# kfkq/DQMC

Measured on AMD Instinct MI355X. Metric: MC sweeps/sec, 2D Hubbard N=256 Ltau=200, higher is better.
Workload: dtype f64; 1 GPU; cfg3: 16x16 Hubbard U=8.0 beta=8.0 Ltau=200 n_stab=10 t=1 mu=-0.1; chains_per_gpu=1, n_chains_total=1, parallelism=independent chains, 1 gpu x 1 chain

## Files before the change

dqmc_amd/abi.py:

```python
from __future__ import annotations

import ctypes as C
import os
from typing import Optional, Tuple

import numpy as np

c_double_p = C.POINTER(C.c_double)
c_int64_p = C.POINTER(C.c_int64)
c_int32_p = C.POINTER(C.c_int32)
c_uint8_p = C.POINTER(C.c_uint8)


class Stats(C.Structure):
    _fields_ = [("acc_rate", C.c_double), ("max_err", C.c_double), ("sum_err", C.c_double),
                ("n_err", C.c_double), ("n_accepted", C.c_int64), ("n_proposed", C.c_int64)]

    @property
    def mean_err(self) -> float:
        return self.sum_err / self.n_err if self.n_err else 0.0


class DqmcError(RuntimeError):
    def __init__(self, code: int, msg: str):
        super().__init__(f"[{code}] {msg}")
        self.code = code


ABI_SYMBOLS = [
    "last_error", "backend", "device_count",
    "to_ldr", "ldr_mul_mat", "mat_mul_ldr", "ldr_mul_ldr", "inv_I_plus_ldr", "inv_I_plus_ldr_mul_ldr",
    "gemm", "rank1_update",
    "create", "create_batch", "n_chains", "destroy", "set_fields", "get_fields", "init", "get_G", "set_G", "get_logdet",
    "n_stack", "get_stack", "sweep_0_to_beta", "sweep_beta_to_0", "sync", "get_stats",
    "wrap_forward", "wrap_backward", "local_update_slice", "calculate_Bbar", "global_action", "set_checkerboard",
    "update_kernel_time", "set_profiling", "slice_path", "debug_snapshot",
    "measure_equal_time", "measure_accumulate", "measure_fetch",
    "sweep_unequal_time", "get_G_tau", "half_warp", "measure_unequal_time", "measure_unequal_fetch",
    "comm_unique_id", "comm_create_rccl", "comm_create_callbacks", "comm_destroy", "comm_rank", "comm_world_size",
    "comm_transport", "comm_barrier", "comm_allreduce_sum", "comm_selftest", "partner_rank", "replica_exchange_round",
    "replica_exchange_batch",
]

UNIQUE_ID_BYTES = 128
SENDRECV_FN = C.CFUNCTYPE(C.c_int, C.c_void_p, C.c_void_p, C.c_void_p, C.c_size_t, C.c_int, C.c_int)


class ExchangeResult(C.Structure):
    _fields_ = [("partner", C.c_int), ("decider", C.c_int), ("accepted", C.c_int), ("pad", C.c_int),
                ("S", C.c_double), ("S_prime", C.c_double), ("S_partner", C.c_double), ("S_prime_partner", C.c_double),
                ("deltaS", C.c_double)]


def _f64(a) -> np.ndarray:
    return np.asfortranarray(a, dtype=np.float64)


def _p(a: np.ndarray):
    return a.ctypes.data_as(c_double_p)


class DqmcLib:

    def __init__(self, path: str, prefix: str):
        if not os.path.exists(path):
            raise FileNotFoundError(
                f"{path} not found: build it first (python -c 'import __graft_entry__ as g; g.build()' or make)")
        self.path, self.prefix = path, prefix
        self._dll = C.CDLL(path, mode=C.RTLD_GLOBAL)
        g = self._sym
        g("last_error").restype = C.c_char_p
        g("backend").restype = C.c_char_p
        g("destroy").restype = None
        g("destroy").argtypes = [C.c_void_p]
        for name in ("set_fields", "get_fields"):
            g(name).argtypes = [C.c_void_p, c_int64_p]
        for name in ("init", "sync", "n_stack"):
            g(name).argtypes = [C.c_void_p]
        g("create").argtypes = [C.POINTER(C.c_void_p), C.c_int, C.c_int, C.c_int, C.c_int, C.c_double,
                                c_double_p, c_double_p, c_double_p, c_double_p]
        if self.has_symbol("create_batch"):
            g("create_batch").argtypes = [C.POINTER(C.c_void_p), C.c_int, C.c_int, C.c_int, C.c_int, C.c_int, c_double_p,
                                          c_double_p, c_double_p, c_double_p, c_double_p]
            g("n_chains").argtypes = [C.c_void_p]
        for name in ("get_G", "set_G", "get_logdet", "global_action"):
            g(name).argtypes = [C.c_void_p, c_double_p]
        g("get_stack").argtypes = [C.c_void_p, C.c_int, c_double_p, c_double_p, c_double_p]
        for name in ("sweep_0_to_beta", "sweep_beta_to_0"):
            g(name).argtypes = [C.c_void_p, c_int32_p, c_uint8_p, c_double_p]
        g("get_stats").argtypes = [C.c_void_p, C.c_void_p]
        for name in ("wrap_forward", "wrap_backward"):
            g(name).argtypes = [C.c_void_p, C.c_int]
        g("local_update_slice").argtypes = [C.c_void_p, C.c_int, c_int32_p, c_uint8_p, c_double_p, C.c_void_p]
        g("calculate_Bbar").argtypes = [C.c_void_p, C.c_int, c_double_p]
        g("set_checkerboard").argtypes = [C.c_void_p, C.c_int, c_int32_p, c_int32_p, c_double_p, c_double_p, c_double_p]
        g("update_kernel_time").argtypes = [C.c_void_p, c_double_p, c_int64_p, c_int64_p]
        g("set_profiling").argtypes = [C.c_void_p, C.c_int]
        if self.has_symbol("slice_path"):
            g("slice_path").argtypes = [C.c_void_p]
        if self.has_symbol("measure_equal_time"):
            g("measure_equal_time").argtypes = [C.c_void_p, C.c_int, C.c_int, c_double_p, c_double_p]
            g("measure_accumulate").argtypes = [C.c_void_p, C.c_int, C.c_int]
            g("measure_fetch").argtypes = [C.c_void_p, c_double_p, c_double_p, c_int64_p, C.c_int]
        if self.has_symbol("sweep_unequal_time"):
            g("sweep_unequal_time").argtypes = [C.c_void_p]
            g("get_G_tau").argtypes = [C.c_void_p, C.c_int, C.c_int, c_double_p]
            g("measure_unequal_time").argtypes = [C.c_void_p, C.c_int, C.c_int, C.c_int, c_double_p]
            g("measure_unequal_fetch").argtypes = [C.c_void_p, c_double_p, c_int64_p, C.c_int]
        if self.has_symbol("half_warp"):
            g("half_warp").argtypes = [C.c_void_p, c_double_p, c_double_p, C.c_int, C.c_int, c_double_p]
        if self.has_symbol("debug_snapshot"):
            g("debug_snapshot").argtypes = [C.c_void_p, c_double_p, C.c_void_p, C.c_void_p, C.c_void_p]
        if self.has_symbol("replica_exchange_round"):
            g("comm_unique_id").argtypes = [C.c_void_p]
            g("comm_create_rccl").argtypes = [C.POINTER(C.c_void_p), C.c_void_p, C.c_int, C.c_int, C.c_int]
            g("comm_create_callbacks").argtypes = [C.POINTER(C.c_void_p), C.c_int, C.c_int, SENDRECV_FN, C.c_void_p]
            g("comm_destroy").argtypes = [C.c_void_p]; g("comm_destroy").restype = None
            g("comm_rank").argtypes = [C.c_void_p]; g("comm_world_size").argtypes = [C.c_void_p]
            g("comm_transport").argtypes = [C.c_void_p]; g("comm_transport").restype = C.c_char_p
            g("comm_barrier").argtypes = [C.c_void_p]; g("comm_selftest").argtypes = [C.c_void_p]
            g("comm_allreduce_sum").argtypes = [C.c_void_p, c_double_p, C.c_int]
            g("partner_rank").argtypes = [C.c_int, C.c_int, C.c_int]
            g("replica_exchange_round").argtypes = [C.c_void_p, C.c_void_p, C.c_int, C.c_double, C.POINTER(ExchangeResult)]
        if self.has_symbol("replica_exchange_batch"):
            g("replica_exchange_batch").argtypes = [C.c_void_p, C.c_void_p, C.c_int, c_double_p, C.POINTER(ExchangeResult)]
        g("to_ldr").argtypes = [C.c_int] + [c_double_p] * 4
        g("ldr_mul_mat").argtypes = [C.c_int] + [c_double_p] * 7
        g("mat_mul_ldr").argtypes = [C.c_int] + [c_double_p] * 7
        g("ldr_mul_ldr").argtypes = [C.c_int] + [c_double_p] * 9
        g("inv_I_plus_ldr").argtypes = [C.c_int] + [c_double_p] * 5
        g("inv_I_plus_ldr_mul_ldr").argtypes = [C.c_int] + [c_double_p] * 7
        g("gemm").argtypes = [C.c_int, c_double_p, C.c_int, c_double_p, C.c_int, c_double_p]
        g("rank1_update").argtypes = [C.c_int, c_double_p, C.c_int, C.c_double]

    def _sym(self, name: str):
        return getattr(self._dll, self.prefix + name)

    def has_symbol(self, name: str) -> bool:
        return hasattr(self._dll, self.prefix + name)

    def check(self, rc: int):
        if rc != 0:
            raise DqmcError(rc, (self._sym("last_error")() or b"").decode())

    def backend(self) -> str:
        return self._sym("backend")().decode()

    def device_count(self) -> int:
        return int(self._sym("device_count")())

    def to_ldr(self, M) -> Tuple[np.ndarray, np.ndarray, np.ndarray]:
        M = _f64(M); n = M.shape[0]
        L, d, R = np.empty((n, n), order="F"), np.empty(n), np.empty((n, n), order="F")
        self.check(self._sym("to_ldr")(n, _p(M), _p(L), _p(d), _p(R)))
        return L, d, R

    def ldr_mul_mat(self, F, M):
        L, d, R = (_f64(x) for x in F); M = _f64(M); n = M.shape[0]
        Lo, do, Ro = np.empty((n, n), order="F"), np.empty(n), np.empty((n, n), order="F")
        self.check(self._sym("ldr_mul_mat")(n, _p(L), _p(d), _p(R), _p(M), _p(Lo), _p(do), _p(Ro)))
        return Lo, do, Ro

    def mat_mul_ldr(self, M, F):
        L, d, R = (_f64(x) for x in F); M = _f64(M); n = M.shape[0]
        Lo, do, Ro = np.empty((n, n), order="F"), np.empty(n), np.empty((n, n), order="F")
        self.check(self._sym("mat_mul_ldr")(n, _p(M), _p(L), _p(d), _p(R), _p(Lo), _p(do), _p(Ro)))
        return Lo, do, Ro

    def ldr_mul_ldr(self, F1, F2):
        L1, d1, R1 = (_f64(x) for x in F1); L2, d2, R2 = (_f64(x) for x in F2); n = L1.shape[0]
        Lo, do, Ro = np.empty((n, n), order="F"), np.empty(n), np.empty((n, n), order="F")
        self.check(self._sym("ldr_mul_ldr")(n, _p(L1), _p(d1), _p(R1), _p(L2), _p(d2), _p(R2), _p(Lo), _p(do), _p(Ro)))
        return Lo, do, Ro

    def inv_I_plus_ldr(self, F) -> Tuple[np.ndarray, float]:
        L, d, R = (_f64(x) for x in F); n = L.shape[0]
        G = np.empty((n, n), order="F"); ld = C.c_double(0.0)
        self.check(self._sym("inv_I_plus_ldr")(n, _p(L), _p(d), _p(R), _p(G), C.byref(ld)))
        return G, ld.value

    def inv_I_plus_ldr_mul_ldr(self, F1, F2) -> np.ndarray:
        L1, d1, R1 = (_f64(x) for x in F1); L2, d2, R2 = (_f64(x) for x in F2); n = L1.shape[0]
        G = np.empty((n, n), order="F")
        self.check(self._sym("inv_I_plus_ldr_mul_ldr")(n, _p(L1), _p(d1), _p(R1), _p(L2), _p(d2), _p(R2), _p(G)))
        return G

    def gemm(self, A, B, transA: bool = False, transB: bool = False) -> np.ndarray:
        A = _f64(A); B = _f64(B); n = A.shape[0]
        Cm = np.empty((n, n), order="F")
        self.check(self._sym("gemm")(n, _p(A), int(transA), _p(B), int(transB), _p(Cm)))
        return Cm

    def rank1_update(self, G, i: int, delta: float) -> np.ndarray:
        G = np.array(G, dtype=np.float64, order="F", copy=True); n = G.shape[0]
        self.check(self._sym("rank1_update")(n, _p(G), int(i), float(delta)))
        return G

    def engine(self, *args, **kw) -> "Engine":
        return Engine(self, *args, **kw)

    def partner_rank(self, rank: int, world: int, attempt: int) -> int:
        return int(self._sym("partner_rank")(rank, world, attempt))

    def exchange_batch(self, engine: "Engine", attempt: int, u, comm: Optional["Comm"] = None) -> list:
        uv = np.ascontiguousarray(np.asarray(u, dtype=np.float64).reshape(-1))
        if uv.shape != (engine.C,):
            raise ValueError(f"u must have shape ({engine.C},), got {uv.shape}")
        res = (ExchangeResult * engine.C)()
        self.check(self._sym("replica_exchange_batch")(engine._h, comm._h if comm is not None else None, int(attempt), _p(uv), res))
        return list(res)

    def comm_unique_id(self) -> bytes:
        buf = C.create_string_buffer(UNIQUE_ID_BYTES)
        self.check(self._sym("comm_unique_id")(buf))
        return buf.raw

    def comm_rccl(self, uid: bytes, world: int, rank: int, device: int) -> "Comm":
        h = C.c_void_p()
        self.check(self._sym("comm_create_rccl")(C.byref(h), C.c_char_p(uid), world, rank, device))
        return Comm(self, h)

    def comm_callbacks(self, world: int, rank: int, fn) -> "Comm":
        def tramp(_user, send, recv, nbytes, partner, tag):
            try:
                got = fn(C.string_at(send, nbytes), int(partner), int(tag))
                if len(got) != nbytes:
                    return -2
                C.memmove(recv, got, nbytes)
                return 0
            except Exception:
                return -1
        cb = SENDRECV_FN(tramp)
        h = C.c_void_p()
        self.check(self._sym("comm_create_callbacks")(C.byref(h), world, rank, cb, None))
        return Comm(self, h, keep=cb)


class Comm:

    def __init__(self, lib: "DqmcLib", h, keep=None):
        self.lib, self._h, self._keep = lib, h, keep

    @property
    def rank(self) -> int:
        return int(self.lib._sym("comm_rank")(self._h))

    @property
    def world(self) -> int:
        return int(self.lib._sym("comm_world_size")(self._h))

    @property
    def transport(self) -> str:
        return self.lib._sym("comm_transport")(self._h).decode()

    def selftest(self):
        self.lib.check(self.lib._sym("comm_selftest")(self._h))

    def barrier(self):
        self.lib.check(self.lib._sym("comm_barrier")(self._h))

    def allreduce_sum(self, x) -> np.ndarray:
        v = np.ascontiguousarray(x, dtype=np.float64).copy()
        self.lib.check(self.lib._sym("comm_allreduce_sum")(self._h, _p(v), int(v.size)))
        return v

    def exchange_round(self, engine: "Engine", attempt: int, u: float) -> ExchangeResult:
        res = ExchangeResult()
        self.lib.check(self.lib._sym("replica_exchange_round")(engine._h, self._h, int(attempt), float(u), C.byref(res)))
        return res

    def exchange_batch(self, engine: "Engine", attempt: int, u) -> list:
        return self.lib.exchange_batch(engine, attempt, u, comm=self)

    def close(self):
        if self._h is not None:
            self.lib._sym("comm_destroy")(self._h); self._h = None

    def __del__(self):
        try:
            self.close()
        except Exception:
            pass


class Engine:

    def __init__(self, lib: DqmcLib, n_sites: int, nt: int, n_stab: int, g, gamma, eta,
                 expK, invexpK, device: int = 0, n_chains: Optional[int] = None):
        self.lib, self.n, self.nt, self.n_stab = lib, int(n_sites), int(nt), int(n_stab)
        self.batched = n_chains is not None
        self.C = int(n_chains) if self.batched else 1
        gamma = np.ascontiguousarray(gamma, dtype=np.float64); eta = np.ascontiguousarray(eta, dtype=np.float64)
        h = C.c_void_p()
        if not self.batched:
            eK, iK = _f64(expK), _f64(invexpK)
            assert eK.shape == (self.n, self.n) and iK.shape == (self.n, self.n)
            lib.check(lib._sym("create")(C.byref(h), device, self.n, self.nt, self.n_stab, float(g),
                                         _p(gamma), _p(eta), _p(eK), _p(iK)))
        else:
            gv = np.ascontiguousarray(np.broadcast_to(np.asarray(g, dtype=np.float64), (self.C,)))
            eK = self._mats_in(np.broadcast_to(np.asarray(expK), (self.C, self.n, self.n)) if np.ndim(expK) == 2 else expK)
            iK = self._mats_in(np.broadcast_to(np.asarray(invexpK), (self.C, self.n, self.n)) if np.ndim(invexpK) == 2 else invexpK)
            lib.check(lib._sym("create_batch")(C.byref(h), device, self.C, self.n, self.nt, self.n_stab, _p(gv),
                                               _p(gamma), _p(eta), _p(eK), _p(iK)))
        self._h: Optional[C.c_void_p] = h

    def _mats_in(self, a) -> np.ndarray:
        a = np.asarray(a, dtype=np.float64).reshape(self.C, self.n, self.n)
        return np.ascontiguousarray(a.transpose(0, 2, 1))

    def _mats_out(self, buf: np.ndarray) -> np.ndarray:
        m = buf.reshape(self.C, self.n, self.n).transpose(0, 2, 1)
        return m if self.batched else np.asfortranarray(m[0])

    def _vec_out(self, buf: np.ndarray) -> np.ndarray:
        return buf.reshape(self.C, -1) if self.batched else buf.reshape(-1)

    def close(self):
        if self._h is not None:
            self.lib._sym("destroy")(self._h); self._h = None

    def __del__(self):
        try:
            self.close()
        except Exception:
            pass

    def __enter__(self):
        return self

    def __exit__(self, *a):
        self.close()

    def _c(self, name, *args):
        self.lib.check(self.lib._sym(name)(self._h, *args))

    def set_fields(self, fields):
        f = np.asarray(fields).reshape(self.C, self.nt, self.n)
        f = np.ascontiguousarray(f.transpose(0, 2, 1), dtype=np.int64)
        self._c("set_fields", f.ctypes.data_as(c_int64_p))

    def get_fields(self) -> np.ndarray:
        f = np.empty((self.C, self.n, self.nt), dtype=np.int64)
        self._c("get_fields", f.ctypes.data_as(c_int64_p))
        f = f.transpose(0, 2, 1)
        return f if self.batched else f[0]

    def init(self):
        self._c("init")

    def get_G(self) -> np.ndarray:
        G = np.empty(self.C * self.n * self.n); self._c("get_G", _p(G)); return self._mats_out(G)

    def set_G(self, G):
        G = self._mats_in(G); self._c("set_G", _p(G))

    def get_logdet(self):
        v = np.zeros(self.C); self._c("get_logdet", _p(v)); return v if self.batched else float(v[0])

    def n_stack(self) -> int:
        return int(self.lib._sym("n_stack")(self._h))

    def get_stack(self, i: int):
        L, d, R = np.empty(self.C * self.n * self.n), np.empty(self.C * self.n), np.empty(self.C * self.n * self.n)
        self._c("get_stack", int(i), _p(L), _p(d), _p(R))
        return self._mats_out(L), self._vec_out(d), self._mats_out(R)

    def _stream(self, perm, kprop, u, rows):
        perm = np.ascontiguousarray(np.asarray(perm).reshape(self.C, rows, self.n), dtype=np.int32)
        kprop = np.ascontiguousarray(np.asarray(kprop).reshape(self.C, rows, self.n), dtype=np.uint8)
        u = np.ascontiguousarray(np.asarray(u).reshape(self.C, rows, self.n), dtype=np.float64)
        return perm, kprop, u

    def sweep_0_to_beta(self, perm, kprop, u):
        perm, kprop, u = self._stream(perm, kprop, u, self.nt)
        self._c("sweep_0_to_beta", perm.ctypes.data_as(c_int32_p), kprop.ctypes.data_as(c_uint8_p), _p(u))

    def sweep_beta_to_0(self, perm, kprop, u):
        perm, kprop, u = self._stream(perm, kprop, u, self.nt)
        self._c("sweep_beta_to_0", perm.ctypes.data_as(c_int32_p), kprop.ctypes.data_as(c_uint8_p), _p(u))

    def sync(self):
        self._c("sync")

    def stats(self):
        arr = (Stats * self.C)(); self._c("get_stats", arr)
        return list(arr) if self.batched else arr[0]

    def wrap_forward(self, l: int):
        self._c("wrap_forward", int(l))

    def wrap_backward(self, l: int):
        self._c("wrap_backward", int(l))

    def local_update_slice(self, l: int, perm, kprop, u):
        perm, kprop, u = self._stream(perm, kprop, u, 1)
        acc = (C.c_int * self.C)()
        self._c("local_update_slice", int(l), perm.ctypes.data_as(c_int32_p), kprop.ctypes.data_as(c_uint8_p), _p(u), acc)
        return list(acc) if self.batched else acc[0]

    def calculate_Bbar(self, i_stack: int) -> np.ndarray:
        B = np.empty(self.C * self.n * self.n); self._c("calculate_Bbar", int(i_stack), _p(B)); return self._mats_out(B)

    def set_checkerboard(self, groups, cosh_t, sinh_t, diag_factor):
        sizes = np.ascontiguousarray([len(g) for g in groups], np.int32)
        flat = [p for g in groups for p in g]
        bonds = np.ascontiguousarray(np.asarray(flat, np.int32).reshape(-1, 2) if flat else np.zeros((1, 2), np.int32))
        par = [np.ascontiguousarray(np.broadcast_to(np.asarray(x, np.float64), (self.C,))) for x in (cosh_t, sinh_t, diag_factor)]
        self._c("set_checkerboard", len(groups), bonds.ctypes.data_as(c_int32_p), sizes.ctypes.data_as(c_int32_p), _p(par[0]), _p(par[1]), _p(par[2]))

    def global_action(self):
        v = np.zeros(self.C); self._c("global_action", _p(v)); return v if self.batched else float(v[0])

    def measure_equal_time(self, L1: int, L2: int):
        sc = np.empty((self.C, 3)); chi = np.empty((self.C, L1 * L2))
        self._c("measure_equal_time", int(L1), int(L2), _p(sc), _p(chi))
        chi = chi.reshape(self.C, L2, L1).transpose(0, 2, 1)
        return (sc, chi) if self.batched else (sc[0], chi[0])

    def measure_accumulate(self, L1: int, L2: int):
        self._c("measure_accumulate", int(L1), int(L2))

    def measure_fetch(self, L1: int, L2: int, reset: bool = True):
        sc = np.empty((self.C, 3)); chi = np.empty((self.C, L1 * L2)); cnt = np.zeros(1, dtype=np.int64)
        self._c("measure_fetch", _p(sc), _p(chi), cnt.ctypes.data_as(c_int64_p), 1 if reset else 0)
        chi = chi.reshape(self.C, L2, L1).transpose(0, 2, 1)
        return ((sc, chi) if self.batched else (sc[0], chi[0])) + (int(cnt[0]),)

    def sweep_unequal_time(self):
        self._c("sweep_unequal_time")

    def get_G_tau(self, which: str, l: int) -> np.ndarray:
        B = np.empty(self.C * self.n * self.n); self._c("get_G_tau", {"tt": 0, "t0": 1, "0t": 2}[which], int(l), _p(B)); return self._mats_out(B)

    def half_warp(self, expK_half=None, invexpK_half=None, which: str = "G", l: int = 0) -> np.ndarray:
        a = _f64(expK_half) if expK_half is not None else None; b = _f64(invexpK_half) if invexpK_half is not None else None
        B = np.empty(self.C * self.n * self.n)
        self._c("half_warp", _p(a) if a is not None else None, _p(b) if b is not None else None, {"G": -1, "tt": 0, "t0": 1, "0t": 2}[which], int(l), _p(B))
        return self._mats_out(B)

    def _ut_cube(self, flat, L1, L2):
        a = flat.reshape(self.C, 3, self.nt + 1, L2, L1).transpose(0, 1, 2, 4, 3)
        return a if self.batched else a[0]

    def measure_unequal_time(self, L1: int, L2: int, accumulate: bool = False):
        if accumulate:
            self._c("measure_unequal_time", int(L1), int(L2), 1, None); return None
        out = np.empty(self.C * 3 * (self.nt + 1) * L1 * L2)
        self._c("measure_unequal_time", int(L1), int(L2), 0, _p(out)); return self._ut_cube(out, L1, L2)

    def measure_unequal_fetch(self, L1: int, L2: int, reset: bool = True):
        out = np.empty(self.C * 3 * (self.nt + 1) * L1 * L2); cnt = np.zeros(1, dtype=np.int64)
        self._c("measure_unequal_fetch", _p(out), cnt.ctypes.data_as(c_int64_p), 1 if reset else 0)
        return self._ut_cube(out, L1, L2), int(cnt[0])

    def debug_snapshot(self):
        ns = self.n_stack()
        we = np.zeros(ns); acc = np.zeros(self.nt, np.int32); sw = np.zeros(80, np.uint32); ep = C.c_uint(0)
        self._c("debug_snapshot", _p(we), acc.ctypes.data, sw.ctypes.data, C.byref(ep))
        return dict(wrap_err=we, accepted=acc, sync_words=sw, slice_epoch=int(ep.value))

    def slice_path(self) -> int:
        return int(self.lib._sym("slice_path")(self._h))

    def set_profiling(self, on: bool):
        self._c("set_profiling", int(bool(on)))

    def update_kernel_time(self):
        ms = C.c_double(0.0); nl = C.c_int64(0); na = C.c_int64(0)
        self._c("update_kernel_time", C.cast(C.byref(ms), c_double_p), C.cast(C.byref(nl), c_int64_p), C.cast(C.byref(na), c_int64_p))
        return ms.value, nl.value, na.value
```

dqmc_amd/csrc/common.h:

```cpp
#pragma once

#include <hip/hip_runtime.h>
#include <cstdint>
#include <memory>
#include <string>

struct dqmc_engine;

namespace dq {

constexpr int WAVE = 64;

void set_error(const std::string& msg);
const char* get_error();

#define DQ_HIP(call)                                                                    \
    do {                                                                                \
        hipError_t _e = (call);                                                         \
        if (_e != hipSuccess) {                                                         \
            ::dq::set_error(std::string(#call) + ": " + hipGetErrorString(_e));         \
            return -2;                                              \
        }                                                                               \
    } while (0)

#define DQ_TRY(expr)                \
    do {                            \
        int _rc = (expr);           \
        if (_rc != 0) return _rc;   \
    } while (0)

template <class T, hipError_t (*Free)(void*)> struct HipDelete { void operator()(T* p) const { (void)Free(p); } };
template <class T> using DevPtr = std::unique_ptr<T[], HipDelete<T, hipFree>>;
using PinnedPtr = std::unique_ptr<char[], HipDelete<char, hipHostFree>>;
template <class T> int dev_alloc(DevPtr<T>& out, size_t count) {
    void* p = nullptr;
    DQ_HIP(hipMalloc(&p, sizeof(T) * count));
    out.reset(static_cast<T*>(p));
    return 0;
}

constexpr int DQ_STATUS_PIVOT = 1;
constexpr int DQ_STATUS_COOP_QR = 2;
constexpr int DQ_STATUS_HANDOFF = 4;
constexpr int DQ_STATUS_CENSUS = 8;

struct Mat {
    double* p = nullptr;
    long stride = 0;
    __host__ __device__ double* at(int c) const { return p + (long)c * stride; }
};
struct CMat {
    const double* p = nullptr;
    long stride = 0;
    CMat() = default;
    __host__ __device__ CMat(const double* p_, long s) : p(p_), stride(s) {}
    __host__ __device__ CMat(const Mat& m) : p(m.p), stride(m.stride) {}
    __host__ __device__ const double* at(int c) const { return p + (long)c * stride; }
};
using Vec = Mat;
using CVec = CMat;

struct GemmDesc {
    CMat A, B;
    Mat C;
    Mat CT{nullptr, 0};
    CVec rs, ks, cs;
    int n = 0;
    int transA = 0;
    int accumulate = 0;
};
int launch_gemm(const GemmDesc& g, int n_chains, hipStream_t s);

int launch_build_expv(const int8_t* fields, long f_stride, int nt, int n, const double* tab_expv ,
                      double* expv, double* invexpv, long v_stride, int n_chains, hipStream_t s);
int launch_split_d(CVec d, Vec dl_inv, Vec ds, double* logsum, int n, int n_chains, hipStream_t s);
int launch_split_d2(CVec d1, Vec dl1, Vec ds1, CVec d2, Vec dl2, Vec ds2, int n, int n_chains, hipStream_t s);
int launch_measure_equal_time(CMat G, double* out, long out_stride, int L1, int L2, int accumulate, int n_chains, hipStream_t s);
int launch_measure_unequal_time(const double* Gtt, const double* Gt0, const double* G0t, double* out, long out_stride, int L1, int L2, int nt,
                                int accumulate, int n_chains, hipStream_t s);
int launch_axpb_identity(CMat in, Mat out, double a, double b, int n, int n_chains, hipStream_t s);
int launch_copy(CMat in, Mat out, long count, int n_chains, hipStream_t s);
int launch_set_identity(Mat out, int n, int n_chains, hipStream_t s);
int launch_transpose_scale(CMat in, Mat out, CVec rs, int n, int n_chains, hipStream_t s);
int launch_max_abs_diff(CMat A, CMat B, double* err, long err_stride, int n, int n_chains, hipStream_t s);
int launch_add_scaled_cols(CMat A, CMat B, CVec cs, Mat C, int n, int n_chains, hipStream_t s);
int launch_scale_rows(CMat in, CVec rs, Mat out, int n, int n_chains, hipStream_t s);
struct DevStats { double acc_rate, max_err, sum_err, n_err; long long n_accepted, n_proposed; };
int launch_fold_stats(DevStats* st, const int* acc, long acc_stride, int n_slices, const double* err, long err_stride, int n_err,
                      int n, int nt, int n_chains, hipStream_t s);

struct QrWork {
    double* tau; long tau_stride;
    int* jpvt; long jpvt_stride;
    unsigned long long* sync = nullptr; long sync_stride = 0;
    int* abort_words = nullptr;
    int* info = nullptr;
    double* pw = nullptr; long pw_stride = 0;
    int* pivpos = nullptr; long pivpos_stride = 0;
};
long qr_panel_work_doubles(int n);
int launch_qr_panel_formq(QrWork w, Mat L, int n, int n_chains, hipStream_t s);
int launch_qr_panel(Mat A, QrWork w, int n, int n_chains, hipStream_t s);
long qrcp_coop_sync_granules(int n);
int qrcp_coop_workgroups(int n, int n_chains);
enum class QrFamily { Panel, ColumnOwner, Cooperative, Streaming };
int launch_to_ldr(QrFamily f, Mat A, Mat L, Vec d, Mat R, QrWork w, int n, int n_chains, hipStream_t s);

int launch_lu_blocked(Mat A, int* perm, long perm_stride, int* rowpos, long rowpos_stride, double* logabsdet, int accumulate_logdet,
                      int* info, int n, int n_chains, hipStream_t s);
int launch_lu_solve(CMat LU, const int* perm, long perm_stride, Mat X, CVec dg, int mode, int n, int n_chains, hipStream_t s);

int launch_tri_solve(CMat R, const int* perm, long perm_stride, Mat X, CVec dg, double* scratch, long scratch_stride, int n, int n_chains, hipStream_t s);

int launch_gj_solve(Mat A, Mat B, Mat X, Mat SA, double* tinv, int* perm, long perm_stride, int* rowpos, long rowpos_stride,
                    double* logabsdet, int accumulate_logdet, int* info, int n, int n_chains, hipStream_t s);

struct UpdateTables {
    double rb[4][3];
    double delta[4][3];
    double ev[4];
    double iev[4];
    double pad[32];
};
struct UpdateDesc {
    Mat G;
    int8_t* fields; long f_stride;
    double* expv; double* invexpv; long v_stride;
    const UpdateTables* tabs;
    const int32_t* perm; const uint8_t* kprop; const double* u; long rs_stride;
    double* Upanel; double* Wpanel; long panel_stride;
    double* Cpanel = nullptr;
    int* state; long state_stride;
    double* prep; long prep_stride;
    Mat GT{nullptr, 0};
    int gt_valid = 0;
    void* slice_sync = nullptr;
    unsigned slice_epoch = 0;
    int slice_absent_tile = -1;
    int slice_absent_l = -1;
    int slice_late_tile = -1, slice_late_us = 0;
    int* info = nullptr;
    int* acc_out; long acc_stride;
    int n, nt;
};
constexpr int UPDATE_KD = 32;

struct SliceSync {
    unsigned long long seq; unsigned int error; unsigned int solo_count; unsigned int pad[12];
    unsigned int arrive[496];
};
constexpr size_t SLICE_SYNC_BYTES = 2048;
static_assert(sizeof(SliceSync) == SLICE_SYNC_BYTES, "SliceSync layout");
constexpr unsigned SLICE_EPOCH_LIMIT = 1u << 24;
constexpr unsigned SLICE_SOLO_BIT = 1u << 30, SLICE_FINAL_BIT = 1u << 31;
__host__ __device__ inline unsigned slice_tag(unsigned epoch, unsigned window) { return (epoch << 8) | window; }
enum class SlicePath { PersistentWalk, PersistentSubmatrix, Solo, Pairs, PairsTailSolo };
int launch_update_slice(SlicePath path, const UpdateDesc& d, int l, int acc_slot, int n_chains, hipStream_t s);
int launch_update_slice_sm(const UpdateDesc& d, int l, int acc_slot, int n_chains, hipStream_t s);
int slice_flush_workgroups(int n);
bool slice_reserve(int device, int n, int n_chains);
void slice_release(int device, int n, int n_chains);
int launch_rank1(Mat G, int i, double delta, double* scratch , long scratch_stride, int n, int n_chains, hipStream_t s);

struct CbDesc {
    CMat in;
    Mat out{nullptr, 0}, outT{nullptr, 0};
    const int* partner = nullptr;
    int n_groups = 0, reverse = 0, inverse = 0;
    const double* par = nullptr; long par_stride = 0;
    CVec rs_in, cs_in, rs_out, cs_out;
    int n = 0;
};
int launch_cb_apply(const CbDesc& d, int n_chains, hipStream_t s);

int update_init_device();
int update_sm_init_device();
int qr_init_device();
int qr_colown_init_device();
int init_device_kernels(int device);

struct EngineFieldsView { int device, n, nt, n_chains; int8_t* fields; hipStream_t stream; };
int engine_fields_view(dqmc_engine* h, EngineFieldsView* v);
int engine_fields_changed(dqmc_engine* h);
int engine_exchange_scratch(dqmc_engine* h, int8_t** saved, int8_t** recv, int** tab);

}
```

dqmc_amd/csrc/engine.hip:

```cpp
#include "common.h"
#include "../../include/dqmc_hip.h"

#include <cmath>
#include <cstdlib>
#include <cstring>
#include <map>
#include <memory>
#include <mutex>
#include <vector>

namespace dq {

static thread_local std::string g_err;
void set_error(const std::string& msg) { g_err = msg; }
const char* get_error() { return g_err.c_str(); }

int init_device_kernels(int device) {
    static std::mutex mu; static bool done[64] = {};
    std::lock_guard<std::mutex> lk(mu);
    if (device < 0 || device >= 64) { set_error("device ordinal out of range"); return -1; }
    if (done[device]) return 0;
    DQ_HIP(hipSetDevice(device));
    DQ_TRY(update_init_device()); DQ_TRY(update_sm_init_device()); DQ_TRY(qr_init_device()); DQ_TRY(qr_colown_init_device());
    done[device] = true;
    return 0;
}

struct Switches { bool qr_panel, qr_streaming, walk_submatrix, lu_classic, slice_multikernel; };
static const Switches& switches() {
    static const Switches sw = [] {
        const char* panel = getenv("DQMC_QR_PANEL");
        return Switches{!(panel && atoi(panel) == 0), getenv("DQMC_QR_STREAMING") != nullptr, getenv("DQMC_WALK_SUBMATRIX") != nullptr,
                        getenv("DQMC_LU_CLASSIC") != nullptr, getenv("DQMC_SLICE_MULTIKERNEL") != nullptr};
    }();
    return sw;
}

constexpr int GJ_MAX_N = 1024, GJ_MAX_CHAINS = 8;
constexpr int TRI_MAX_N = 640;

static QrFamily pick_qr(int n, int chains, bool allow_panel) {
    const Switches& sw = switches();
    if (sw.qr_streaming) return QrFamily::Streaming;
    if (allow_panel && sw.qr_panel && n >= 64 && n <= 1024 && n % 16 == 0 && chains <= 8) return QrFamily::Panel;
    if (n <= 256) return QrFamily::ColumnOwner;
    return qrcp_coop_workgroups(n, chains) <= 200 ? QrFamily::Cooperative : QrFamily::Streaming;
}

struct KernelPlan {
    QrFamily qr;
    enum class Solve { GaussJordan, BlockedLu } solve;
    enum class Rinv { Blocked, PerColumn } rinv;
    static KernelPlan pick(int n, int chains) {
        return KernelPlan{pick_qr(n, chains, true),
                          n <= GJ_MAX_N && chains <= GJ_MAX_CHAINS && !switches().lu_classic ? Solve::GaussJordan : Solve::BlockedLu,
                          n <= TRI_MAX_N ? Rinv::Blocked : Rinv::PerColumn};
    }
};

static SlicePath pick_slice_path(int n, int chains, bool reserved) {
    const Switches& sw = switches();
    const bool walk = n <= 256;
    if (sw.slice_multikernel) return SlicePath::Pairs;
    if (reserved) return walk && !sw.walk_submatrix ? SlicePath::PersistentWalk : SlicePath::PersistentSubmatrix;
    if (!walk) return SlicePath::Pairs;
    return chains >= 224 ? SlicePath::Solo : SlicePath::PairsTailSolo;
}
static bool is_persistent(SlicePath p) { return p == SlicePath::PersistentWalk || p == SlicePath::PersistentSubmatrix; }

struct LdrRef {
    Mat L; Vec d; Mat R;
    int* jpvt = nullptr;
    bool* tri = nullptr;
};
struct LdrStore {
    int n = 0, C = 0;
    DevPtr<double> L, d, R;
    DevPtr<int> jpvt;
    std::unique_ptr<bool[]> tri;
    int alloc(int k, int n_, int C_) {
        n = n_; C = C_;
        const size_t nn = (size_t)n * n;
        DQ_TRY(dev_alloc(L, (size_t)k * C * nn)); DQ_TRY(dev_alloc(d, (size_t)k * C * n));
        DQ_TRY(dev_alloc(R, (size_t)k * C * nn)); DQ_TRY(dev_alloc(jpvt, (size_t)k * C * n));
        tri.reset(new bool[k]());
        return 0;
    }
    LdrRef at(int i) const {
        const long nn = (long)n * n;
        return LdrRef{Mat{L.get() + (long)i * C * nn, nn}, Vec{d.get() + (long)i * C * n, (long)n}, Mat{R.get() + (long)i * C * nn, nn},
                      jpvt.get() + (long)i * C * n, &tri[i]};
    }
};

struct Ctx {
    int n = 0, C = 0, device = 0;
    long nn = 0;
    hipStream_t stream = nullptr;
    static constexpr int NT = 6, NV = 5;
    DevPtr<double> pool;
    DevPtr<double> vpool;
    DevPtr<int> ipool;
    DevPtr<unsigned long long> qsync;
    DevPtr<int> qabort;
    DevPtr<double> tinv;
    DevPtr<double> qpw;
    DevPtr<int> qpivpos;
    DevPtr<double> trinv;
    KernelPlan plan{};

    Mat T(int k) const { return Mat{pool.get() + (long)k * C * nn, nn}; }
    Vec V(int k) const { return Vec{vpool.get() + (long)k * C * n, (long)n}; }
    int* jpvt() const { return ipool.get(); }
    int* lperm() const { return ipool.get() + (long)C * n; }
    int* rowpos() const { return ipool.get() + 2L * C * n; }
    int* info() const { return ipool.get() + 3L * C * n; }

    int init(int n_, int C_, int device_) {
        n = n_; C = C_; device = device_; nn = (long)n * n;
        DQ_HIP(hipSetDevice(device));
        DQ_TRY(init_device_kernels(device));
        DQ_HIP(hipStreamCreateWithFlags(&stream, hipStreamNonBlocking));
        DQ_TRY(dev_alloc(pool, (size_t)NT * C * nn));
        DQ_TRY(dev_alloc(vpool, (size_t)NV * C * n));
        DQ_TRY(dev_alloc(ipool, 3L * C * n + 4));
        plan = KernelPlan::pick(n, C);
        if (plan.qr == QrFamily::Cooperative) { DQ_TRY(dev_alloc(qsync, (size_t)qrcp_coop_sync_granules(n) * C)); DQ_TRY(dev_alloc(qabort, C)); }
        if (plan.qr == QrFamily::Panel) { DQ_TRY(dev_alloc(qpw, (size_t)qr_panel_work_doubles(n) * C)); DQ_TRY(dev_alloc(qpivpos, (size_t)n * C)); }
        if (plan.solve == KernelPlan::Solve::GaussJordan) DQ_TRY(dev_alloc(tinv, (size_t)2048 * C));
        if (plan.rinv == KernelPlan::Rinv::Blocked) DQ_TRY(dev_alloc(trinv, (size_t)16 * (n + 16) * C));
        DQ_HIP(hipMemsetAsync(ipool.get(), 0, sizeof(int) * (3L * C * n + 4), stream));
        return 0;
    }
    ~Ctx() { if (stream) (void)hipStreamDestroy(stream); }

    int gemm(CMat A, CMat B, Mat Cm, CVec rs = CVec(), CVec ks = CVec(), CVec cs = CVec(), int transA = 0, int accumulate = 0, Mat CT = Mat{nullptr, 0}) {
        GemmDesc g; g.A = A; g.B = B; g.C = Cm; g.CT = CT; g.rs = rs; g.ks = ks; g.cs = cs; g.n = n; g.transA = transA; g.accumulate = accumulate;
        return launch_gemm(g, C, stream);
    }
    int to_ldr(Mat A, LdrRef out, bool direct = true) {
        const bool keep = direct && out.jpvt != nullptr;
        QrWork w{V(4).p, (long)n, keep ? out.jpvt : jpvt(), (long)n};
        w.sync = qsync.get(); w.sync_stride = qrcp_coop_sync_granules(n); w.abort_words = qabort.get(); w.info = info();
        w.pw = qpw.get(); w.pw_stride = qr_panel_work_doubles(n); w.pivpos = qpivpos.get(); w.pivpos_stride = n;
        if (out.tri) *out.tri = keep;
        return launch_to_ldr(plan.qr, A, out.L, out.d, out.R, w, n, C, stream);
    }
    int r_inverse_scaled(LdrRef F, CVec dinv, Mat X, Mat lu_scratch) {
        if (F.tri && *F.tri && F.jpvt) {
            if (plan.rinv == KernelPlan::Rinv::Blocked) return launch_tri_solve(F.R, F.jpvt, n, X, dinv, trinv.get(), 16L * (n + 16), n, C, stream);
            return launch_lu_solve(F.R, F.jpvt, n, X, dinv, 2, n, C, stream);
        }
        DQ_TRY(launch_copy(F.R, lu_scratch, nn, C, stream));
        DQ_TRY(launch_lu_blocked(lu_scratch, lperm(), n, rowpos(), n, nullptr, 0, info(), n, C, stream));
        return launch_lu_solve(lu_scratch, lperm(), n, X, dinv, 1, n, C, stream);
    }
    int mat_mul_ldr(CMat M, LdrRef F, LdrRef out) {
        DQ_TRY(gemm(M, F.L, T(0), CVec(), CVec(), CVec(F.d)));
        LdrRef q{out.L, out.d, T(1)};
        DQ_TRY(to_ldr(T(0), q));
        if (out.tri) *out.tri = false;
        return gemm(T(1), F.R, out.R);
    }
    int ldr_mul_mat(LdrRef F, CMat M, LdrRef out) {
        DQ_TRY(gemm(F.R, M, T(0), CVec(F.d)));
        LdrRef q{T(1), out.d, out.R, out.jpvt, out.tri};
        DQ_TRY(to_ldr(T(0), q));
        return gemm(F.L, T(1), out.L);
    }
    int ldr_mul_ldr(LdrRef F1, LdrRef F2, LdrRef out) {
        DQ_TRY(gemm(F1.R, F2.L, T(0), CVec(F1.d), CVec(), CVec(F2.d)));
        LdrRef q{T(1), out.d, T(2)};
        DQ_TRY(to_ldr(T(0), q));
        if (out.tri) *out.tri = false;
        DQ_TRY(gemm(F1.L, T(1), out.L));
        return gemm(T(2), F2.R, out.R);
    }
    int solve(Mat M, Mat RHS, Mat out, double* logdet_acc, Mat* Y) {
        if (plan.solve == KernelPlan::Solve::GaussJordan) {
            DQ_TRY(launch_gj_solve(M, RHS, out, T(5), tinv.get(), lperm(), n, rowpos(), n, logdet_acc, 1, info(), n, C, stream));
            *Y = out; return 0;
        }
        DQ_TRY(launch_lu_blocked(M, lperm(), n, rowpos(), n, logdet_acc, 1, info(), n, C, stream));
        DQ_TRY(launch_lu_solve(M, lperm(), n, RHS, CVec(), 0, n, C, stream));
        *Y = RHS; return 0;
    }
    int inv_I_plus_ldr(LdrRef F, Mat G, double* logdet ) {
        DQ_TRY(launch_split_d(F.d, V(0), V(1), logdet, n, C, stream));
        DQ_TRY(r_inverse_scaled(F, V(0), T(1), T(0)));
        DQ_TRY(launch_add_scaled_cols(T(1), F.L, V(1), T(2), n, C, stream));
        DQ_TRY(launch_transpose_scale(T(2), T(3), CVec(), n, C, stream));
        DQ_TRY(launch_transpose_scale(T(1), T(4), CVec(), n, C, stream));
        Mat Y; DQ_TRY(solve(T(3), T(4), T(0), logdet, &Y));
        return launch_transpose_scale(Y, G, CVec(), n, C, stream);
    }
    int inv_I_plus_ldr_mul_ldr(LdrRef F1, LdrRef F2, Mat G) {
        DQ_TRY(launch_split_d2(F1.d, V(0), V(1), F2.d, V(2), V(3), n, C, stream));
        DQ_TRY(r_inverse_scaled(F2, V(2), T(1), T(0)));
        DQ_TRY(gemm(F1.L, T(1), T(2), V(0), CVec(), CVec(), 1));
        DQ_TRY(gemm(F1.R, F2.L, T(2), V(1), CVec(), V(3), 0, 1));
        DQ_TRY(launch_transpose_scale(F1.L, T(3), V(0), n, C, stream));
        Mat Y; DQ_TRY(solve(T(2), T(3), T(0), nullptr, &Y));
        return gemm(T(1), Y, G);
    }
    int inv_invldr_plus_ldr(LdrRef F1, LdrRef F2, Mat G, bool negate) {
        DQ_TRY(launch_split_d(F1.d, V(0), V(1), nullptr, n, C, stream));
        DQ_TRY(launch_split_d(F2.d, V(2), V(3), nullptr, n, C, stream));
        DQ_TRY(r_inverse_scaled(F2, V(2), T(1), T(0)));
        DQ_TRY(gemm(F1.L, T(1), T(2), V(0), CVec(), CVec(), 1));
        DQ_TRY(gemm(F1.R, F2.L, T(2), V(1), CVec(), V(3), 0, 1));
        DQ_TRY(launch_scale_rows(F1.R, V(1), T(3), n, C, stream));
        Mat Y; DQ_TRY(solve(T(2), T(3), T(0), nullptr, &Y));
        DQ_TRY(gemm(T(1), Y, G));
        if (negate) DQ_TRY(launch_axpb_identity(G, G, -1.0, 0.0, n, C, stream));
        return 0;
    }
};

static int take_status(const Ctx& c, int* bits = nullptr) {
    int w[4] = {0, 0, 0, 0};
    DQ_HIP(hipMemcpy(w, c.info(), sizeof w, hipMemcpyDeviceToHost));
    if (bits) *bits = w[0];
    if (w[0] == 0) return 0;
    (void)hipMemset(c.info(), 0, sizeof w);
    if (w[0] & DQ_STATUS_HANDOFF) {
        set_error("persistent slice kernel: a workgroup that had checked in stopped answering (device fault or pre-emption beyond the spin bound); the chain state is undefined -- set the fields again and call dqmc_init; this engine uses the scan / flush kernel pairs from now on");
    } else if (w[0] & DQ_STATUS_CENSUS) {
        char msg[640];
        snprintf(msg, sizeof msg, "persistent sub-matrix slice kernel: its workgroups did not all become resident at time slice %d (device shared with other "
                 "work?).  That slice and every later slice of the call(s) in flight proposed NOTHING (fields unchanged there, acceptance counts 0, their part of "
                 "the random stream is spent); wraps and stabilisations ran, so fields, G and the stack are consistent with each other, but the sweep is not the "
                 "one the stream describes from that slice on.  This engine uses the scan / flush kernel pairs from now on: restore the fields of the last "
                 "completed sweep and call dqmc_init, or keep the state as a valid (shortened) sweep", w[1] - 1);
        set_error(msg);
    } else if (w[0] & DQ_STATUS_COOP_QR) {
        set_error("cooperative QRCP gave up waiting for a partner workgroup (not co-resident?)");
    } else {
        set_error("LU factorisation hit a zero or NaN pivot");
    }
    return DQMC_ENUMERIC;
}

struct Engine {
    int n = 0, nt = 0, n_stab = 0, n_stack = 0, C = 1, device = 0;
    long nn = 0;
    std::vector<int> loc_l_end;
    std::vector<double> g_host, gamma_host, eta_host;
    std::vector<unsigned char> seen;
    Ctx ctx;
    hipStream_t s = nullptr;

    DevPtr<double> expK, invexpK;
    bool cb = false; int cb_groups = 0;
    DevPtr<int> cb_partner;
    DevPtr<double> cb_par;
    DevPtr<int8_t> fields;
    DevPtr<double> expv, invexpv;
    DevPtr<UpdateTables> tabs; DevPtr<double> tab8;
    bool gt_valid = false;
    DevPtr<double> G, Gtmp, GT;
    DevPtr<double> pg_eye, pg_ones;
    DevPtr<double> bb0, bb1;
    LdrStore stack;
    LdrStore spare;
    DevPtr<double> logdet;
    DevPtr<int32_t> rs_perm; DevPtr<uint8_t> rs_k; DevPtr<double> rs_u;
    PinnedPtr h_stage;
    hipEvent_t stage_free = nullptr;
    DevPtr<double> Upanel, Wpanel;
    DevPtr<double> Cpanel;
    struct InitBatch { DevPtr<double> bb, tau; LdrStore f; } ib;
    DevPtr<int> state;
    DevPtr<double> prep;
    DevPtr<double> meas_now, meas_sum;
    struct UnequalTime { DevPtr<double> G[3], tmp, err, meas_now, meas_sum; LdrStore bt; } ut;
    bool ut_valid = false; long long ut_meas_count = 0;
    struct HalfWarp { DevPtr<double> expK, invexpK, out; } hw;
    long long meas_count = 0;
    DevPtr<char> slice_sync;
    bool reserved = false;
    SlicePath slice_path = SlicePath::Pairs;
    unsigned slice_epoch = 0;
    int slice_absent_l = -1;
    int slice_late_tile = -1, slice_late_us = 0;
    int slice_absent_tile = -1;
    DevPtr<int> acc;
    struct Exchange { DevPtr<int8_t> saved, recv; DevPtr<int> tab; } xch;
    DevPtr<double> err;
    DevPtr<DevStats> dstats;
    bool stack_valid = false;
    bool profiling = false;
    std::vector<std::pair<hipEvent_t, hipEvent_t>> ev_pairs;
    size_t ev_used = 0;
    double upd_ms = 0.0; long long upd_launches = 0; long long upd_accept_base = 0;

    Mat mG() const { return Mat{G.get(), nn}; }
    CVec ev(int l) const { return CVec(expv.get() + (long)l * n, (long)nt * n); }
    CVec iev(int l) const { return CVec(invexpv.get() + (long)l * n, (long)nt * n); }
    int stack_idx(int l) const { return l / n_stab; }
    int local_l(int l) const { return l % n_stab; }

    ~Engine() {
        if (s) (void)hipStreamSynchronize(s);
        if (reserved) slice_release(device, n, C);
        for (auto& p : ev_pairs) { (void)hipEventDestroy(p.first); (void)hipEventDestroy(p.second); }
        if (stage_free) (void)hipEventDestroy(stage_free);
    }

    int create(int device_, int C_, int n_, int nt_, int n_stab_, const double* g, const double* gamma, const double* eta,
               const double* eK, const double* ieK) {
        device = device_; C = C_; n = n_; nt = nt_; n_stab = n_stab_; nn = (long)n * n;
        n_stack = (int)std::ceil(static_cast<double>(nt) / n_stab);
        loc_l_end.assign(n_stack, n_stab - 1);
        if (nt % n_stab != 0) loc_l_end[n_stack - 1] = nt % n_stab - 1;
        g_host.assign(g, g + C); gamma_host.assign(gamma, gamma + 4); eta_host.assign(eta, eta + 4);
        DQ_TRY(ctx.init(n, C, device)); s = ctx.stream;
        reserved = slice_reserve(device, n, C);
        slice_path = pick_slice_path(n, C, reserved);
        if (const char* a = getenv("DQMC_DEBUG_SLICE_ABSENT")) { slice_absent_tile = atoi(a); if (const char* c = strchr(a, ':')) slice_absent_l = atoi(c + 1); }
        if (const char* a = getenv("DQMC_DEBUG_SLICE_LATE")) { slice_late_tile = atoi(a); if (const char* c = strchr(a, ':')) slice_late_us = atoi(c + 1); }
        DQ_TRY(dev_alloc(expK, C * nn)); DQ_TRY(dev_alloc(invexpK, C * nn));
        DQ_TRY(dev_alloc(fields, (size_t)C * nt * n)); DQ_TRY(dev_alloc(expv, (size_t)C * nt * n)); DQ_TRY(dev_alloc(invexpv, (size_t)C * nt * n));
        DQ_TRY(dev_alloc(tabs, C)); DQ_TRY(dev_alloc(tab8, (size_t)C * 8));
        if (C == 1) { DQ_TRY(dev_alloc(pg_eye, nn)); DQ_TRY(dev_alloc(pg_ones, (size_t)n)); DQ_TRY(launch_set_identity(Mat{pg_eye.get(), nn}, n, 1, s)); const std::vector<double> one_h((size_t)n, 1.0); DQ_HIP(hipMemcpy(pg_ones.get(), one_h.data(), sizeof(double) * n, hipMemcpyHostToDevice)); }
        DQ_TRY(dev_alloc(G, C * nn)); DQ_TRY(dev_alloc(Gtmp, C * nn)); DQ_TRY(dev_alloc(GT, C * nn)); DQ_TRY(dev_alloc(bb0, C * nn)); DQ_TRY(dev_alloc(bb1, C * nn));
        DQ_TRY(stack.alloc(n_stack, n, C)); DQ_TRY(spare.alloc(1, n, C));
        DQ_TRY(dev_alloc(logdet, C));
        DQ_TRY(dev_alloc(rs_perm, (size_t)C * nt * n)); DQ_TRY(dev_alloc(rs_k, (size_t)C * nt * n)); DQ_TRY(dev_alloc(rs_u, (size_t)C * nt * n));
        DQ_TRY(dev_alloc(Upanel, (size_t)C * UPDATE_KD * n)); DQ_TRY(dev_alloc(Wpanel, (size_t)C * UPDATE_KD * n)); DQ_TRY(dev_alloc(Cpanel, (size_t)C * UPDATE_KD * UPDATE_KD));
        DQ_TRY(dev_alloc(state, (size_t)C * 4)); DQ_TRY(dev_alloc(prep, (size_t)C * 4 * n)); DQ_TRY(dev_alloc(meas_now, (size_t)C * (3 + n))); DQ_TRY(dev_alloc(meas_sum, (size_t)C * (3 + n))); DQ_HIP(hipMemsetAsync(meas_sum.get(), 0, sizeof(double) * C * (3 + n), s)); DQ_TRY(dev_alloc(slice_sync, (size_t)C * SLICE_SYNC_BYTES)); DQ_HIP(hipMemsetAsync(slice_sync.get(), 0, (size_t)C * SLICE_SYNC_BYTES, s)); DQ_TRY(dev_alloc(acc, (size_t)C * nt)); DQ_TRY(dev_alloc(err, (size_t)C * n_stack));
        DQ_TRY(dev_alloc(dstats, C));
        void* stage = nullptr;
        DQ_HIP(hipHostMalloc(&stage, (size_t)C * nt * n * (sizeof(int32_t) + sizeof(uint8_t) + sizeof(double)), hipHostMallocDefault)); h_stage.reset(static_cast<char*>(stage));
        DQ_HIP(hipEventCreateWithFlags(&stage_free, hipEventDisableTiming));
        DQ_HIP(hipEventRecord(stage_free, s));
        DQ_HIP(hipMemcpyAsync(expK.get(), eK, sizeof(double) * C * nn, hipMemcpyHostToDevice, s));
        DQ_HIP(hipMemcpyAsync(invexpK.get(), ieK, sizeof(double) * C * nn, hipMemcpyHostToDevice, s));
        DQ_HIP(hipMemsetAsync(fields.get(), 0, (size_t)C * nt * n, s));
        DQ_HIP(hipMemsetAsync(G.get(), 0, sizeof(double) * C * nn, s));
        DQ_HIP(hipMemsetAsync(dstats.get(), 0, sizeof(DevStats) * C, s));
        DQ_HIP(hipMemsetAsync(logdet.get(), 0, sizeof(double) * C, s));
        DQ_HIP(hipMemsetAsync(state.get(), 0, sizeof(int) * C * 4, s));
        std::vector<UpdateTables> ht(C); std::vector<double> h8((size_t)C * 8);
        static const int proposal[4][3] = {{1, 2, 3}, {0, 2, 3}, {0, 1, 3}, {0, 1, 2}};
        const double alpha = -1.0;
        for (int c = 0; c < C; ++c) {
            std::memset(&ht[c], 0, sizeof(UpdateTables));
            for (int o = 0; o < 4; ++o) for (int k = 0; k < 3; ++k) {
                const int nf = proposal[o][k];
                const double gammaR = gamma[nf] / gamma[o];
                const double d_eta = eta[nf] - eta[o];
                const double bosonR = std::exp(alpha * g[c] * d_eta);
                ht[c].rb[o][k] = gammaR * bosonR;
                ht[c].delta[o][k] = (1.0 / bosonR) - 1.0;
            }
            for (int f = 0; f < 4; ++f) { ht[c].ev[f] = std::exp(g[c] * eta[f]); ht[c].iev[f] = std::exp(-g[c] * eta[f]); h8[(size_t)c * 8 + f] = ht[c].ev[f]; h8[(size_t)c * 8 + 4 + f] = ht[c].iev[f]; }
        }
        DQ_HIP(hipMemcpyAsync(tabs.get(), ht.data(), sizeof(UpdateTables) * C, hipMemcpyHostToDevice, s));
        DQ_HIP(hipMemcpyAsync(tab8.get(), h8.data(), sizeof(double) * C * 8, hipMemcpyHostToDevice, s));
        DQ_TRY(launch_build_expv(fields.get(), (long)nt * n, nt, n, tab8.get(), expv.get(), invexpv.get(), (long)nt * n, C, s));
        DQ_HIP(hipStreamSynchronize(s));
        return 0;
    }

    int cb_apply(CMat in, Mat out, Mat outT, bool reverse, bool inverse, CVec rs_in, CVec cs_in, CVec rs_out, CVec cs_out, int chains, long par_stride) {
        CbDesc d; d.in = in; d.out = out; d.outT = outT; d.partner = cb_partner.get(); d.n_groups = cb_groups; d.reverse = reverse ? 1 : 0; d.inverse = inverse ? 1 : 0;
        d.par = cb_par.get(); d.par_stride = par_stride; d.rs_in = rs_in; d.cs_in = cs_in; d.rs_out = rs_out; d.cs_out = cs_out; d.n = n;
        return launch_cb_apply(d, chains, s);
    }
    int set_checkerboard(int n_groups, const int32_t* bonds, const int32_t* group_sizes, const double* ch, const double* sh, const double* f) {
        if (n_groups < 1 || n_groups > 64 || !bonds || !group_sizes || !ch || !sh || !f) { set_error("set_checkerboard: bad argument"); return DQMC_EINVAL; }
        if (n > 4096) { set_error("set_checkerboard: n_sites > 4096"); return DQMC_EINVAL; }
        std::vector<int> partner((size_t)n_groups * n);
        size_t b = 0;
        for (int g = 0; g < n_groups; ++g) {
            int* pt = partner.data() + (size_t)g * n;
            for (int i = 0; i < n; ++i) pt[i] = i;
            if (group_sizes[g] < 0 || group_sizes[g] > n / 2) { set_error("set_checkerboard: a group holds at most n_sites/2 bonds"); return DQMC_EINVAL; }
            for (int k = 0; k < group_sizes[g]; ++k, ++b) {
                const int i = bonds[2 * b], j = bonds[2 * b + 1];
                if (i < 0 || i >= n || j < 0 || j >= n || i == j) { set_error("set_checkerboard: bond site out of range"); return DQMC_EINVAL; }
                if (pt[i] != i || pt[j] != j) { set_error("set_checkerboard: the bonds of one group must be disjoint"); return DQMC_EINVAL; }
                pt[i] = j; pt[j] = i;
            }
        }
        std::vector<double> par((size_t)C * 4);
        for (int c = 0; c < C; ++c) {
            if (!(f[c] > 0.0) || !std::isfinite(ch[c]) || !std::isfinite(sh[c])) { set_error("set_checkerboard: diag_factor must be positive, cosh / sinh finite"); return DQMC_EINVAL; }
            par[4 * c] = ch[c]; par[4 * c + 1] = sh[c]; par[4 * c + 2] = f[c]; par[4 * c + 3] = 1.0 / f[c];
        }
        DQ_HIP(hipStreamSynchronize(s));
        if (!cb_par) DQ_TRY(dev_alloc(cb_par, (size_t)C * 4));
        DevPtr<int> pt;
        DQ_TRY(dev_alloc(pt, partner.size()));
        DQ_HIP(hipMemcpy(pt.get(), partner.data(), sizeof(int) * partner.size(), hipMemcpyHostToDevice));
        DQ_HIP(hipMemcpy(cb_par.get(), par.data(), sizeof(double) * par.size(), hipMemcpyHostToDevice));
        cb_partner = std::move(pt); cb_groups = n_groups; cb = true;
        Mat id{bb0.get(), nn};
        DQ_TRY(launch_set_identity(id, n, C, s));
        DQ_TRY(cb_apply(id, Mat{expK.get(), nn}, Mat{nullptr, 0}, false, false, CVec(), CVec(), CVec(), CVec(), C, 4));
        DQ_TRY(cb_apply(id, Mat{invexpK.get(), nn}, Mat{nullptr, 0}, true, true, CVec(), CVec(), CVec(), CVec(), C, 4));
        stack_valid = false; gt_valid = false; ut_valid = false;
        DQ_HIP(hipStreamSynchronize(s));
        return 0;
    }

    int Bbar(int is, Mat* out) {
        const int l0 = is * n_stab;
        Mat cur{bb0.get(), nn}, nxt{bb1.get(), nn};
        DQ_TRY(launch_scale_rows(CMat(expK.get(), nn), ev(l0), cur, n, C, s));
        for (int loc = 1; loc <= loc_l_end[is]; ++loc) {
            if (cb) DQ_TRY(cb_apply(cur, nxt, Mat{nullptr, 0}, false, false, CVec(), CVec(), ev(l0 + loc), CVec(), C, 4));
            else DQ_TRY(ctx.gemm(CMat(expK.get(), nn), cur, nxt, ev(l0 + loc)));
            std::swap(cur, nxt);
        }
        *out = cur; return 0;
    }
    int init() {
        if (C == 1 && n <= 256 && nt % n_stab == 0 && n_stack >= 2) return init_batched();
        const LdrRef tmp = spare.at(0);
        for (int i = n_stack - 1; i >= 0; --i) {
            Mat bb; DQ_TRY(Bbar(i, &bb));
            if (i == n_stack - 1) DQ_TRY(ctx.to_ldr(bb, stack.at(i)));
            else { DQ_TRY(ctx.to_ldr(bb, tmp)); DQ_TRY(ctx.ldr_mul_ldr(stack.at(i + 1), tmp, stack.at(i))); }
        }
        stack_valid = true;
        gt_valid = false;
        return ctx.inv_I_plus_ldr(stack.at(0), mG(), logdet.get());
    }
    int init_batched() {
        const int S = n_stack;
        if (!ib.tau) {
            InitBatch b; DQ_TRY(dev_alloc(b.bb, (size_t)2 * S * nn)); DQ_TRY(dev_alloc(b.tau, (size_t)S * n)); DQ_TRY(b.f.alloc(S, n, 1));
            ib = std::move(b);
        }
        const long bstride = (long)n_stab * n;
        Mat cur{ib.bb.get(), nn}, nxt{ib.bb.get() + (size_t)S * nn, nn};
        DQ_TRY(launch_scale_rows(CMat(expK.get(), 0), CVec(expv.get(), bstride), cur, n, S, s));
        for (int loc = 1; loc < n_stab; ++loc) {
            if (cb) DQ_TRY(cb_apply(cur, nxt, Mat{nullptr, 0}, false, false, CVec(), CVec(), CVec(expv.get() + (long)loc * n, bstride), CVec(), S, 0));
            else {
                GemmDesc g; g.A = CMat(expK.get(), 0); g.B = cur; g.C = nxt; g.rs = CVec(expv.get() + (long)loc * n, bstride); g.n = n;
                DQ_TRY(launch_gemm(g, S, s));
            }
            std::swap(cur, nxt);
        }
        const LdrRef all = ib.f.at(0);
        QrWork w{ib.tau.get(), (long)n, all.jpvt, (long)n};
        w.info = ctx.info();
        DQ_TRY(launch_to_ldr(pick_qr(n, S, false), cur, all.L, all.d, all.R, w, n, S, s));
        const LdrRef last = stack.at(S - 1), own = ib.f.at(S - 1);
        DQ_TRY(launch_copy(own.L, last.L, nn, 1, s));
        DQ_TRY(launch_copy(own.R, last.R, nn, 1, s));
        DQ_HIP(hipMemcpyAsync(last.d.p, own.d.p, sizeof(double) * n, hipMemcpyDeviceToDevice, s));
        DQ_HIP(hipMemcpyAsync(last.jpvt, own.jpvt, sizeof(int) * n, hipMemcpyDeviceToDevice, s));
        *last.tri = true;
        for (int i = S - 2; i >= 0; --i) DQ_TRY(ctx.ldr_mul_ldr(stack.at(i + 1), ib.f.at(i), stack.at(i)));
        stack_valid = true;
        gt_valid = false;
        return ctx.inv_I_plus_ldr(stack.at(0), mG(), logdet.get());
    }
    int wrap_forward(int l) {
        if (cb) {
            DQ_TRY(cb_apply(mG(), Mat{nullptr, 0}, ctx.T(0), false, false, CVec(), CVec(), CVec(), CVec(), C, 4));
            gt_valid = use_gt();
            return cb_apply(ctx.T(0), Mat{GT.get(), nn}, mG(), false, true, CVec(), CVec(), iev(l), ev(l), C, 4);
        }
        DQ_TRY(ctx.gemm(CMat(expK.get(), nn), mG(), ctx.T(0)));
        gt_valid = use_gt();
        return ctx.gemm(ctx.T(0), CMat(invexpK.get(), nn), mG(), ev(l), CVec(), iev(l), 0, 0, use_gt() ? Mat{GT.get(), nn} : Mat{nullptr, 0});
    }
    bool piggyback() const { return C == 1 && !cb && n <= 256 && pg_eye != nullptr; }
    int wrap_forward_piggy(int l, const double* Pprev, double* Pnext) {
        GemmDesc g; g.A = CMat(expK.get(), 0); g.B = CMat(G.get(), (long)(Pprev - G.get())); g.C = Mat{ctx.T(0).p, (long)(Pnext - ctx.T(0).p)};
        g.rs = CVec(pg_ones.get(), (long)((expv.get() + (long)(l - 1) * n) - pg_ones.get())); g.n = n;
        DQ_TRY(launch_gemm(g, 2, s));
        gt_valid = use_gt();
        return ctx.gemm(ctx.T(0), CMat(invexpK.get(), nn), mG(), ev(l), CVec(), iev(l), 0, 0, use_gt() ? Mat{GT.get(), nn} : Mat{nullptr, 0});
    }
    int wrap_backward_piggy(int l, const double* Pprev, double* Pnext) {
        DQ_TRY(ctx.gemm(CMat(invexpK.get(), nn), mG(), ctx.T(0), CVec(), iev(l)));
        gt_valid = use_gt();
        GemmDesc g; g.A = CMat(ctx.T(0).p, (long)(Pprev - ctx.T(0).p)); g.B = CMat(expK.get(), 0); g.C = Mat{G.get(), (long)(Pnext - G.get())};
        g.ks = CVec(expv.get() + (long)l * n, 0); g.n = n;
        if (use_gt()) g.CT = Mat{GT.get(), (long)(ctx.T(1).p - GT.get())};
        return launch_gemm(g, 2, s);
    }
    int wrap_backward(int l) {
        if (cb) {
            DQ_TRY(cb_apply(mG(), Mat{nullptr, 0}, ctx.T(0), true, true, iev(l), ev(l), CVec(), CVec(), C, 4));
            gt_valid = use_gt();
            return cb_apply(ctx.T(0), Mat{GT.get(), nn}, mG(), true, false, CVec(), CVec(), CVec(), CVec(), C, 4);
        }
        DQ_TRY(ctx.gemm(CMat(invexpK.get(), nn), mG(), ctx.T(0), CVec(), iev(l)));
        gt_valid = use_gt();
        return ctx.gemm(ctx.T(0), CMat(expK.get(), nn), mG(), CVec(), ev(l), CVec(), 0, 0, use_gt() ? Mat{GT.get(), nn} : Mat{nullptr, 0});
    }
    bool use_gt() const { return n <= 256 || slice_path == SlicePath::PersistentSubmatrix; }
    UpdateDesc udesc() const {
        UpdateDesc d; d.G = mG(); d.fields = fields.get(); d.f_stride = (long)nt * n; d.expv = expv.get(); d.invexpv = invexpv.get(); d.v_stride = (long)nt * n;
        d.tabs = tabs.get(); d.perm = rs_perm.get(); d.kprop = rs_k.get(); d.u = rs_u.get(); d.rs_stride = (long)nt * n; d.Upanel = Upanel.get(); d.Wpanel = Wpanel.get(); d.Cpanel = Cpanel.get();
        d.panel_stride = (long)UPDATE_KD * n; d.state = state.get(); d.state_stride = 4; d.prep = prep.get(); d.prep_stride = 4L * n; d.slice_sync = is_persistent(slice_path) ? slice_sync.get() : nullptr; d.slice_epoch = slice_epoch; d.slice_absent_tile = slice_absent_tile; d.slice_absent_l = slice_absent_l; d.slice_late_tile = slice_late_tile; d.slice_late_us = slice_late_us; d.GT = Mat{GT.get(), nn}; d.gt_valid = gt_valid ? 1 : 0; d.info = ctx.info(); d.acc_out = acc.get(); d.acc_stride = nt; d.n = n; d.nt = nt;
        return d;
    }
    int local_update(int l) {
        hipEvent_t e0 = nullptr, e1 = nullptr;
        if (profiling) {
            if (ev_used == ev_pairs.size()) { hipEvent_t a, b; DQ_HIP(hipEventCreate(&a)); DQ_HIP(hipEventCreate(&b)); ev_pairs.emplace_back(a, b); }
            e0 = ev_pairs[ev_used].first; e1 = ev_pairs[ev_used].second; ++ev_used;
            DQ_HIP(hipEventRecord(e0, s));
        }
        if (is_persistent(slice_path)) {
            if (++slice_epoch >= SLICE_EPOCH_LIMIT) { DQ_HIP(hipMemsetAsync(slice_sync.get(), 0, (size_t)C * SLICE_SYNC_BYTES, s)); slice_epoch = 1; }
        }
        DQ_TRY(launch_update_slice(slice_path, udesc(), l, l, C, s));
        if (profiling) DQ_HIP(hipEventRecord(e1, s));
        return 0;
    }
    int check_stream(const char* who, const int32_t* perm, const uint8_t* kprop, const double* u, size_t rows) {
        if (!perm || !kprop || !u) { set_error(std::string(who) + ": null random-stream pointer"); return DQMC_EINVAL; }
        seen.assign((size_t)n, 0);
        for (size_t row = 0; row < rows; ++row) {
            const int32_t* pr = perm + row * n; const uint8_t* kr = kprop + row * n; const unsigned char mark = (unsigned char)(1 + (row & 1));
            if ((row & 1) == 0) std::fill(seen.begin(), seen.end(), 0);
            for (int idx = 0; idx < n; ++idx) {
                const int32_t i = pr[idx];
                if (i < 0 || i >= n || seen[i] == mark || kr[idx] > 2) { set_error(std::string(who) + ": perm is not a permutation of the sites, or kprop > 2"); return DQMC_EINVAL; }
                seen[i] = mark;
            }
        }
        return 0;
    }
    int upload_stream(const int32_t* perm, const uint8_t* kprop, const double* u) {
        const size_t cnt = (size_t)C * nt * n;
        DQ_TRY(check_stream("sweep", perm, kprop, u, (size_t)C * nt));
        DQ_HIP(hipEventSynchronize(stage_free));
        char* base = h_stage.get();
        double* hu = reinterpret_cast<double*>(base);
        int32_t* hp = reinterpret_cast<int32_t*>(base + cnt * sizeof(double));
        uint8_t* hk = reinterpret_cast<uint8_t*>(base + cnt * (sizeof(double) + sizeof(int32_t)));
        std::memcpy(hu, u, cnt * sizeof(double)); std::memcpy(hp, perm, cnt * sizeof(int32_t)); std::memcpy(hk, kprop, cnt);
        DQ_HIP(hipMemcpyAsync(rs_u.get(), hu, cnt * sizeof(double), hipMemcpyHostToDevice, s));
        DQ_HIP(hipMemcpyAsync(rs_perm.get(), hp, cnt * sizeof(int32_t), hipMemcpyHostToDevice, s));
        DQ_HIP(hipMemcpyAsync(rs_k.get(), hk, cnt, hipMemcpyHostToDevice, s));
        DQ_HIP(hipEventRecord(stage_free, s));
        return 0;
    }
    int sweep_fwd() {
        int n_err = 0;
        DQ_HIP(hipMemsetAsync(err.get(), 0, sizeof(double) * C * n_stack, s));
        const bool pg = piggyback();
        double* Pcur = bb0.get(); double* Pnxt = bb1.get();
        for (int l = 0; l < nt; ++l) {
            const int is = stack_idx(l), loc = local_l(l);
            if (pg && loc >= 1) { DQ_TRY(wrap_forward_piggy(l, loc == 1 ? pg_eye.get() : Pcur, Pnxt)); std::swap(Pcur, Pnxt); }
            else DQ_TRY(wrap_forward(l));
            DQ_TRY(local_update(l));
            if (loc == loc_l_end[is]) {
                std::swap(G, Gtmp);
                Mat bb;
                if (pg) {
                    if (loc == 0) DQ_TRY(launch_scale_rows(CMat(expK.get(), nn), ev(l), Mat{Pnxt, nn}, n, C, s));
                    else DQ_TRY(ctx.gemm(CMat(expK.get(), nn), CMat(Pcur, nn), Mat{Pnxt, nn}, ev(l)));
                    std::swap(Pcur, Pnxt); bb = Mat{Pcur, nn};
                } else DQ_TRY(Bbar(is, &bb));
                if (is == 0) DQ_TRY(ctx.to_ldr(bb, stack.at(0)));
                else DQ_TRY(ctx.mat_mul_ldr(bb, stack.at(is - 1), stack.at(is)));
                gt_valid = false;
                if (l == nt - 1) DQ_TRY(ctx.inv_I_plus_ldr(stack.at(is), mG(), logdet.get()));
                else DQ_TRY(ctx.inv_I_plus_ldr_mul_ldr(stack.at(is), stack.at(is + 1), mG()));
                DQ_TRY(launch_max_abs_diff(CMat(Gtmp.get(), nn), mG(), err.get() + n_err, n_stack, n, C, s));
                ++n_err;
            }
        }
        return launch_fold_stats(dstats.get(), acc.get(), nt, nt, err.get(), n_stack, n_err, n, nt, C, s);
    }
    int sweep_bwd() {
        int n_err = 0;
        DQ_HIP(hipMemsetAsync(err.get(), 0, sizeof(double) * C * n_stack, s));
        const bool pg = piggyback();
        double* Pcur = bb0.get(); double* Pnxt = bb1.get();
        for (int l = nt - 1; l >= 0; --l) {
            DQ_TRY(local_update(l));
            const int is = stack_idx(l);
            if (pg) { DQ_TRY(wrap_backward_piggy(l, local_l(l) == loc_l_end[is] ? pg_eye.get() : Pcur, Pnxt)); std::swap(Pcur, Pnxt); }
            else DQ_TRY(wrap_backward(l));
            if (local_l(l) == 0) {
                std::swap(G, Gtmp);
                Mat bb;
                if (pg) bb = Mat{Pcur, nn}; else DQ_TRY(Bbar(is, &bb));
                if (is == n_stack - 1) DQ_TRY(ctx.to_ldr(bb, stack.at(is)));
                else DQ_TRY(ctx.ldr_mul_mat(stack.at(is + 1), bb, stack.at(is)));
                gt_valid = false;
                if (l == 0) DQ_TRY(ctx.inv_I_plus_ldr(stack.at(is), mG(), logdet.get()));
                else DQ_TRY(ctx.inv_I_plus_ldr_mul_ldr(stack.at(is - 1), stack.at(is), mG()));
                DQ_TRY(launch_max_abs_diff(CMat(Gtmp.get(), nn), mG(), err.get() + n_err, n_stack, n, C, s));
                ++n_err;
            }
        }
        return launch_fold_stats(dstats.get(), acc.get(), nt, nt, err.get(), n_stack, n_err, n, nt, C, s);
    }
    Mat utm(int which, int l) const { return Mat{ut.G[which].get() + (long)l * C * nn, nn}; }
    int sweep_unequal() {
        if (!ut.tmp) {
            UnequalTime u;
            for (int w = 0; w < 3; ++w) DQ_TRY(dev_alloc(u.G[w], (size_t)(nt + 1) * C * nn));
            DQ_TRY(dev_alloc(u.tmp, (size_t)3 * C * nn)); DQ_TRY(dev_alloc(u.err, (size_t)C * 3 * n_stack));
            const size_t mcount = (size_t)C * 3 * (nt + 1) * n;
            DQ_TRY(dev_alloc(u.meas_now, mcount)); DQ_TRY(dev_alloc(u.meas_sum, mcount)); DQ_TRY(u.bt.alloc(2, n, C));
            DQ_HIP(hipMemsetAsync(u.meas_sum.get(), 0, sizeof(double) * mcount, s));
            ut = std::move(u);
        }
        auto bt = [&](int b) { return ut.bt.at(b); };
        int cur = 0, n_err = 0;
        DQ_HIP(hipMemsetAsync(ut.err.get(), 0, sizeof(double) * C * 3 * n_stack, s));
        DQ_TRY(launch_copy(mG(), utm(0, 0), nn, C, s));
        for (int l = 0; l < nt; ++l) {
            if (l == 0) {
                DQ_TRY(launch_copy(utm(0, 0), utm(1, 0), nn, C, s));
                DQ_TRY(launch_axpb_identity(utm(0, 0), utm(2, 0), 1.0, -1.0, n, C, s));
            }
            DQ_TRY(ctx.gemm(CMat(expK.get(), nn), utm(0, l), ctx.T(0)));
            DQ_TRY(ctx.gemm(ctx.T(0), CMat(invexpK.get(), nn), utm(0, l + 1), ev(l), CVec(), iev(l)));
            DQ_TRY(ctx.gemm(CMat(expK.get(), nn), utm(1, l), utm(1, l + 1), ev(l)));
            DQ_TRY(ctx.gemm(utm(2, l), CMat(invexpK.get(), nn), utm(2, l + 1), CVec(), CVec(), iev(l)));
            const int is = stack_idx(l);
            if (local_l(l) == loc_l_end[is]) {
                for (int w = 0; w < 3; ++w) DQ_TRY(launch_copy(utm(w, l + 1), Mat{ut.tmp.get() + (long)w * C * nn, nn}, nn, C, s));
                Mat bb; DQ_TRY(Bbar(is, &bb));
                if (is == 0) DQ_TRY(ctx.to_ldr(bb, bt(cur)));
                else { DQ_TRY(ctx.mat_mul_ldr(bb, bt(cur), bt(cur ^ 1))); cur ^= 1; }
                if (l == nt - 1) {
                    DQ_TRY(ctx.inv_I_plus_ldr(bt(cur), utm(0, l + 1), logdet.get()));
                    DQ_TRY(launch_axpb_identity(utm(0, l + 1), utm(1, l + 1), -1.0, 1.0, n, C, s));
                    DQ_TRY(launch_axpb_identity(utm(0, l + 1), utm(2, l + 1), -1.0, 0.0, n, C, s));
                } else {
                    DQ_TRY(ctx.inv_I_plus_ldr_mul_ldr(bt(cur), stack.at(is + 1), utm(0, l + 1)));
                    DQ_TRY(ctx.inv_invldr_plus_ldr(bt(cur), stack.at(is + 1), utm(1, l + 1), false));
                    DQ_TRY(ctx.inv_invldr_plus_ldr(stack.at(is + 1), bt(cur), utm(2, l + 1), true));
                }
                for (int w = 0; w < 3; ++w) {
                    DQ_TRY(launch_max_abs_diff(CMat(ut.tmp.get() + (long)w * C * nn, nn), utm(w, l + 1), ut.err.get() + n_err, 3L * n_stack, n, C, s));
                    ++n_err;
                }
            }
        }
        ut_valid = true;
        return launch_fold_stats(dstats.get(), acc.get(), nt, 0, ut.err.get(), 3L * n_stack, n_err, n, nt, C, s);
    }
    int sync_and_check() {
        DQ_HIP(hipStreamSynchronize(s));
        if (profiling && ev_used) {
            for (size_t k = 0; k < ev_used; ++k) { float ms = 0.f; DQ_HIP(hipEventElapsedTime(&ms, ev_pairs[k].first, ev_pairs[k].second)); upd_ms += ms; }
            upd_launches += (long long)ev_used; ev_used = 0;
        }
        int bits = 0;
        const int rc = take_status(ctx, &bits);
        if (bits & (DQ_STATUS_HANDOFF | DQ_STATUS_CENSUS)) {
            slice_path = pick_slice_path(n, C, false); gt_valid = false;
            if (bits & DQ_STATUS_HANDOFF) { (void)hipMemset(slice_sync.get(), 0, (size_t)C * SLICE_SYNC_BYTES); slice_epoch = 0; }
        }
        return rc;
    }
    int download_fields(std::vector<int8_t>& f) const {
        std::vector<int8_t> dev((size_t)C * nt * n);
        DQ_HIP(hipMemcpy(dev.data(), fields.get(), dev.size(), hipMemcpyDeviceToHost));
        f.resize(dev.size());
        for (int c = 0; c < C; ++c) for (int i = 0; i < n; ++i) for (int l = 0; l < nt; ++l)
            f[(size_t)c * nt * n + l + (size_t)nt * i] = dev[(size_t)c * nt * n + (size_t)l * n + i];
        return 0;
    }
    int copy_out_equal_time(const double* src, double* scalars, double* chi_r) const {
        const size_t w = 3 + (size_t)n;
        std::vector<double> tmp((size_t)C * w);
        DQ_HIP(hipMemcpy(tmp.data(), src, sizeof(double) * tmp.size(), hipMemcpyDeviceToHost));
        for (int c = 0; c < C; ++c) {
            if (scalars) std::copy(tmp.begin() + c * w, tmp.begin() + c * w + 3, scalars + 3 * (size_t)c);
            if (chi_r) std::copy(tmp.begin() + c * w + 3, tmp.begin() + (c + 1) * w, chi_r + (size_t)c * n);
        }
        return 0;
    }
};

struct Stateless {
    Ctx ctx;
    LdrStore ldr;
    DevPtr<double> mats;
    DevPtr<double> logdet;
    Mat M(int k) const { return Mat{mats.get() + k * ctx.nn, ctx.nn}; }
};
static std::mutex g_ctx_mu;
static std::map<int, std::unique_ptr<Stateless>> g_ctx;

static int get_ctx(int n, Stateless** out) {
    if (n <= 0) { set_error("n must be positive"); return DQMC_EINVAL; }
    int count = 0;
    if (hipGetDeviceCount(&count) != hipSuccess || count == 0) { set_error("no HIP device available: this library requires a gfx950 GPU"); return DQMC_ENODEVICE; }
    auto it = g_ctx.find(n);
    if (it == g_ctx.end()) {
        std::unique_ptr<Stateless> x(new Stateless);
        DQ_TRY(x->ctx.init(n, 1, 0));
        DQ_TRY(x->ldr.alloc(3, n, 1)); DQ_TRY(dev_alloc(x->mats, 4L * n * n)); DQ_TRY(dev_alloc(x->logdet, 1));
        it = g_ctx.emplace(n, std::move(x)).first;
    }
    *out = it->second.get();
    return hipSetDevice(0) == hipSuccess ? 0 : DQMC_ENODEVICE;
}
static int upload_ldr(Stateless* x, int k, const double* L, const double* d, const double* R, LdrRef* out) {
    const Ctx& c = x->ctx;
    *out = x->ldr.at(k); *out->tri = false;
    DQ_HIP(hipMemcpyAsync(out->L.p, L, sizeof(double) * c.nn, hipMemcpyHostToDevice, c.stream));
    DQ_HIP(hipMemcpyAsync(out->R.p, R, sizeof(double) * c.nn, hipMemcpyHostToDevice, c.stream));
    DQ_HIP(hipMemcpyAsync(out->d.p, d, sizeof(double) * c.n, hipMemcpyHostToDevice, c.stream));
    return 0;
}
static int download_ldr(Ctx* c, LdrRef f, double* L, double* d, double* R) {
    DQ_HIP(hipMemcpyAsync(L, f.L.p, sizeof(double) * c->nn, hipMemcpyDeviceToHost, c->stream));
    DQ_HIP(hipMemcpyAsync(R, f.R.p, sizeof(double) * c->nn, hipMemcpyDeviceToHost, c->stream));
    DQ_HIP(hipMemcpyAsync(d, f.d.p, sizeof(double) * c->n, hipMemcpyDeviceToHost, c->stream));
    DQ_HIP(hipStreamSynchronize(c->stream));
    return take_status(*c);
}

}

using namespace dq;

struct dqmc_engine { Engine e; };

#define ENGINE_CALL(h) if (!(h)) { set_error("null engine"); return DQMC_EINVAL; } Engine& e = (h)->e; DQ_HIP(hipSetDevice(e.device))

namespace dq {
int engine_fields_view(dqmc_engine* h, EngineFieldsView* v) {
    if (!h || !v) { set_error("null engine"); return DQMC_EINVAL; }
    Engine& e = h->e;
    v->device = e.device; v->n = e.n; v->nt = e.nt; v->n_chains = e.C; v->fields = e.fields.get(); v->stream = e.s;
    return 0;
}
int engine_fields_changed(dqmc_engine* h) {
    ENGINE_CALL(h);
    e.stack_valid = false; e.gt_valid = false;
    return launch_build_expv(e.fields.get(), (long)e.nt * e.n, e.nt, e.n, e.tab8.get(), e.expv.get(), e.invexpv.get(), (long)e.nt * e.n, e.C, e.s);
}
int engine_exchange_scratch(dqmc_engine* h, int8_t** saved, int8_t** recv, int** tab) {
    ENGINE_CALL(h);
    if (!e.xch.tab) {
        Engine::Exchange x; DQ_TRY(dev_alloc(x.saved, (size_t)e.C * e.nt * e.n)); DQ_TRY(dev_alloc(x.recv, (size_t)2 * e.nt * e.n)); DQ_TRY(dev_alloc(x.tab, (size_t)2 * e.C));
        e.xch = std::move(x);
    }
    *saved = e.xch.saved.get(); *recv = e.xch.recv.get(); *tab = e.xch.tab.get();
    return 0;
}
}

#define API_LOCK std::lock_guard<std::mutex> _lk(g_ctx_mu)

extern "C" {

const char* dqmc_last_error(void) { return get_error(); }
const char* dqmc_backend(void) { return "hip:gfx950"; }
int dqmc_device_count(void) { int c = 0; if (hipGetDeviceCount(&c) != hipSuccess) return 0; return c; }

int dqmc_to_ldr(int n, const double* M, double* L, double* d, double* R) {
    API_LOCK; Stateless* x; DQ_TRY(get_ctx(n, &x)); Ctx* c = &x->ctx;
    if (!M || !L || !d || !R) { set_error("null pointer"); return DQMC_EINVAL; }
    DQ_HIP(hipMemcpyAsync(x->M(0).p, M, sizeof(double) * c->nn, hipMemcpyHostToDevice, c->stream));
    LdrRef out = x->ldr.at(0);
    DQ_TRY(c->to_ldr(x->M(0), out));
    return download_ldr(c, out, L, d, R);
}
int dqmc_ldr_mul_mat(int n, const double* L, const double* d, const double* R, const double* M, double* Lo, double* d_o, double* Ro) {
    API_LOCK; Stateless* x; DQ_TRY(get_ctx(n, &x)); Ctx* c = &x->ctx;
    LdrRef F; DQ_TRY(upload_ldr(x, 0, L, d, R, &F));
    DQ_HIP(hipMemcpyAsync(x->M(0).p, M, sizeof(double) * c->nn, hipMemcpyHostToDevice, c->stream));
    LdrRef out = x->ldr.at(2);
    DQ_TRY(c->ldr_mul_mat(F, x->M(0), out));
    return download_ldr(c, out, Lo, d_o, Ro);
}
int dqmc_mat_mul_ldr(int n, const double* M, const double* L, const double* d, const double* R, double* Lo, double* d_o, double* Ro) {
    API_LOCK; Stateless* x; DQ_TRY(get_ctx(n, &x)); Ctx* c = &x->ctx;
    LdrRef F; DQ_TRY(upload_ldr(x, 0, L, d, R, &F));
    DQ_HIP(hipMemcpyAsync(x->M(0).p, M, sizeof(double) * c->nn, hipMemcpyHostToDevice, c->stream));
    LdrRef out = x->ldr.at(2);
    DQ_TRY(c->mat_mul_ldr(x->M(0), F, out));
    return download_ldr(c, out, Lo, d_o, Ro);
}
int dqmc_ldr_mul_ldr(int n, const double* L1, const double* d1, const double* R1, const double* L2, const double* d2, const double* R2, double* Lo, double* d_o, double* Ro) {
    API_LOCK; Stateless* x; DQ_TRY(get_ctx(n, &x)); Ctx* c = &x->ctx;
    LdrRef F1, F2; DQ_TRY(upload_ldr(x, 0, L1, d1, R1, &F1)); DQ_TRY(upload_ldr(x, 1, L2, d2, R2, &F2));
    LdrRef out = x->ldr.at(2);
    DQ_TRY(c->ldr_mul_ldr(F1, F2, out));
    return download_ldr(c, out, Lo, d_o, Ro);
}
int dqmc_inv_I_plus_ldr(int n, const double* L, const double* d, const double* R, double* G, double* logdet) {
    API_LOCK; Stateless* x; DQ_TRY(get_ctx(n, &x)); Ctx* c = &x->ctx;
    LdrRef F; DQ_TRY(upload_ldr(x, 0, L, d, R, &F));
    DQ_TRY(c->inv_I_plus_ldr(F, x->M(1), x->logdet.get()));
    DQ_HIP(hipMemcpyAsync(G, x->M(1).p, sizeof(double) * c->nn, hipMemcpyDeviceToHost, c->stream));
    double ld = 0.0;
    DQ_HIP(hipMemcpyAsync(&ld, x->logdet.get(), sizeof(double), hipMemcpyDeviceToHost, c->stream));
    DQ_HIP(hipStreamSynchronize(c->stream));
    if (logdet) *logdet = ld;
    return take_status(*c);
}
int dqmc_inv_I_plus_ldr_mul_ldr(int n, const double* L1, const double* d1, const double* R1, const double* L2, const double* d2, const double* R2, double* G) {
    API_LOCK; Stateless* x; DQ_TRY(get_ctx(n, &x)); Ctx* c = &x->ctx;
    LdrRef F1, F2; DQ_TRY(upload_ldr(x, 0, L1, d1, R1, &F1)); DQ_TRY(upload_ldr(x, 1, L2, d2, R2, &F2));
    DQ_TRY(c->inv_I_plus_ldr_mul_ldr(F1, F2, x->M(1)));
    DQ_HIP(hipMemcpyAsync(G, x->M(1).p, sizeof(double) * c->nn, hipMemcpyDeviceToHost, c->stream));
    DQ_HIP(hipStreamSynchronize(c->stream));
    return take_status(*c);
}
int dqmc_gemm(int n, const double* A, int transA, const double* B, int transB, double* Cm) {
    API_LOCK; Stateless* x; DQ_TRY(get_ctx(n, &x)); Ctx* c = &x->ctx;
    DQ_HIP(hipMemcpyAsync(x->M(0).p, A, sizeof(double) * c->nn, hipMemcpyHostToDevice, c->stream));
    DQ_HIP(hipMemcpyAsync(x->M(1).p, B, sizeof(double) * c->nn, hipMemcpyHostToDevice, c->stream));
    CMat Bm = x->M(1);
    if (transB) { DQ_TRY(launch_transpose_scale(x->M(1), x->M(2), CVec(), n, 1, c->stream)); Bm = x->M(2); }
    DQ_TRY(c->gemm(x->M(0), Bm, x->M(3), CVec(), CVec(), CVec(), transA ? 1 : 0));
    DQ_HIP(hipMemcpyAsync(Cm, x->M(3).p, sizeof(double) * c->nn, hipMemcpyDeviceToHost, c->stream));
    DQ_HIP(hipStreamSynchronize(c->stream));
    return 0;
}
int dqmc_rank1_update(int n, double* G, int i, double delta) {
    API_LOCK; Stateless* x; DQ_TRY(get_ctx(n, &x)); Ctx* c = &x->ctx;
    if (i < 0 || i >= n) { set_error("site index out of range"); return DQMC_ERANGE; }
    DQ_HIP(hipMemcpyAsync(x->M(0).p, G, sizeof(double) * c->nn, hipMemcpyHostToDevice, c->stream));
    DQ_TRY(launch_rank1(x->M(0), i, delta, x->M(1).p, 2L * n + 1, n, 1, c->stream));
    DQ_HIP(hipMemcpyAsync(G, x->M(0).p, sizeof(double) * c->nn, hipMemcpyDeviceToHost, c->stream));
    DQ_HIP(hipStreamSynchronize(c->stream));
    return 0;
}

int dqmc_create_batch(dqmc_engine** out, int device, int n_chains, int n_sites, int nt, int n_stab, const double* g,
                      const double gamma[4], const double eta[4], const double* expK, const double* invexpK) {
    if (!out || n_chains <= 0 || n_sites <= 0 || nt <= 0 || n_stab <= 0 || !g || !gamma || !eta || !expK || !invexpK) { set_error("bad argument"); return DQMC_EINVAL; }
    if (n_sites > 1024) { set_error("n_sites > 1024 is not supported by the single-workgroup kernels"); return DQMC_EINVAL; }
    int count = 0;
    if (hipGetDeviceCount(&count) != hipSuccess || count == 0) { set_error("no HIP device available: this library requires a gfx950 GPU"); return DQMC_ENODEVICE; }
    if (device < 0 || device >= count) { set_error("device ordinal out of range"); return DQMC_EINVAL; }
    dqmc_engine* h = new (std::nothrow) dqmc_engine;
    if (!h) return DQMC_ENOMEM;
    int rc = h->e.create(device, n_chains, n_sites, nt, n_stab, g, gamma, eta, expK, invexpK);
    if (rc) { delete h; return rc; }
    *out = h; return 0;
}
int dqmc_create(dqmc_engine** out, int device, int n_sites, int nt, int n_stab, double g, const double gamma[4], const double eta[4],
                const double* expK, const double* invexpK) {
    return dqmc_create_batch(out, device, 1, n_sites, nt, n_stab, &g, gamma, eta, expK, invexpK);
}
int dqmc_set_checkerboard(dqmc_engine* h, int n_groups, const int32_t* bonds, const int32_t* group_sizes, const double* cosh_t, const double* sinh_t,
                          const double* diag_factor) {
    ENGINE_CALL(h);
    return e.set_checkerboard(n_groups, bonds, group_sizes, cosh_t, sinh_t, diag_factor);
}
void dqmc_destroy(dqmc_engine* h) { if (h) { (void)hipSetDevice(h->e.device); delete h; } }
int dqmc_n_chains(dqmc_engine* h) { return h ? h->e.C : 0; }

int dqmc_set_fields(dqmc_engine* h, const int64_t* f) {
    ENGINE_CALL(h);
    std::vector<int8_t> tmp((size_t)e.C * e.nt * e.n);
    for (int c = 0; c < e.C; ++c) for (int i = 0; i < e.n; ++i) for (int l = 0; l < e.nt; ++l) {
        const int64_t v = f[(size_t)c * e.nt * e.n + l + (size_t)e.nt * i];
        if (v < 0 || v > 3) { set_error("field value outside {0,1,2,3}"); return DQMC_EINVAL; }
        tmp[(size_t)c * e.nt * e.n + (size_t)l * e.n + i] = (int8_t)v;
    }
    DQ_HIP(hipStreamSynchronize(e.s));
    DQ_HIP(hipMemcpy(e.fields.get(), tmp.data(), tmp.size(), hipMemcpyHostToDevice));
    DQ_TRY(launch_build_expv(e.fields.get(), (long)e.nt * e.n, e.nt, e.n, e.tab8.get(), e.expv.get(), e.invexpv.get(), (long)e.nt * e.n, e.C, e.s));
    DQ_HIP(hipStreamSynchronize(e.s));
    return 0;
}
int dqmc_get_fields(dqmc_engine* h, int64_t* f) {
    ENGINE_CALL(h);
    DQ_TRY(e.sync_and_check());
    std::vector<int8_t> tmp; DQ_TRY(e.download_fields(tmp));
    std::copy(tmp.begin(), tmp.end(), f);
    return 0;
}
int dqmc_init(dqmc_engine* h) { ENGINE_CALL(h); DQ_TRY(e.init()); return e.sync_and_check(); }
int dqmc_get_G(dqmc_engine* h, double* G) {
    ENGINE_CALL(h); DQ_TRY(e.sync_and_check());
    DQ_HIP(hipMemcpy(G, e.G.get(), sizeof(double) * e.C * e.nn, hipMemcpyDeviceToHost)); return 0;
}
int dqmc_set_G(dqmc_engine* h, const double* G) {
    ENGINE_CALL(h); DQ_HIP(hipStreamSynchronize(e.s));
    DQ_HIP(hipMemcpy(e.G.get(), G, sizeof(double) * e.C * e.nn, hipMemcpyHostToDevice)); e.gt_valid = false; return 0;
}
int dqmc_get_logdet(dqmc_engine* h, double* ld) {
    ENGINE_CALL(h); DQ_TRY(e.sync_and_check());
    DQ_HIP(hipMemcpy(ld, e.logdet.get(), sizeof(double) * e.C, hipMemcpyDeviceToHost)); return 0;
}
int dqmc_n_stack(dqmc_engine* h) { return h ? h->e.n_stack : 0; }
int dqmc_get_stack(dqmc_engine* h, int i, double* L, double* d, double* R) {
    ENGINE_CALL(h);
    if (i < 0 || i >= e.n_stack) { set_error("LDR Stack index out of bounds"); return DQMC_ERANGE; }
    if (!e.stack_valid) { set_error("stack not initialised: call dqmc_init first"); return DQMC_EINVAL; }
    DQ_TRY(e.sync_and_check());
    LdrRef f = e.stack.at(i);
    DQ_HIP(hipMemcpy(L, f.L.p, sizeof(double) * e.C * e.nn, hipMemcpyDeviceToHost));
    DQ_HIP(hipMemcpy(R, f.R.p, sizeof(double) * e.C * e.nn, hipMemcpyDeviceToHost));
    DQ_HIP(hipMemcpy(d, f.d.p, sizeof(double) * e.C * e.n, hipMemcpyDeviceToHost));
    return 0;
}
int dqmc_sweep_0_to_beta(dqmc_engine* h, const int32_t* perm, const uint8_t* kprop, const double* u) {
    ENGINE_CALL(h);
    if (!e.stack_valid) { set_error("dqmc_init must be called before sweeping"); return DQMC_EINVAL; }
    DQ_TRY(e.upload_stream(perm, kprop, u)); return e.sweep_fwd();
}
int dqmc_sweep_beta_to_0(dqmc_engine* h, const int32_t* perm, const uint8_t* kprop, const double* u) {
    ENGINE_CALL(h);
    if (!e.stack_valid) { set_error("dqmc_init must be called before sweeping"); return DQMC_EINVAL; }
    DQ_TRY(e.upload_stream(perm, kprop, u)); return e.sweep_bwd();
}
int dqmc_sync(dqmc_engine* h) { ENGINE_CALL(h); return e.sync_and_check(); }
int dqmc_get_stats(dqmc_engine* h, dqmc_stats* out) {
    ENGINE_CALL(h); DQ_TRY(e.sync_and_check());
    static_assert(sizeof(DevStats) == sizeof(dqmc_stats), "stats layout");
    DQ_HIP(hipMemcpy(out, e.dstats.get(), sizeof(DevStats) * e.C, hipMemcpyDeviceToHost)); return 0;
}
int dqmc_wrap_forward(dqmc_engine* h, int l) {
    ENGINE_CALL(h);
    if (l < 0 || l >= e.nt) { set_error("time slice out of range"); return DQMC_ERANGE; }
    return e.wrap_forward(l);
}
int dqmc_wrap_backward(dqmc_engine* h, int l) {
    ENGINE_CALL(h);
    if (l < 0 || l >= e.nt) { set_error("time slice out of range"); return DQMC_ERANGE; }
    return e.wrap_backward(l);
}
int dqmc_local_update_slice(dqmc_engine* h, int l, const int32_t* perm, const uint8_t* kprop, const double* u, int* accepted) {
    ENGINE_CALL(h);
    if (l < 0 || l >= e.nt) { set_error("time slice out of range"); return DQMC_ERANGE; }
    DQ_TRY(e.check_stream("local_update_slice", perm, kprop, u, e.C));
    DQ_HIP(hipStreamSynchronize(e.s));
    for (int c = 0; c < e.C; ++c) {
        const size_t off = ((size_t)c * e.nt + l) * e.n;
        DQ_HIP(hipMemcpy(e.rs_perm.get() + off, perm + (size_t)c * e.n, sizeof(int32_t) * e.n, hipMemcpyHostToDevice));
        DQ_HIP(hipMemcpy(e.rs_k.get() + off, kprop + (size_t)c * e.n, e.n, hipMemcpyHostToDevice));
        DQ_HIP(hipMemcpy(e.rs_u.get() + off, u + (size_t)c * e.n, sizeof(double) * e.n, hipMemcpyHostToDevice));
    }
    DQ_TRY(e.local_update(l));
    DQ_TRY(launch_fold_stats(e.dstats.get(), e.acc.get() + l, e.nt, 1, e.err.get(), e.n_stack, 0, e.n, e.nt, e.C, e.s));
    DQ_TRY(e.sync_and_check());
    if (accepted) for (int c = 0; c < e.C; ++c) DQ_HIP(hipMemcpy(accepted + c, e.acc.get() + (size_t)c * e.nt + l, sizeof(int), hipMemcpyDeviceToHost));
    return 0;
}
int dqmc_calculate_Bbar(dqmc_engine* h, int is, double* out) {
    ENGINE_CALL(h);
    if (is < 0 || is >= e.n_stack) { set_error("stack index out of range"); return DQMC_ERANGE; }
    Mat bb; DQ_TRY(e.Bbar(is, &bb)); DQ_HIP(hipStreamSynchronize(e.s));
    DQ_HIP(hipMemcpy(out, bb.p, sizeof(double) * e.C * e.nn, hipMemcpyDeviceToHost)); return 0;
}
int dqmc_global_action(dqmc_engine* h, double* S) {
    ENGINE_CALL(h); DQ_TRY(e.sync_and_check());
    std::vector<int8_t> tmp; std::vector<double> ld(e.C);
    DQ_TRY(e.download_fields(tmp));
    DQ_HIP(hipMemcpy(ld.data(), e.logdet.get(), sizeof(double) * e.C, hipMemcpyDeviceToHost));
    const double alpha = -1.0;
    const size_t per = (size_t)e.nt * e.n;
    for (int c = 0; c < e.C; ++c) {
        double lb = 0.0, lg = 0.0;
        for (size_t k = 0; k < per; ++k) {
            const int f = tmp[c * per + k];
            lb += alpha * e.g_host[c] * e.eta_host[f]; lg += std::log(e.gamma_host[f]);
        }
        S[c] = -2.0 * ld[c] - (lb + lg);
    }
    return 0;
}
int dqmc_sweep_unequal_time(dqmc_engine* h) {
    ENGINE_CALL(h);
    if (!e.stack_valid) { set_error("sweep_unequal_time: call dqmc_init first"); return DQMC_EINVAL; }
    return e.sweep_unequal();
}
int dqmc_get_G_tau(dqmc_engine* h, int which, int l, double* out) {
    ENGINE_CALL(h);
    if (which < 0 || which > 2 || l < 0 || l > e.nt) { set_error("get_G_tau: which in 0..2, l in 0..nt"); return DQMC_ERANGE; }
    if (!e.ut_valid) { set_error("get_G_tau: run dqmc_sweep_unequal_time first"); return DQMC_EINVAL; }
    DQ_TRY(e.sync_and_check());
    DQ_HIP(hipMemcpy(out, e.utm(which, l).p, sizeof(double) * e.C * e.nn, hipMemcpyDeviceToHost));
    return 0;
}
int dqmc_half_warp(dqmc_engine* h, const double* expK_half, const double* invexpK_half, int which, int l, double* out) {
    ENGINE_CALL(h);
    if (!out) { set_error("half_warp: out is NULL"); return DQMC_EINVAL; }
    if (which < -1 || which > 2 || (which >= 0 && (l < 0 || l > e.nt))) { set_error("half_warp: which in -1..2, l in 0..nt"); return DQMC_ERANGE; }
    if (which >= 0 && !e.ut_valid) { set_error("half_warp: run dqmc_sweep_unequal_time first"); return DQMC_EINVAL; }
    if ((expK_half == nullptr) != (invexpK_half == nullptr)) { set_error("half_warp: pass both half-step matrices or neither"); return DQMC_EINVAL; }
    if (expK_half) {
        if (!e.hw.out) { Engine::HalfWarp x; DQ_TRY(dev_alloc(x.expK, e.nn)); DQ_TRY(dev_alloc(x.invexpK, e.nn)); DQ_TRY(dev_alloc(x.out, (size_t)e.C * e.nn)); e.hw = std::move(x); }
        DQ_HIP(hipStreamSynchronize(e.s));
        DQ_HIP(hipMemcpy(e.hw.expK.get(), expK_half, sizeof(double) * e.nn, hipMemcpyHostToDevice));
        DQ_HIP(hipMemcpy(e.hw.invexpK.get(), invexpK_half, sizeof(double) * e.nn, hipMemcpyHostToDevice));
    } else if (!e.hw.out) { set_error("half_warp: no half-step matrices uploaded yet"); return DQMC_EINVAL; }
    const CMat M = which < 0 ? CMat(e.mG()) : CMat(e.utm(which, l));
    DQ_TRY(e.ctx.gemm(CMat(e.hw.invexpK.get(), 0), M, e.ctx.T(0)));
    DQ_TRY(e.ctx.gemm(e.ctx.T(0), CMat(e.hw.expK.get(), 0), Mat{e.hw.out.get(), e.nn}));
    DQ_TRY(e.sync_and_check());
    DQ_HIP(hipMemcpy(out, e.hw.out.get(), sizeof(double) * e.C * e.nn, hipMemcpyDeviceToHost));
    return 0;
}
int dqmc_measure_unequal_time(dqmc_engine* h, int L1, int L2, int accumulate, double* out) {
    ENGINE_CALL(h);
    if (L1 < 1 || L2 < 1 || L1 * L2 != e.n) { set_error("measure_unequal_time: L1*L2 must equal n_sites"); return DQMC_EINVAL; }
    if (!e.ut_valid) { set_error("measure_unequal_time: run dqmc_sweep_unequal_time first"); return DQMC_EINVAL; }
    const long stride = 3L * (e.nt + 1) * e.n;
    if (accumulate) {
        DQ_TRY(launch_measure_unequal_time(e.ut.G[0].get(), e.ut.G[1].get(), e.ut.G[2].get(), e.ut.meas_sum.get(), stride, L1, L2, e.nt, 1, e.C, e.s));
        ++e.ut_meas_count; return 0;
    }
    if (!out) { set_error("measure_unequal_time: out is NULL"); return DQMC_EINVAL; }
    DQ_TRY(launch_measure_unequal_time(e.ut.G[0].get(), e.ut.G[1].get(), e.ut.G[2].get(), e.ut.meas_now.get(), stride, L1, L2, e.nt, 0, e.C, e.s));
    DQ_TRY(e.sync_and_check());
    DQ_HIP(hipMemcpy(out, e.ut.meas_now.get(), sizeof(double) * e.C * stride, hipMemcpyDeviceToHost));
    return 0;
}
int dqmc_measure_unequal_fetch(dqmc_engine* h, double* out_sum, int64_t* n_measurements, int reset) {
    ENGINE_CALL(h); DQ_TRY(e.sync_and_check());
    if (!e.ut.meas_sum) { set_error("measure_unequal_fetch: nothing measured yet"); return DQMC_EINVAL; }
    const size_t cnt = (size_t)e.C * 3 * (e.nt + 1) * e.n;
    if (out_sum) DQ_HIP(hipMemcpy(out_sum, e.ut.meas_sum.get(), sizeof(double) * cnt, hipMemcpyDeviceToHost));
    if (n_measurements) *n_measurements = e.ut_meas_count;
    if (reset) { DQ_HIP(hipMemset(e.ut.meas_sum.get(), 0, sizeof(double) * cnt)); e.ut_meas_count = 0; }
    return 0;
}
int dqmc_measure_equal_time(dqmc_engine* h, int L1, int L2, double* scalars, double* chi_r) {
    ENGINE_CALL(h);
    if (L1 < 1 || L2 < 1 || L1 * L2 != e.n) { set_error("measure_equal_time: L1*L2 must equal n_sites"); return DQMC_EINVAL; }
    DQ_TRY(launch_measure_equal_time(CMat(e.G.get(), e.nn), e.meas_now.get(), 3 + e.n, L1, L2, 0, e.C, e.s));
    DQ_TRY(e.sync_and_check());
    return e.copy_out_equal_time(e.meas_now.get(), scalars, chi_r);
}
int dqmc_measure_accumulate(dqmc_engine* h, int L1, int L2) {
    ENGINE_CALL(h);
    if (L1 < 1 || L2 < 1 || L1 * L2 != e.n) { set_error("measure_accumulate: L1*L2 must equal n_sites"); return DQMC_EINVAL; }
    DQ_TRY(launch_measure_equal_time(CMat(e.G.get(), e.nn), e.meas_sum.get(), 3 + e.n, L1, L2, 1, e.C, e.s));
    ++e.meas_count;
    return 0;
}
int dqmc_measure_fetch(dqmc_engine* h, double* scalars_sum, double* chi_r_sum, int64_t* n_measurements, int reset) {
    ENGINE_CALL(h); DQ_TRY(e.sync_and_check());
    DQ_TRY(e.copy_out_equal_time(e.meas_sum.get(), scalars_sum, chi_r_sum));
    if (n_measurements) *n_measurements = e.meas_count;
    if (reset) { DQ_HIP(hipMemset(e.meas_sum.get(), 0, sizeof(double) * e.C * (3 + e.n))); e.meas_count = 0; }
    return 0;
}
int dqmc_update_kernel_time(dqmc_engine* h, double* ms, int64_t* n_launches, int64_t* n_accepted) {
    ENGINE_CALL(h); DQ_TRY(e.sync_and_check());
    std::vector<DevStats> st(e.C);
    DQ_HIP(hipMemcpy(st.data(), e.dstats.get(), sizeof(DevStats) * e.C, hipMemcpyDeviceToHost));
    long long acc = 0; for (auto& x : st) acc += x.n_accepted;
    if (ms) *ms = e.upd_ms; if (n_launches) *n_launches = e.upd_launches; if (n_accepted) *n_accepted = acc - e.upd_accept_base;
    e.upd_ms = 0.0; e.upd_launches = 0; e.upd_accept_base = acc;
    return 0;
}
int dqmc_debug_snapshot(dqmc_engine* h, double* wrap_err, int* accepted, unsigned int* sync_words, unsigned int* slice_epoch) {
    ENGINE_CALL(h);
    DQ_HIP(hipStreamSynchronize(e.s));
    if (wrap_err) DQ_HIP(hipMemcpy(wrap_err, e.err.get(), sizeof(double) * e.n_stack, hipMemcpyDeviceToHost));
    if (accepted) DQ_HIP(hipMemcpy(accepted, e.acc.get(), sizeof(int) * e.nt, hipMemcpyDeviceToHost));
    if (sync_words) DQ_HIP(hipMemcpy(sync_words, e.slice_sync.get(), sizeof(unsigned int) * 80, hipMemcpyDeviceToHost));
    if (slice_epoch) *slice_epoch = e.slice_epoch;
    return 0;
}
int dqmc_slice_path(dqmc_engine* h) {
    if (!h) return -1;
    Engine& e = h->e;
    if (!is_persistent(e.slice_path)) return 0;
    unsigned solo = 0;
    for (int c = 0; c < e.C && !solo; ++c) {
        SliceSync hs; if (hipMemcpy(&hs, e.slice_sync.get() + (size_t)c * SLICE_SYNC_BYTES, 64, hipMemcpyDeviceToHost) != hipSuccess) break;
        solo = hs.solo_count;
    }
    return solo ? 2 : 1;
}
int dqmc_set_profiling(dqmc_engine* h, int on) {
    ENGINE_CALL(h); DQ_TRY(e.sync_and_check());
    e.profiling = on != 0; return 0;
}

}
```

dqmc_amd/csrc/qr.hip:

```cpp
#include "common.h"
#include "wave.h"
#include <cstdlib>

namespace dq {


template <int NR>
__global__ __launch_bounds__(1024) void qrcp_kernel(Mat Am, QrWork w, int n) {
    extern __shared__ __attribute__((aligned(16))) unsigned char smem[];
    double* vn1 = reinterpret_cast<double*>(smem);
    double* vn2 = vn1 + n;
    double* v = vn2 + n;
    double* candcol = v + n;
    double* cand_v = candcol + 16 * (size_t)n;
    double* red = cand_v + 16;
    int* cand_i = reinterpret_cast<int*>(red + 16);
    int* pivpos = cand_i + 16;
    const int chain = blockIdx.y;
    double* __restrict__ A = Am.at(chain);
    double* tau = w.tau + (long)chain * w.tau_stride;
    int* jpvt = w.jpvt + (long)chain * w.jpvt_stride;
    const int t = threadIdx.x, lane = t & 63, wave = t >> 6;
    const double tol3z = 1.0536712127723509e-08;
    constexpr int QR_CB = NR <= 2 ? 8 : (NR <= 4 ? 4 : (NR <= 9 ? 2 : 1));

    {
        double bestn = -1.0; int besti = -1; double bcol[NR];
#pragma unroll
        for (int q = 0; q < NR; ++q) bcol[q] = 0.0;
        for (int c = wave; c < n; c += 16) {
            double a[NR]; double s = 0.0;
#pragma unroll
            for (int q = 0; q < NR; ++q) { const int r = lane + 64 * q; a[q] = (r < n) ? A[r + (long)n * c] : 0.0; s += a[q] * a[q]; }
            s = wave_sum(s);
            const double nn = sqrt(s);
            if (lane == 0) { vn1[c] = nn; vn2[c] = nn; pivpos[c] = -1; }
            if (nn > bestn) {
                bestn = nn; besti = c;
#pragma unroll
                for (int q = 0; q < NR; ++q) bcol[q] = a[q];
            }
        }
        if (lane == 0) { cand_v[wave] = bestn; cand_i[wave] = besti; }
#pragma unroll
        for (int q = 0; q < NR; ++q) { const int r = lane + 64 * q; if (r < n) candcol[(size_t)wave * n + r] = bcol[q]; }
    }
    __syncthreads();

    for (int i = 0; i < n; ++i) {
        double best = cand_v[0]; int bw = 0; int p = cand_i[0];
#pragma unroll
        for (int k = 1; k < 16; ++k) {
            const double ob = cand_v[k]; const int oi = cand_i[k];
            if (oi >= 0 && (p < 0 || ob > best || (ob == best && oi < p))) { best = ob; bw = k; p = oi; }
        }
        const double x = (t >= i && t < n) ? candcol[(size_t)bw * n + t] : 0.0;
        double ss = (t > i) ? x * x : 0.0;
        ss = wave_sum(ss);
        if (lane == 0) red[wave] = ss;
        __syncthreads();
        double xnorm2 = 0.0;
#pragma unroll
        for (int k = 0; k < 16; ++k) xnorm2 += red[k];
        const double al = candcol[(size_t)bw * n + i];
        double tau_i = 0.0, beta = al, scale = 0.0;
        if (xnorm2 != 0.0) {
            beta = -copysign(sqrt(al * al + xnorm2), al);
            tau_i = (beta - al) / beta;
            scale = 1.0 / (al - beta);
        }
        if (t < n) {
            double vr = 0.0;
            if (t == i) { vr = 1.0; A[t + (long)n * p] = beta; }
            else if (t > i) { vr = x * scale; A[t + (long)n * p] = vr; }
            v[t] = vr;
        }
        if (t == 0) { tau[i] = tau_i; jpvt[i] = p; pivpos[p] = i; }
        __syncthreads();
        double vr[NR];
#pragma unroll
        for (int q = 0; q < NR; ++q) { const int r = lane + 64 * q; vr[q] = (r < n) ? v[r] : 0.0; }
        double bestn = -1.0; int besti = -1; double bcol[NR];
#pragma unroll
        for (int q = 0; q < NR; ++q) bcol[q] = 0.0;
        for (int cb = wave; cb < n; cb += 16 * QR_CB) {
            double a[QR_CB][NR]; bool live[QR_CB];
#pragma unroll
            for (int k = 0; k < QR_CB; ++k) {
                const int c = cb + 16 * k;
                live[k] = c < n && pivpos[c] < 0;
#pragma unroll
                for (int q = 0; q < NR; ++q) { const int r = lane + 64 * q; a[k][q] = (live[k] && r >= i && r < n) ? A[r + (long)n * c] : 0.0; }
            }
#pragma unroll
            for (int k = 0; k < QR_CB; ++k) {
                if (!live[k]) continue;
                const int c = cb + 16 * k;
                double s = 0.0;
#pragma unroll
                for (int q = 0; q < NR; ++q) s += a[k][q] * vr[q];
                s = wave_sum(s) * tau_i;
                double tail = 0.0, ai_q = 0.0;
#pragma unroll
                for (int q = 0; q < NR; ++q) {
                    const int r = lane + 64 * q;
                    if (r >= i && r < n) {
                        a[k][q] -= s * vr[q];
                        if (tau_i != 0.0) A[r + (long)n * c] = a[k][q];
                        if (r > i) tail += a[k][q] * a[k][q];
                    }
                    if (q == (i >> 6)) ai_q = a[k][q];
                }
                const double aic = readlane_f64(ai_q, i & 63);
                double n1 = vn1[c];
                if (n1 != 0.0) {
                    double temp = fabs(aic) / n1; temp = fmax(0.0, 1.0 - temp * temp);
                    const double rr = n1 / vn2[c];
                    const double temp2 = temp * rr * rr;
                    if (temp2 <= tol3z) {
                        tail = wave_sum(tail);
                        n1 = (i + 1 < n) ? sqrt(tail) : 0.0;
                        if (lane == 0) { vn1[c] = n1; vn2[c] = n1; }
                    } else {
                        n1 = n1 * sqrt(temp);
                        if (lane == 0) vn1[c] = n1;
                    }
                }
                if (n1 > bestn || besti < 0) {
                    bestn = n1; besti = c;
#pragma unroll
                    for (int q = 0; q < NR; ++q) bcol[q] = a[k][q];
                }
            }
        }
        if (lane == 0) { cand_v[wave] = bestn; cand_i[wave] = besti; }
        if (besti >= 0) {
#pragma unroll
            for (int q = 0; q < NR; ++q) { const int r = lane + 64 * q; if (r < n) candcol[(size_t)wave * n + r] = bcol[q]; }
        }
        __syncthreads();
    }
}

template <int NRR>
__global__ __launch_bounds__(256) void formq_kernel(CMat Am, const double* tau_p, long tau_stride, const int* jpvt_p, long jpvt_stride, Mat Qm, int n) {
    const int chain = blockIdx.y;
    const double* __restrict__ A = Am.at(chain);
    const double* __restrict__ tau = tau_p + (long)chain * tau_stride;
    const int* __restrict__ jpvt = jpvt_p + (long)chain * jpvt_stride;
    double* __restrict__ Q = Qm.at(chain);
    const int lane = threadIdx.x & 63, wave = threadIdx.x >> 6;
    const int rg = lane & 15, cq = lane >> 4;
    const int c = blockIdx.x * 16 + wave * 4 + cq;
    const int cw_max = min(blockIdx.x * 16 + wave * 4 + 3, n - 1);
    const bool wave_idle = blockIdx.x * 16 + wave * 4 >= n;
    double q[NRR];
#pragma unroll
    for (int j = 0; j < NRR; ++j) q[j] = (16 * j + rg == c) ? 1.0 : 0.0;
    __shared__ int s_jpvt[1024];
    __shared__ double s_tau[1024];
    for (int k = threadIdx.x; k < n; k += blockDim.x) { s_jpvt[k] = jpvt[k]; s_tau[k] = tau[k]; }
    __syncthreads();
    if (wave_idle) return;
    constexpr int PD = 3;
    double vq[PD][NRR]; double tq[PD];
    auto fetch = [&](int slot, int ii) {
        const int ic = ii > 0 ? ii : 0;
        const long cb = (long)n * s_jpvt[ic]; tq[slot] = s_tau[ic];
#pragma unroll
        for (int j = 0; j < NRR; ++j) vq[slot][j] = A[min(16 * j + rg, n - 1) + cb];
    };
    auto apply = [&](int slot, int i) {
        const double ti = tq[slot];
        if (ti == 0.0) return;
        double v[NRR];
#pragma unroll
        for (int j = 0; j < NRR; ++j) { const int r = 16 * j + rg; v[j] = (r > i && r < n) ? vq[slot][j] : (r == i ? 1.0 : 0.0); }
        double s = 0.0;
#pragma unroll
        for (int j = 0; j < NRR; ++j) s += v[j] * q[j];
        s = row16_sum(s) * ti;
        if (c < i) s = 0.0;
#pragma unroll
        for (int j = 0; j < NRR; ++j) q[j] -= s * v[j];
    };
    fetch(0, cw_max); fetch(1, cw_max - 1); fetch(2, cw_max - 2);
    int i = cw_max;
    for (; i >= 2; i -= 3) {
        apply(0, i);     fetch(0, i - 3);
        apply(1, i - 1); fetch(1, i - 4);
        apply(2, i - 2); fetch(2, i - 5);
    }
    if (i >= 0) apply(0, i);
    if (i >= 1) apply(1, i - 1);
    if (c < n) {
#pragma unroll
        for (int j = 0; j < NRR; ++j) { const int r = 16 * j + rg; if (r < n) Q[r + (long)n * c] = q[j]; }
    }
}

template <int NRR, int M>
struct FormQBlock {
    static constexpr int J0 = M > 0 ? M - 1 : 0;
    static __device__ __forceinline__ void fetch(double (&v)[NRR], double& t, const double* __restrict__ A, const int* s_jpvt, const double* s_tau,
                                                 int n, int rg, int ii) {
        const int ic = ii > 0 ? ii : 0;
        const long cb = (long)n * s_jpvt[ic]; t = s_tau[ic];
#pragma unroll
        for (int j = J0; j < NRR; ++j) v[j] = A[16 * j + rg + cb];
    }
    static __device__ __forceinline__ void apply(double (&q)[NRR], const double (&v)[NRR], double ti, int c, int i, int rg) {
        if (ti == 0.0) return;
        const int rm = 16 * M + rg;
        const double vm = (rm > i) ? v[M] : (rm == i ? 1.0 : 0.0);
        double s0 = vm * q[M], s1 = 0.0;
#pragma unroll
        for (int j = M + 1; j < NRR; ++j) { if ((j - M) & 1) s1 = fma(v[j], q[j], s1); else s0 = fma(v[j], q[j], s0); }
        double s = row16_sum(s0 + s1) * ti;
        if (c < i) s = 0.0;
        q[M] = fma(-s, vm, q[M]);
#pragma unroll
        for (int j = M + 1; j < NRR; ++j) q[j] = fma(-s, v[j], q[j]);
    }
    static __device__ __forceinline__ void run(double (&q)[NRR], double (&vq)[4][NRR], double (&tq)[4], const double* __restrict__ A, const int* s_jpvt,
                                               const double* s_tau, int n, int rg, int c, int cw_max) {
        const int mtop = cw_max >> 4;
        if (M <= mtop) {
            const int hi = M == mtop ? cw_max : 16 * M + 15;
            if (M == mtop) {
#pragma unroll
                for (int e = 0; e < 4; ++e) fetch(vq[e], tq[e], A, s_jpvt, s_tau, n, rg, hi - e);
            }
            for (int top = hi; top >= 16 * M; top -= 4) {
#pragma unroll
                for (int e = 0; e < 4; ++e) {
                    apply(q, vq[e], tq[e], c, top - e, rg);
                    fetch(vq[e], tq[e], A, s_jpvt, s_tau, n, rg, top - e - 4);
                }
            }
        }
        FormQBlock<NRR, M - 1>::run(q, vq, tq, A, s_jpvt, s_tau, n, rg, c, cw_max);
    }
};
template <int NRR>
struct FormQBlock<NRR, -1> {
    static __device__ __forceinline__ void run(double (&)[NRR], double (&)[4][NRR], double (&)[4], const double*, const int*, const double*, int, int, int, int) {}
};
template <int NRR>
__global__ __launch_bounds__(256) void formq_blocked_kernel(CMat Am, const double* tau_p, long tau_stride, const int* jpvt_p, long jpvt_stride, Mat Qm, int n) {
    const int chain = blockIdx.y;
    const double* __restrict__ A = Am.at(chain);
    const double* __restrict__ tau = tau_p + (long)chain * tau_stride;
    const int* __restrict__ jpvt = jpvt_p + (long)chain * jpvt_stride;
    double* __restrict__ Q = Qm.at(chain);
    const int lane = threadIdx.x & 63, wave = threadIdx.x >> 6;
    const int rg = lane & 15, cq = lane >> 4;
    const int c = blockIdx.x * 16 + wave * 4 + cq;
    const int cw_max = blockIdx.x * 16 + wave * 4 + 3;
    __shared__ int s_jpvt[16 * NRR];
    __shared__ double s_tau[16 * NRR];
    for (int k = threadIdx.x; k < n; k += blockDim.x) { s_jpvt[k] = jpvt[k]; s_tau[k] = tau[k]; }
    __syncthreads();
    double q[NRR];
#pragma unroll
    for (int j = 0; j < NRR; ++j) q[j] = (16 * j + rg == c) ? 1.0 : 0.0;
    double vq[4][NRR]; double tq[4];
#pragma unroll
    for (int e = 0; e < 4; ++e) {
        tq[e] = 0.0;
#pragma unroll
        for (int j = 0; j < NRR; ++j) vq[e][j] = 0.0;
    }
    FormQBlock<NRR, NRR - 1>::run(q, vq, tq, A, s_jpvt, s_tau, n, rg, c, cw_max);
#pragma unroll
    for (int j = 0; j < NRR; ++j) { const int r = 16 * j + rg; if (r < n) Q[r + (long)n * c] = q[j]; }
}

static bool formq_blocked_ok(int n) {
    return (n == 16 || n == 32 || n == 64 || n == 128 || n == 256 || n == 576);
}
static void launch_formq_blocked(CMat A, const QrWork& w, Mat L, int n, int n_chains, hipStream_t s) {
    const dim3 grid(n / 16, n_chains), block(256);
#define DQ_FQ(NRR) hipLaunchKernelGGL((formq_blocked_kernel<NRR>), grid, block, 0, s, A, (const double*)w.tau, w.tau_stride, (const int*)w.jpvt, w.jpvt_stride, L, n)
    if (n <= 16) DQ_FQ(1); else if (n <= 32) DQ_FQ(2); else if (n <= 64) DQ_FQ(4); else if (n <= 128) DQ_FQ(8); else if (n <= 256) DQ_FQ(16); else DQ_FQ(36);
#undef DQ_FQ
}

__global__ void assemble_r_kernel(CMat Am, const int* jpvt_p, long jpvt_stride, Vec dv, Mat Rm, int n) {
    const int chain = blockIdx.y;
    const double* __restrict__ A = Am.at(chain);
    const int* jpvt = jpvt_p + (long)chain * jpvt_stride;
    double* __restrict__ R = Rm.at(chain);
    double* d = dv.at(chain);
    const int j = blockIdx.x;
    const int col = jpvt[j];
    for (int r = threadIdx.x; r < n; r += blockDim.x) {
        double val = 0.0;
        if (r <= j) val = A[r + (long)n * col] / fabs(A[r + (long)n * jpvt[r]]);
        R[r + (long)n * col] = val;
    }
    if (threadIdx.x == 0) d[j] = fabs(A[j + (long)n * col]);
}

int qr_init_device() {
    DQ_HIP(hipFuncSetAttribute(reinterpret_cast<const void*>(qrcp_kernel<1>), hipFuncAttributeMaxDynamicSharedMemorySize, 160 * 1024));
    DQ_HIP(hipFuncSetAttribute(reinterpret_cast<const void*>(qrcp_kernel<2>), hipFuncAttributeMaxDynamicSharedMemorySize, 160 * 1024));
    DQ_HIP(hipFuncSetAttribute(reinterpret_cast<const void*>(qrcp_kernel<4>), hipFuncAttributeMaxDynamicSharedMemorySize, 160 * 1024));
    DQ_HIP(hipFuncSetAttribute(reinterpret_cast<const void*>(qrcp_kernel<9>), hipFuncAttributeMaxDynamicSharedMemorySize, 160 * 1024));
    DQ_HIP(hipFuncSetAttribute(reinterpret_cast<const void*>(qrcp_kernel<16>), hipFuncAttributeMaxDynamicSharedMemorySize, 160 * 1024));
    return 0;
}

int launch_qrcp_coop(Mat A, QrWork w, int n, int n_chains, hipStream_t s);
int launch_qrcp_colown(Mat A, QrWork w, int n, int n_chains, hipStream_t s);

static int launch_assemble_r(Mat A, Vec d, Mat R, const QrWork& w, int n, int n_chains, hipStream_t s) {
    hipLaunchKernelGGL(assemble_r_kernel, dim3(n, n_chains), dim3(128), 0, s, CMat(A), (const int*)w.jpvt, w.jpvt_stride, d, R, n);
    DQ_HIP(hipGetLastError());
    return 0;
}
static int formq_assemble(Mat A, Mat L, Vec d, Mat R, const QrWork& w, int n, int n_chains, hipStream_t s) {
    if (formq_blocked_ok(n)) launch_formq_blocked(CMat(A), w, L, n, n_chains, s);
    else if (n <= 256) hipLaunchKernelGGL((formq_kernel<16>), dim3((n + 15) / 16, n_chains), dim3(256), 0, s, CMat(A), (const double*)w.tau, w.tau_stride,
                                          (const int*)w.jpvt, w.jpvt_stride, L, n);
    else if (n <= 576) hipLaunchKernelGGL((formq_kernel<36>), dim3((n + 15) / 16, n_chains), dim3(256), 0, s, CMat(A), (const double*)w.tau, w.tau_stride,
                                          (const int*)w.jpvt, w.jpvt_stride, L, n);
    else hipLaunchKernelGGL((formq_kernel<64>), dim3((n + 15) / 16, n_chains), dim3(256), 0, s, CMat(A), (const double*)w.tau, w.tau_stride,
                            (const int*)w.jpvt, w.jpvt_stride, L, n);
    return launch_assemble_r(A, d, R, w, n, n_chains, s);
}
static int to_ldr_panel(Mat A, Mat L, Vec d, Mat R, const QrWork& w, int n, int n_chains, hipStream_t s) {
    DQ_TRY(launch_qr_panel(A, w, n, n_chains, s));
    DQ_TRY(launch_qr_panel_formq(w, L, n, n_chains, s));
    return launch_assemble_r(A, d, R, w, n, n_chains, s);
}
template <int NR>
static int to_ldr_streaming(Mat A, Mat L, Vec d, Mat R, const QrWork& w, int n, int n_chains, hipStream_t s) {
    const size_t lds = sizeof(double) * ((size_t)3 * n + (size_t)16 * n + 32) + sizeof(int) * (16 + (size_t)n) + 64;
    hipLaunchKernelGGL((qrcp_kernel<NR>), dim3(1, n_chains), dim3(1024), lds, s, A, w, n);
    hipLaunchKernelGGL((formq_kernel<4 * NR>), dim3((n + 15) / 16, n_chains), dim3(256), 0, s, CMat(A), (const double*)w.tau, w.tau_stride,
                       (const int*)w.jpvt, w.jpvt_stride, L, n);
    return launch_assemble_r(A, d, R, w, n, n_chains, s);
}

int launch_to_ldr(QrFamily f, Mat A, Mat L, Vec d, Mat R, QrWork w, int n, int n_chains, hipStream_t s) {
    if (n > 1024) { set_error("to_LDR kernel supports n <= 1024"); return -1; }
    switch (f) {
    case QrFamily::Panel: return to_ldr_panel(A, L, d, R, w, n, n_chains, s);
    case QrFamily::ColumnOwner:
        if (n > 256) break;
        DQ_TRY(launch_qrcp_colown(A, w, n, n_chains, s));
        return formq_assemble(A, L, d, R, w, n, n_chains, s);
    case QrFamily::Cooperative:
        DQ_TRY(launch_qrcp_coop(A, w, n, n_chains, s));
        return formq_assemble(A, L, d, R, w, n, n_chains, s);
    case QrFamily::Streaming:
        if (n <= 64) return to_ldr_streaming<1>(A, L, d, R, w, n, n_chains, s);
        if (n <= 128) return to_ldr_streaming<2>(A, L, d, R, w, n, n_chains, s);
        if (n <= 256) return to_ldr_streaming<4>(A, L, d, R, w, n, n_chains, s);
        if (n <= 576) return to_ldr_streaming<9>(A, L, d, R, w, n, n_chains, s);
        return to_ldr_streaming<16>(A, L, d, R, w, n, n_chains, s);
    }
    set_error("to_LDR: kernel family not available at this n");
    return -1;
}

}
```

dqmc_amd/csrc/qr_panel.hip:

```cpp
#include "common.h"
#include "wave.h"
#include <utility>

namespace dq {

namespace {

#ifdef DQ_QP_STAMPS
#define QST(i) { unsigned long long t_; asm volatile("s_memtime %0\n\ts_waitcnt lgkmcnt(0)" : "=s"(t_) :: "memory"); if (threadIdx.x == 0) qst[i] = t_; }
#else
#define QST(i)
#endif

constexpr int QP_B = 16;
constexpr int QP_SR = 32;
#ifndef QP_SEL_ROWS
#define QP_SEL_ROWS 32
#endif
constexpr int QP_SEL = QP_SEL_ROWS;
typedef double d4 __attribute__((ext_vector_type(4)));

__device__ __forceinline__ unsigned qp_row_bits(unsigned r) {
    unsigned h = r * 0x9E3779B1u + 0x85EBCA77u;
    h ^= h >> 16; h *= 0x85EBCA6Bu; h ^= h >> 13; h *= 0xC2B2AE35u; h ^= h >> 16;
    return h;
}
__device__ __forceinline__ double qp_sign(unsigned bits, int i) {
    return __hiloint2double((int)(0x3FF00000u | (((bits >> i) & 1u) << 31)), 0);
}

__device__ __forceinline__ double rows4_sum(double x) {
    const unsigned lo = (unsigned)__double_as_longlong(x), hi = (unsigned)(__double_as_longlong(x) >> 32);
    auto l16 = __builtin_amdgcn_permlane16_swap(lo, lo, false, false);
    auto h16 = __builtin_amdgcn_permlane16_swap(hi, hi, false, false);
    const double e = __hiloint2double((int)h16[0], (int)l16[0]), o = __hiloint2double((int)h16[1], (int)l16[1]);
    const double s = e + o;
    const unsigned slo = (unsigned)__double_as_longlong(s), shi = (unsigned)(__double_as_longlong(s) >> 32);
    auto l32 = __builtin_amdgcn_permlane32_swap(slo, slo, false, false);
    auto h32 = __builtin_amdgcn_permlane32_swap(shi, shi, false, false);
    return __hiloint2double((int)h32[0], (int)l32[0]) + __hiloint2double((int)h32[1], (int)l32[1]);
}

template <int J>
__device__ __forceinline__ void dpp_fmac_self(double& d, double a) {
    asm volatile("v_fmac_f64_dpp %0, %1, %1 row_newbcast:%2 row_mask:0xf bank_mask:0xf" : "+v"(d) : "v"(a), "n"(J));
}
template <int J>
__device__ __forceinline__ void dpp_axpy_self(double& a, double m) {
    asm volatile("v_fmac_f64_dpp %0, %0, %1 row_newbcast:%2 row_mask:0xf bank_mask:0xf" : "+v"(a) : "v"(m), "n"(J));
}
__device__ __forceinline__ void dpp_fence(double (&a)[16]) {
    asm volatile("s_nop 1" : "+v"(a[0]), "+v"(a[1]), "+v"(a[2]), "+v"(a[3]), "+v"(a[4]), "+v"(a[5]), "+v"(a[6]), "+v"(a[7]),
                             "+v"(a[8]), "+v"(a[9]), "+v"(a[10]), "+v"(a[11]), "+v"(a[12]), "+v"(a[13]), "+v"(a[14]), "+v"(a[15]));
}

__device__ __forceinline__ void dpp_fence1(double& z) { asm volatile("s_nop 1" : "+v"(z)); }
template <int T>
__device__ __forceinline__ void dpp_fmac(double& d, double z, double y) {
    asm volatile("v_fmac_f64_dpp %0, %1, %2 row_newbcast:%3 row_mask:0xf bank_mask:0xf" : "+v"(d) : "v"(z), "v"(y), "n"(T));
}
template <int... Ts>
__device__ __forceinline__ void t_row_dot(double& tj, const double (&trow)[16], double z, std::integer_sequence<int, Ts...>) {
    (dpp_fmac<Ts>(tj, z, trow[Ts]), ...);
}

template <int NW>
struct PanelShared {
    static constexpr int NWP = NW < 2 ? 2 : NW;
    alignas(16) unsigned long long key[2][NWP];
    alignas(16) double cand[2][QP_SEL + 2];
    alignas(16) double part[2][QP_B][NWP];
    alignas(16) double prow[2][QP_B];
    int sel[QP_B];
};

template <int NEWTON>
__device__ __forceinline__ void householder(double alpha, double tail2, double& beta, double& tau, double& scale) {
    const double s = fma(alpha, alpha, tail2);
    double r = __builtin_amdgcn_rsq(s);
    const double h = 0.5 * s;
#pragma unroll
    for (int it = 0; it < NEWTON; ++it) r = r * fma(-h * r, r, 1.5);
    double sq = s * r;
    if (NEWTON > 1) sq = fma(0.5 * r, fma(-sq, sq, s), sq);
    const double b = -copysign(sq, alpha);
    const double d = alpha - b;
    double id = __builtin_amdgcn_rcp(d);
#pragma unroll
    for (int it = 0; it < NEWTON; ++it) id = id * fma(-d, id, 2.0);
    const bool none = tail2 == 0.0;
    beta = none ? alpha : b;
    tau = none ? 0.0 : d * copysign(r, alpha);
    scale = none ? 0.0 : id;
}

__device__ __forceinline__ void lds_barrier() {
    asm volatile("s_waitcnt lgkmcnt(0)" ::: "memory");
    __builtin_amdgcn_s_barrier();
    asm volatile("" ::: "memory");
}

template <int J, int NW, int CPL>
__device__ __forceinline__ void select_step(double (&y)[CPL][QP_SEL], unsigned& live, int t, int lane, int wave, PanelShared<NW>& sh) {
    constexpr int par = J & 1;
    unsigned long long key = 0ULL; int bq = 0; double btail = 0.0;
#pragma unroll
    for (int q = 0; q < CPL; ++q) {
        double tl[4] = {0.0, 0.0, 0.0, 0.0};
#pragma unroll
        for (int i = J + 1; i < QP_SEL; ++i) tl[i & 3] = fma(y[q][i], y[q][i], tl[i & 3]);
        const double tail = (tl[0] + tl[1]) + (tl[2] + tl[3]);
        const double nrm2 = fma(y[q][J], y[q][J], tail);
        const unsigned long long kq = ((live >> q) & 1u) ? (((unsigned long long)__double_as_longlong(nrm2) & ~0x7FFULL) | (unsigned long long)(1024 - (t + 64 * NW * q))) : 0ULL;
        if (kq > key) { key = kq; bq = q; btail = tail; }
    }
    const unsigned long long wmax = wave_max_u64(key);
    const bool cand_ = wmax != 0ULL && key == wmax;
    if (cand_) sh.key[par][wave] = wmax;
    if (wmax == 0ULL && lane == 0) sh.key[par][wave] = 0ULL;
    lds_barrier();
    unsigned long long best = sh.key[par][0]; int ww = 0;
#pragma unroll
    for (int q = 1; q < NW; ++q) { const unsigned long long o = sh.key[par][q]; if (o > best) { best = o; ww = q; } }
    if (cand_ && wave == ww) {
#pragma unroll
        for (int q = 0; q < CPL; ++q) {
            if (bq == q) {
#pragma unroll
                for (int i = J & ~1; i < QP_SEL; i += 2) *reinterpret_cast<double2*>(&sh.cand[par][i]) = double2{y[q][i], y[q][i + 1]};
            }
        }
        sh.cand[par][QP_SEL] = btail;
    }
    lds_barrier();
    const int pcol = 1024 - (int)(best & 0x7FFULL);
    const double* xs = sh.cand[par];
    double x[QP_SEL];
#pragma unroll
    for (int i = J & ~1; i < QP_SEL; i += 2) { const double2 v = *reinterpret_cast<const double2*>(&xs[i]); x[i] = v.x; x[i + 1] = v.y; }
    double beta, tau, scale;
    householder<1>(x[J], xs[QP_SEL], beta, tau, scale);
    const double st = -scale * tau;
#pragma unroll
    for (int q = 0; q < CPL; ++q) {
        double dt[4] = {0.0, 0.0, 0.0, 0.0};
#pragma unroll
        for (int i = J + 1; i < QP_SEL; ++i) dt[i & 3] = fma(x[i], y[q][i], dt[i & 3]);
        const double dot = (dt[0] + dt[1]) + (dt[2] + dt[3]);
        const double cf = st * fma(scale, dot, y[q][J]);
#pragma unroll
        for (int i = J + 1; i < QP_SEL; ++i) y[q][i] = fma(x[i], cf, y[q][i]);
        if (t + 64 * NW * q == pcol) live &= ~(1u << q);
    }
    if (lane == 0 && wave == 0) sh.sel[J] = pcol;
}

template <int J, int NW, int CPL>
__device__ __forceinline__ void panel_step(double (&a)[CPL][16], double (&trow)[QP_B], double& myscale, unsigned diag, unsigned blk_live, int c, int g, int wave,
                                           PanelShared<NW>& sh, double* tau_out) {
    constexpr int par = J & 1;
    if (blk_live) {
        double acc = 0.0;
#pragma unroll
        for (int b = 0; b < CPL; ++b) {
            if ((blk_live >> b) & 1u) {
                double dlo0 = 0.0, dlo1 = 0.0, dhi0 = 0.0, dhi1 = 0.0;
#pragma unroll
                for (int i = 0; i < 16; ++i) {
                    if (i <= J) { if (i & 1) dpp_fmac_self<J>(dlo1, a[b][i]); else dpp_fmac_self<J>(dlo0, a[b][i]); }
                    else { if (i & 1) dpp_fmac_self<J>(dhi1, a[b][i]); else dpp_fmac_self<J>(dhi0, a[b][i]); }
                }
                acc += (dhi0 + dhi1) + (((diag >> b) & 1u) ? 0.0 : dlo0 + dlo1);
                if ((diag >> b) & 1u) sh.prow[par][c] = a[b][J];
            }
        }
        const double part = rows4_sum(acc);
        if (g == 0) sh.part[par][c][wave] = part;
    } else if (g == 0) sh.part[par][c][wave] = 0.0;
    lds_barrier();
    double s_c = sh.part[par][c][0], s_j = sh.part[par][J][0];
#pragma unroll
    for (int q = 1; q < NW; ++q) { s_c += sh.part[par][c][q]; s_j += sh.part[par][J][q]; }
    const double alpha = sh.prow[par][J], apc = sh.prow[par][c];
    double beta, tau, scale;
    householder<2>(alpha, s_j, beta, tau, scale);
    const double zc = fma(scale, s_c, apc);
    if (c == J) myscale = scale;
    if (blk_live) {
        const double mcf = c > J ? -scale * tau * zc : 0.0;
#pragma unroll
        for (int b = 0; b < CPL; ++b) {
            if ((blk_live >> b) & 1u) {
                const bool isd = (diag >> b) & 1u;
                const double mlo = isd ? 0.0 : mcf;
#pragma unroll
                for (int i = 0; i < 16; ++i) {
                    if (i <= J) dpp_axpy_self<J>(a[b][i], mlo);
                    else dpp_axpy_self<J>(a[b][i], mcf);
                }
                const double newd = c > J ? fma(-tau, zc, a[b][J]) : beta;
                a[b][J] = (isd && c >= J) ? newd : a[b][J];
                dpp_fence(a[b]);
            }
        }
    }
    if (wave == 0) {
        double zt = myscale * zc;
        double tj = 0.0;
        dpp_fence1(zt);
        t_row_dot(tj, trow, zt, std::make_integer_sequence<int, J>{});
        trow[J] = c < J ? -tau * tj : (c == J ? tau : 0.0);
        if (g == 0 && c == J) tau_out[J] = tau;
    }
}

}

template <int NW, int CPL>
__global__ __launch_bounds__(64 * NW) void qp_panel_kernel(Mat Am, QrWork w, int n, int k) {
    __shared__ PanelShared<NW> sh;
    const int chain = blockIdx.y;
    double* __restrict__ A = Am.at(chain);
    double* __restrict__ pw = w.pw + (long)chain * w.pw_stride;
    const double* __restrict__ Y = pw;
    double* __restrict__ Vp = pw + (long)QP_SR * n + (long)n * k;
    double* __restrict__ Tm = pw + (long)QP_SR * n + (long)n * n + (long)QP_B * k;
    double* __restrict__ VTp = pw + (long)QP_SR * n + (long)n * n + (long)QP_B * n + (long)n * k;
    int* __restrict__ pivpos = w.pivpos + (long)chain * w.pivpos_stride;
    double* tau = w.tau + (long)chain * w.tau_stride;
    int* jpvt = w.jpvt + (long)chain * w.jpvt_stride;
    const int t = threadIdx.x, lane = t & 63, wave = t >> 6;

#ifdef DQ_QP_STAMPS
    __shared__ unsigned long long qst[40];
#endif
    QST(0)
    {
        unsigned live = 0u;
        double y[CPL][QP_SEL]; int pp[CPL];
#pragma unroll
        for (int q = 0; q < CPL; ++q) {
            const int col = t + 64 * NW * q, cc = col < n ? col : n - 1;
#pragma unroll
            for (int i = 0; i < QP_SEL; ++i) y[q][i] = Y[(long)i * n + cc];
            pp[q] = pivpos[cc];
        }
#pragma unroll
        for (int q = 0; q < CPL; ++q) {
            const int col = t + 64 * NW * q;
            if (col < n && pp[q] < 0) live |= 1u << q;
            if (col >= n) {
#pragma unroll
                for (int i = 0; i < QP_SEL; ++i) y[q][i] = 0.0;
            }
        }
        if (y[0][0] == 1.2345e300) live = 0u;
        QST(1)
#define QP_SEL_STEP(J) select_step<J, NW, CPL>(y, live, t, lane, wave, sh); QST(2 + J)
        QP_SEL_STEP(0) QP_SEL_STEP(1) QP_SEL_STEP(2) QP_SEL_STEP(3) QP_SEL_STEP(4) QP_SEL_STEP(5) QP_SEL_STEP(6) QP_SEL_STEP(7)
        QP_SEL_STEP(8) QP_SEL_STEP(9) QP_SEL_STEP(10) QP_SEL_STEP(11) QP_SEL_STEP(12) QP_SEL_STEP(13) QP_SEL_STEP(14) QP_SEL_STEP(15)
#undef QP_SEL_STEP
    }
    lds_barrier();
    const int c = lane & 15, g = lane >> 4;
    const int mycol = sh.sel[c];
    double a[CPL][16], trow[QP_B], myscale = 0.0;
    unsigned diag = 0u, blk_live = 0u;
#pragma unroll
    for (int b = 0; b < CPL; ++b) {
        const int r0 = 64 * NW * b + 64 * wave + 16 * g;
        if (r0 == k) diag |= 1u << b;
        if (64 * NW * b + 64 * wave + 64 > k && 64 * NW * b + 64 * wave < n) blk_live |= 1u << b;
        const double2* src = reinterpret_cast<const double2*>(A + (long)n * mycol + r0);
        const bool rows_live = r0 >= k && r0 < n;
#pragma unroll
        for (int i = 0; i < 16; i += 2) { const double2 v = rows_live ? src[i >> 1] : double2{0.0, 0.0}; a[b][i] = v.x; a[b][i + 1] = v.y; }
        dpp_fence(a[b]);
    }
#pragma unroll
    for (int i = 0; i < QP_B; ++i) trow[i] = 0.0;
    double* tau_out = tau + k;
#ifdef DQ_QP_STAMPS
    if (a[0][0] == 1.2345e300) myscale = 1.0;
#endif
    QST(18)
#define QP_PAN(J) panel_step<J, NW, CPL>(a, trow, myscale, diag, blk_live, c, g, wave, sh, tau_out); QST(19 + J)
    QP_PAN(0) QP_PAN(1) QP_PAN(2) QP_PAN(3) QP_PAN(4) QP_PAN(5) QP_PAN(6) QP_PAN(7)
    QP_PAN(8) QP_PAN(9) QP_PAN(10) QP_PAN(11) QP_PAN(12) QP_PAN(13) QP_PAN(14) QP_PAN(15)
#undef QP_PAN
#pragma unroll
    for (int b = 0; b < CPL; ++b) {
        const int r0 = 64 * NW * b + 64 * wave + 16 * g;
        if (r0 >= k && r0 < n) {
            const bool isd = (diag >> b) & 1u;
            double2* dst = reinterpret_cast<double2*>(A + (long)n * mycol + r0);
            double2* vdst = reinterpret_cast<double2*>(Vp + (long)n * c + r0);
            double v[16], vc[16];
#pragma unroll
            for (int i = 0; i < 16; ++i) {
                const bool below = !isd || i > c;
                v[i] = below ? a[b][i] * myscale : a[b][i];
                vc[i] = below ? v[i] : (i == c ? 1.0 : 0.0);
                VTp[(long)QP_B * (r0 + i) + c] = vc[i];
            }
#pragma unroll
            for (int i = 0; i < 16; i += 2) { dst[i >> 1] = double2{v[i], v[i + 1]}; vdst[i >> 1] = double2{vc[i], vc[i + 1]}; }
        }
    }
    if (wave == 0 && g == 0) {
#pragma unroll
        for (int i = 0; i < QP_B; ++i) Tm[c + QP_B * i] = trow[i];
        jpvt[k + c] = mycol;
        pivpos[mycol] = k + c;
    }
#ifdef DQ_QP_STAMPS
    asm volatile("s_waitcnt vmcnt(0)" ::: "memory");
    QST(35)
    __syncthreads();
    if (t == 0 && k == 0 && blockIdx.y == 0) {
        printf("panel k=0 n=%d (100 MHz ticks x 24 = clk @2.4GHz): load Y %llu | sel steps", n, qst[1] - qst[0]);
        for (int j = 0; j < 16; ++j) printf(" %llu", qst[2 + j] - qst[1 + j]);
        printf(" | gather %llu | panel steps", qst[18] - qst[17]);
        for (int j = 0; j < 16; ++j) printf(" %llu", qst[19 + j] - qst[18 + j]);
        printf(" | write-out %llu | total %llu\n", qst[35] - qst[34], qst[35] - qst[0]);
    }
#endif
}

constexpr int QP_UW = 8;
template <bool UPDATE, int TPW>
__global__ __launch_bounds__(64 * QP_UW) void qp_update_kernel(Mat Am, QrWork w, int n, int k) {
    constexpr int YT = QP_SR / 16;
    __shared__ double red[QP_UW][YT * 4][64];
    const int chain = blockIdx.y;
    double* __restrict__ A = Am.at(chain);
    double* __restrict__ pw = w.pw + (long)chain * w.pw_stride;
    double* __restrict__ Y = pw;
    const double* __restrict__ Vp = pw + (long)QP_SR * n + (long)n * k;
    const double* __restrict__ Tm = pw + (long)QP_SR * n + (long)n * n + (long)QP_B * k;
    const double* __restrict__ VTp = pw + (long)QP_SR * n + (long)n * n + (long)QP_B * n + (long)n * k;
    int* __restrict__ pivpos = w.pivpos + (long)chain * w.pivpos_stride;
    const int t = threadIdx.x, lane = t & 63, wave = t >> 6;
    const int r16 = lane & 15, kk = lane >> 4;
    const int col = 16 * blockIdx.x + r16;
    double* __restrict__ Ac = A + (long)n * col;
    const int m_tiles = (n - k) / 16;
    int pp = -1;
    if (UPDATE) pp = pivpos[col];
    d4 At[TPW]; double v1[TPW][4], v2[TPW][4], tv[4];
#pragma unroll
    for (int ti = 0; ti < TPW; ++ti) {
        const int rt = wave + QP_UW * ti;
        At[ti] = d4{0.0, 0.0, 0.0, 0.0};
#pragma unroll
        for (int s = 0; s < 4; ++s) { v1[ti][s] = 0.0; v2[ti][s] = 0.0; }
        if (rt < m_tiles) {
            const int r0 = k + 16 * rt;
#pragma unroll
            for (int r = 0; r < 4; ++r) At[ti][r] = Ac[r0 + kk + 4 * r];
            if (UPDATE) {
#pragma unroll
                for (int s = 0; s < 4; ++s) { v1[ti][s] = VTp[(long)QP_B * (r0 + kk + 4 * s) + r16]; v2[ti][s] = Vp[(long)n * (kk + 4 * s) + (r0 + r16)]; }
            }
        }
    }
    if (UPDATE) {
#pragma unroll
        for (int s = 0; s < 4; ++s) tv[s] = Tm[(kk + 4 * s) + QP_B * r16];
    }
    const bool live_col = pp < 0;
    if (UPDATE) { if (__ballot(live_col) == 0ULL) return; }
    else if (t < 16) pivpos[col] = -1;
    d4 wp = {0.0, 0.0, 0.0, 0.0};
    if (UPDATE) {
        d4 acc = {0.0, 0.0, 0.0, 0.0};
#pragma unroll
        for (int ti = 0; ti < TPW; ++ti) {
#pragma unroll
            for (int s = 0; s < 4; ++s) acc = __builtin_amdgcn_mfma_f64_16x16x4f64(v1[ti][s], At[ti][s], acc, 0, 0, 0);
        }
#pragma unroll
        for (int r = 0; r < 4; ++r) red[wave][r][lane] = acc[r];
        __syncthreads();
        d4 W;
#pragma unroll
        for (int r = 0; r < 4; ++r) {
            double v = red[0][r][lane];
#pragma unroll
            for (int q = 1; q < QP_UW; ++q) v += red[q][r][lane];
            W[r] = live_col ? v : 0.0;
        }
#pragma unroll
        for (int s = 0; s < 4; ++s) wp = __builtin_amdgcn_mfma_f64_16x16x4f64(tv[s], W[s], wp, 0, 0, 0);
        wp = -wp;
        __syncthreads();
    }
    d4 ya[YT];
#pragma unroll
    for (int yt = 0; yt < YT; ++yt) ya[yt] = d4{0.0, 0.0, 0.0, 0.0};
#pragma unroll
    for (int ti = 0; ti < TPW; ++ti) {
        const int rt = wave + QP_UW * ti;
        if (rt < m_tiles) {
            const int r0 = k + 16 * rt;
            if (UPDATE) {
#pragma unroll
                for (int s = 0; s < 4; ++s) At[ti] = __builtin_amdgcn_mfma_f64_16x16x4f64(v2[ti][s], wp[s], At[ti], 0, 0, 0);
                if (live_col) {
#pragma unroll
                    for (int r = 0; r < 4; ++r) Ac[r0 + kk + 4 * r] = At[ti][r];
                }
            }
            if (!UPDATE || rt >= 1) {
#pragma unroll
                for (int s = 0; s < 4; ++s) {
                    const unsigned bits = qp_row_bits((unsigned)(r0 + kk + 4 * s));
#pragma unroll
                    for (int yt = 0; yt < YT; ++yt) ya[yt] = __builtin_amdgcn_mfma_f64_16x16x4f64(qp_sign(bits, 16 * yt + r16), At[ti][s], ya[yt], 0, 0, 0);
                }
            }
        }
    }
#pragma unroll
    for (int yt = 0; yt < YT; ++yt)
#pragma unroll
        for (int r = 0; r < 4; ++r) red[wave][4 * yt + r][lane] = ya[yt][r];
    __syncthreads();
    for (int idx = t; idx < YT * 4 * 64; idx += 64 * QP_UW) {
        const int l = idx & 63, q = idx >> 6, yt = q >> 2, r = q & 3;
        double v = red[0][q][l];
#pragma unroll
        for (int qq = 1; qq < QP_UW; ++qq) v += red[qq][q][l];
        Y[(long)(16 * yt + (l >> 4) + 4 * r) * n + 16 * blockIdx.x + (l & 15)] = v;
    }
}

template <int TPW>
__global__ __launch_bounds__(64 * QP_UW) void qp_formq_kernel(QrWork w, Mat Lm, int n) {
    __shared__ double red[QP_UW][4][64];
    const int chain = blockIdx.y;
    const double* __restrict__ pw = w.pw + (long)chain * w.pw_stride;
    const double* __restrict__ Vall = pw + (long)QP_SR * n;
    const double* __restrict__ Tall = Vall + (long)n * n;
    const double* __restrict__ VTall = Tall + (long)QP_B * n;
    double* __restrict__ L = Lm.at(chain);
    const int t = threadIdx.x, lane = t & 63, wave = t >> 6;
    const int r16 = lane & 15, kk = lane >> 4;
    const int cb = blockIdx.x, col = 16 * cb + r16;
    const int n_tiles = n / 16;
    d4 Qt[TPW];
#pragma unroll
    for (int ti = 0; ti < TPW; ++ti) {
        const int rt = wave + QP_UW * ti;
#pragma unroll
        for (int r = 0; r < 4; ++r) Qt[ti][r] = (16 * rt + kk + 4 * r == col) ? 1.0 : 0.0;
    }
    double v1[TPW][4], v2[TPW][4], tv[4], n1[TPW][4], n2[TPW][4], nt_[4];
    auto load = [&](int k, double (&a1)[TPW][4], double (&a2)[TPW][4], double (&at)[4]) {
        const double* Vp = Vall + (long)n * 16 * k;
        const double* Tm = Tall + (long)QP_B * 16 * k;
        const double* VTp = VTall + (long)n * 16 * k;
#pragma unroll
        for (int s = 0; s < 4; ++s) at[s] = Tm[r16 + QP_B * (kk + 4 * s)];
#pragma unroll
        for (int ti = 0; ti < TPW; ++ti) {
            const int rt = wave + QP_UW * ti;
            const bool in = rt < n_tiles && rt >= k;
#pragma unroll
            for (int s = 0; s < 4; ++s) {
                a1[ti][s] = in ? VTp[(long)QP_B * (16 * rt + kk + 4 * s) + r16] : 0.0;
                a2[ti][s] = in ? Vp[(long)n * (kk + 4 * s) + (16 * rt + r16)] : 0.0;
            }
        }
    };
    load(cb, v1, v2, tv);
    for (int k = cb; k >= 0; --k) {
        if (k > 0) load(k - 1, n1, n2, nt_);
        d4 acc = {0.0, 0.0, 0.0, 0.0};
#pragma unroll
        for (int ti = 0; ti < TPW; ++ti)
#pragma unroll
            for (int s = 0; s < 4; ++s) acc = __builtin_amdgcn_mfma_f64_16x16x4f64(v1[ti][s], Qt[ti][s], acc, 0, 0, 0);
#pragma unroll
        for (int r = 0; r < 4; ++r) red[wave][r][lane] = acc[r];
        __syncthreads();
        d4 W;
#pragma unroll
        for (int r = 0; r < 4; ++r) {
            double v = red[0][r][lane];
#pragma unroll
            for (int q = 1; q < QP_UW; ++q) v += red[q][r][lane];
            W[r] = v;
        }
        d4 wp = {0.0, 0.0, 0.0, 0.0};
#pragma unroll
        for (int s = 0; s < 4; ++s) wp = __builtin_amdgcn_mfma_f64_16x16x4f64(tv[s], W[s], wp, 0, 0, 0);
        wp = -wp;
#pragma unroll
        for (int ti = 0; ti < TPW; ++ti)
#pragma unroll
            for (int s = 0; s < 4; ++s) Qt[ti] = __builtin_amdgcn_mfma_f64_16x16x4f64(v2[ti][s], wp[s], Qt[ti], 0, 0, 0);
        __syncthreads();
#pragma unroll
        for (int ti = 0; ti < TPW; ++ti)
#pragma unroll
            for (int s = 0; s < 4; ++s) { v1[ti][s] = n1[ti][s]; v2[ti][s] = n2[ti][s]; }
#pragma unroll
        for (int s = 0; s < 4; ++s) tv[s] = nt_[s];
    }
#pragma unroll
    for (int ti = 0; ti < TPW; ++ti) {
        const int rt = wave + QP_UW * ti;
        if (rt < n_tiles) {
#pragma unroll
            for (int r = 0; r < 4; ++r) L[(long)n * col + 16 * rt + kk + 4 * r] = Qt[ti][r];
        }
    }
}

int launch_qr_panel_formq(QrWork w, Mat L, int n, int n_chains, hipStream_t s) {
    const dim3 grid(n / 16, n_chains);
    const int tpw = (n / 16 + QP_UW - 1) / QP_UW;
    if (tpw <= 2) hipLaunchKernelGGL((qp_formq_kernel<2>), grid, dim3(64 * QP_UW), 0, s, w, L, n);
    else if (tpw <= 5) hipLaunchKernelGGL((qp_formq_kernel<5>), grid, dim3(64 * QP_UW), 0, s, w, L, n);
    else hipLaunchKernelGGL((qp_formq_kernel<8>), grid, dim3(64 * QP_UW), 0, s, w, L, n);
    DQ_HIP(hipGetLastError());
    return 0;
}

static bool qr_panel_ok(int n, const QrWork& w) { return n >= 16 && n <= 1024 && n % 16 == 0 && w.pw != nullptr && w.pivpos != nullptr && w.pw_stride >= qr_panel_work_doubles(n); }
long qr_panel_work_doubles(int n) { return (long)(QP_SR + 2 * n) * n + (long)QP_B * n; }

int launch_qr_panel(Mat A, QrWork w, int n, int n_chains, hipStream_t s) {
    if (!qr_panel_ok(n, w)) { set_error("panel QR: n must be a multiple of 16 in [16, 1024] and the workspace present"); return -1; }
    const dim3 ugrid(n / 16, n_chains);
    const int tpw = (n / 16 + QP_UW - 1) / QP_UW;
#define QP_UPD(U, K) do { if (tpw <= 2) hipLaunchKernelGGL((qp_update_kernel<U, 2>), ugrid, dim3(64 * QP_UW), 0, s, A, w, n, K); \
                          else if (tpw <= 5) hipLaunchKernelGGL((qp_update_kernel<U, 5>), ugrid, dim3(64 * QP_UW), 0, s, A, w, n, K); \
                          else hipLaunchKernelGGL((qp_update_kernel<U, 8>), ugrid, dim3(64 * QP_UW), 0, s, A, w, n, K); } while (0)
    QP_UPD(false, 0);
    for (int k = 0; k < n; k += QP_B) {
#define QP_LAUNCH(NW, CPL) hipLaunchKernelGGL((qp_panel_kernel<NW, CPL>), dim3(1, n_chains), dim3(64 * NW), 0, s, A, w, n, k)
        if (n <= 64) QP_LAUNCH(1, 1); else if (n <= 128) QP_LAUNCH(2, 1); else if (n <= 256) QP_LAUNCH(4, 1); else if (n <= 512) QP_LAUNCH(4, 2);
        else if (n <= 576) QP_LAUNCH(3, 3); else if (n <= 768) QP_LAUNCH(4, 3); else QP_LAUNCH(4, 4);
#undef QP_LAUNCH
        if (k + QP_B < n) QP_UPD(true, k);
    }
#undef QP_UPD
    DQ_HIP(hipGetLastError());
    return 0;
}

}
```

include/dqmc_hip.h:

```cpp
#ifndef DQMC_HIP_H
#define DQMC_HIP_H

#include <stddef.h>
#include <stdint.h>

#ifdef __cplusplus
extern "C" {
#endif

#define DQMC_OK         0
#define DQMC_EINVAL    -1
#define DQMC_ENODEVICE -2
#define DQMC_ENUMERIC  -3
#define DQMC_ERANGE    -4
#define DQMC_ENOMEM    -5

typedef struct dqmc_engine dqmc_engine;

typedef struct dqmc_stats {
    double  acc_rate;
    double  max_err;
    double  sum_err;
    double  n_err;
    int64_t n_accepted;
    int64_t n_proposed;
} dqmc_stats;

const char* dqmc_last_error(void);
const char* dqmc_backend(void);
int dqmc_device_count(void);


int dqmc_to_ldr(int n, const double* M, double* L, double* d, double* R);

int dqmc_ldr_mul_mat(int n, const double* L, const double* d, const double* R,
                     const double* M, double* Lo, double* d_o, double* Ro);

int dqmc_mat_mul_ldr(int n, const double* M,
                     const double* L, const double* d, const double* R,
                     double* Lo, double* d_o, double* Ro);

int dqmc_ldr_mul_ldr(int n,
                     const double* L1, const double* d1, const double* R1,
                     const double* L2, const double* d2, const double* R2,
                     double* Lo, double* d_o, double* Ro);

int dqmc_inv_I_plus_ldr(int n, const double* L, const double* d, const double* R,
                        double* G, double* logdet);

int dqmc_inv_I_plus_ldr_mul_ldr(int n,
                                const double* L1, const double* d1, const double* R1,
                                const double* L2, const double* d2, const double* R2,
                                double* G);

int dqmc_gemm(int n, const double* A, int transA, const double* B, int transB, double* C);

int dqmc_rank1_update(int n, double* G, int i, double delta);


int dqmc_create(dqmc_engine** out, int device, int n_sites, int nt, int n_stab,
                double g, const double gamma[4], const double eta[4],
                const double* expK, const double* invexpK);
int dqmc_create_batch(dqmc_engine** out, int device, int n_chains, int n_sites, int nt, int n_stab,
                      const double* g, const double gamma[4], const double eta[4],
                      const double* expK, const double* invexpK);
int dqmc_n_chains(dqmc_engine* e);
void dqmc_destroy(dqmc_engine* e);

int dqmc_set_fields(dqmc_engine* e, const int64_t* fields);
int dqmc_get_fields(dqmc_engine* e, int64_t* fields);

int dqmc_init(dqmc_engine* e);

int dqmc_get_G(dqmc_engine* e, double* G);
int dqmc_set_G(dqmc_engine* e, const double* G);
int dqmc_get_logdet(dqmc_engine* e, double* logdet);

int dqmc_n_stack(dqmc_engine* e);
int dqmc_get_stack(dqmc_engine* e, int i_stack, double* L, double* d, double* R);

int dqmc_sweep_0_to_beta(dqmc_engine* e, const int32_t* perm, const uint8_t* kprop, const double* u);
int dqmc_sweep_beta_to_0(dqmc_engine* e, const int32_t* perm, const uint8_t* kprop, const double* u);
int dqmc_sync(dqmc_engine* e);
int dqmc_get_stats(dqmc_engine* e, dqmc_stats* out);

int dqmc_wrap_forward(dqmc_engine* e, int l);
int dqmc_wrap_backward(dqmc_engine* e, int l);
int dqmc_local_update_slice(dqmc_engine* e, int l, const int32_t* perm,
                            const uint8_t* kprop, const double* u, int* accepted);
int dqmc_calculate_Bbar(dqmc_engine* e, int i_stack, double* Bbar);
int dqmc_global_action(dqmc_engine* e, double* S);

int dqmc_set_checkerboard(dqmc_engine* e, int n_groups, const int32_t* bonds, const int32_t* group_sizes,
                          const double* cosh_t, const double* sinh_t, const double* diag_factor);

int dqmc_measure_equal_time(dqmc_engine* e, int L1, int L2, double* scalars, double* chi_r);
int dqmc_measure_accumulate(dqmc_engine* e, int L1, int L2);
int dqmc_measure_fetch(dqmc_engine* e, double* scalars_sum, double* chi_r_sum, int64_t* n_measurements, int reset);

int dqmc_sweep_unequal_time(dqmc_engine* e);
int dqmc_get_G_tau(dqmc_engine* e, int which, int l, double* out);

int dqmc_half_warp(dqmc_engine* e, const double* expK_half, const double* invexpK_half, int which, int l, double* out);

int dqmc_measure_unequal_time(dqmc_engine* e, int L1, int L2, int accumulate, double* out);
int dqmc_measure_unequal_fetch(dqmc_engine* e, double* out_sum, int64_t* n_measurements, int reset);

typedef struct dqmc_comm dqmc_comm;
#define DQMC_UNIQUE_ID_BYTES 128
typedef int (*dqmc_sendrecv_fn)(void* user, const void* send, void* recv, size_t bytes, int partner, int tag);

int dqmc_comm_unique_id(void* id );
int dqmc_comm_create_rccl(dqmc_comm** out, const void* id, int world_size, int rank, int device);
int dqmc_comm_create_callbacks(dqmc_comm** out, int world_size, int rank, dqmc_sendrecv_fn fn, void* user);
void dqmc_comm_destroy(dqmc_comm* c);
int dqmc_comm_rank(dqmc_comm* c);
int dqmc_comm_world_size(dqmc_comm* c);
const char* dqmc_comm_transport(dqmc_comm* c);
int dqmc_comm_selftest(dqmc_comm* c);
int dqmc_comm_barrier(dqmc_comm* c);
int dqmc_comm_allreduce_sum(dqmc_comm* c, double* x, int count);

int dqmc_partner_rank(int rank, int world_size, int exchange_attempt);

typedef struct dqmc_exchange_result {
    int    partner;
    int    decider;
    int    accepted;
    int    pad;
    double S;
    double S_prime;
    double S_partner;
    double S_prime_partner;
    double deltaS;
} dqmc_exchange_result;

int dqmc_replica_exchange_round(dqmc_engine* e, dqmc_comm* comm, int exchange_attempt, double u,
                                dqmc_exchange_result* result);

int dqmc_replica_exchange_batch(dqmc_engine* e, dqmc_comm* comm, int exchange_attempt, const double* u,
                                dqmc_exchange_result* result);

int dqmc_update_kernel_time(dqmc_engine* e, double* ms, int64_t* n_launches, int64_t* n_accepted);
int dqmc_slice_path(dqmc_engine* e);
int dqmc_debug_snapshot(dqmc_engine* e, double* wrap_err, int* accepted, unsigned int* sync_words, unsigned int* slice_epoch);
int dqmc_set_profiling(dqmc_engine* e, int on);

#ifdef __cplusplus
}
#endif
#endif
```

Baseline: 12.51 sweeps/s.

## Fuse Q formation into panel QR updates, cache R inverses, emit G transpose

The panel QR no longer runs a separate form-Q kernel after factorisation. Extra blocks in each trailing-update launch now apply the current block reflector to an accumulated Q, overlapping Q formation with the panel sweep at the cost of more workspace and a larger grid. Stack entries also cache the scaled R-inverse X, with a valid flag that every writer clears, so repeated stabilisation solves can skip the triangular or LU solve. The final gemm in inv_I_plus_ldr_mul_ldr also writes G transposed so GT stays valid, and an optional debug check compares it against an explicit transpose.

```diff
diff --git a/dqmc_amd/abi.py b/dqmc_amd/abi.py
--- a/dqmc_amd/abi.py
+++ b/dqmc_amd/abi.py
@@ -34,7 +34,7 @@
     "create", "create_batch", "n_chains", "destroy", "set_fields", "get_fields", "init", "get_G", "set_G", "get_logdet",
     "n_stack", "get_stack", "sweep_0_to_beta", "sweep_beta_to_0", "sync", "get_stats",
     "wrap_forward", "wrap_backward", "local_update_slice", "calculate_Bbar", "global_action", "set_checkerboard",
-    "update_kernel_time", "set_profiling", "slice_path", "debug_snapshot",
+    "update_kernel_time", "set_profiling", "slice_path", "debug_snapshot", "debug_gt_check",
     "measure_equal_time", "measure_accumulate", "measure_fetch",
     "sweep_unequal_time", "get_G_tau", "half_warp", "measure_unequal_time", "measure_unequal_fetch",
     "comm_unique_id", "comm_create_rccl", "comm_create_callbacks", "comm_destroy", "comm_rank", "comm_world_size",
@@ -111,6 +111,8 @@
             g("half_warp").argtypes = [C.c_void_p, c_double_p, c_double_p, C.c_int, C.c_int, c_double_p]
         if self.has_symbol("debug_snapshot"):
             g("debug_snapshot").argtypes = [C.c_void_p, c_double_p, C.c_void_p, C.c_void_p, C.c_void_p]
+        if self.has_symbol("debug_gt_check"):
+            g("debug_gt_check").argtypes = [C.c_void_p, C.c_int, c_double_p, c_int64_p]
         if self.has_symbol("replica_exchange_round"):
             g("comm_unique_id").argtypes = [C.c_void_p]
             g("comm_create_rccl").argtypes = [C.POINTER(C.c_void_p), C.c_void_p, C.c_int, C.c_int, C.c_int]
@@ -460,6 +462,11 @@
         self._c("debug_snapshot", _p(we), acc.ctypes.data, sw.ctypes.data, C.byref(ep))
         return dict(wrap_err=we, accepted=acc, sync_words=sw, slice_epoch=int(ep.value))
 
+    def debug_gt_check(self, on: bool):
+        err = np.zeros(self.C); cnt = np.zeros(1, dtype=np.int64)
+        self._c("debug_gt_check", int(bool(on)), _p(err), cnt.ctypes.data_as(c_int64_p))
+        return err, int(cnt[0])
+
     def slice_path(self) -> int:
         return int(self.lib._sym("slice_path")(self._h))
 
diff --git a/dqmc_amd/csrc/common.h b/dqmc_amd/csrc/common.h
--- a/dqmc_amd/csrc/common.h
+++ b/dqmc_amd/csrc/common.h
@@ -99,8 +99,7 @@
     int* pivpos = nullptr; long pivpos_stride = 0;
 };
 long qr_panel_work_doubles(int n);
-int launch_qr_panel_formq(QrWork w, Mat L, int n, int n_chains, hipStream_t s);
-int launch_qr_panel(Mat A, QrWork w, int n, int n_chains, hipStream_t s);
+int launch_qr_panel(Mat A, Mat L, QrWork w, int n, int n_chains, hipStream_t s);
 long qrcp_coop_sync_granules(int n);
 int qrcp_coop_workgroups(int n, int n_chains);
 enum class QrFamily { Panel, ColumnOwner, Cooperative, Streaming };
diff --git a/dqmc_amd/csrc/engine.hip b/dqmc_amd/csrc/engine.hip
--- a/dqmc_amd/csrc/engine.hip
+++ b/dqmc_amd/csrc/engine.hip
@@ -72,24 +72,30 @@
     Mat L; Vec d; Mat R;
     int* jpvt = nullptr;
     bool* tri = nullptr;
+    Mat X{nullptr, 0};
+    bool* xok = nullptr;
+    void touch() const { if (xok) *xok = false; }
 };
 struct LdrStore {
     int n = 0, C = 0;
-    DevPtr<double> L, d, R;
+    DevPtr<double> L, d, R, X;
     DevPtr<int> jpvt;
-    std::unique_ptr<bool[]> tri;
-    int alloc(int k, int n_, int C_) {
+    std::unique_ptr<bool[]> tri, xok;
+    int alloc(int k, int n_, int C_, bool with_x = false) {
         n = n_; C = C_;
         const size_t nn = (size_t)n * n;
         DQ_TRY(dev_alloc(L, (size_t)k * C * nn)); DQ_TRY(dev_alloc(d, (size_t)k * C * n));
         DQ_TRY(dev_alloc(R, (size_t)k * C * nn)); DQ_TRY(dev_alloc(jpvt, (size_t)k * C * n));
-        tri.reset(new bool[k]());
+        if (with_x) DQ_TRY(dev_alloc(X, (size_t)k * C * nn));
+        tri.reset(new bool[k]()); xok.reset(new bool[k]());
         return 0;
     }
     LdrRef at(int i) const {
         const long nn = (long)n * n;
-        return LdrRef{Mat{L.get() + (long)i * C * nn, nn}, Vec{d.get() + (long)i * C * n, (long)n}, Mat{R.get() + (long)i * C * nn, nn},
-                      jpvt.get() + (long)i * C * n, &tri[i]};
+        LdrRef f{Mat{L.get() + (long)i * C * nn, nn}, Vec{d.get() + (long)i * C * n, (long)n}, Mat{R.get() + (long)i * C * nn, nn},
+                 jpvt.get() + (long)i * C * n, &tri[i]};
+        if (X) { f.X = Mat{X.get() + (long)i * C * nn, nn}; f.xok = &xok[i]; }
+        return f;
     }
 };
 
@@ -144,27 +150,36 @@
         w.sync = qsync.get(); w.sync_stride = qrcp_coop_sync_granules(n); w.abort_words = qabort.get(); w.info = info();
         w.pw = qpw.get(); w.pw_stride = qr_panel_work_doubles(n); w.pivpos = qpivpos.get(); w.pivpos_stride = n;
         if (out.tri) *out.tri = keep;
+        out.touch();
         return launch_to_ldr(plan.qr, A, out.L, out.d, out.R, w, n, C, stream);
     }
-    int r_inverse_scaled(LdrRef F, CVec dinv, Mat X, Mat lu_scratch) {
+    int r_inverse_scaled(LdrRef F, CVec dinv, Mat scratch, Mat lu_scratch, Mat* Xout) {
+        const Mat X = F.X.p ? F.X : scratch;
+        *Xout = X;
+        if (F.xok && *F.xok) return 0;
         if (F.tri && *F.tri && F.jpvt) {
-            if (plan.rinv == KernelPlan::Rinv::Blocked) return launch_tri_solve(F.R, F.jpvt, n, X, dinv, trinv.get(), 16L * (n + 16), n, C, stream);
-            return launch_lu_solve(F.R, F.jpvt, n, X, dinv, 2, n, C, stream);
-        }
-        DQ_TRY(launch_copy(F.R, lu_scratch, nn, C, stream));
-        DQ_TRY(launch_lu_blocked(lu_scratch, lperm(), n, rowpos(), n, nullptr, 0, info(), n, C, stream));
-        return launch_lu_solve(lu_scratch, lperm(), n, X, dinv, 1, n, C, stream);
+            if (plan.rinv == KernelPlan::Rinv::Blocked) DQ_TRY(launch_tri_solve(F.R, F.jpvt, n, X, dinv, trinv.get(), 16L * (n + 16), n, C, stream));
+            else DQ_TRY(launch_lu_solve(F.R, F.jpvt, n, X, dinv, 2, n, C, stream));
+        } else {
+            DQ_TRY(launch_copy(F.R, lu_scratch, nn, C, stream));
+            DQ_TRY(launch_lu_blocked(lu_scratch, lperm(), n, rowpos(), n, nullptr, 0, info(), n, C, stream));
+            DQ_TRY(launch_lu_solve(lu_scratch, lperm(), n, X, dinv, 1, n, C, stream));
+        }
+        if (F.xok) *F.xok = true;
+        return 0;
     }
     int mat_mul_ldr(CMat M, LdrRef F, LdrRef out) {
         DQ_TRY(gemm(M, F.L, T(0), CVec(), CVec(), CVec(F.d)));
         LdrRef q{out.L, out.d, T(1)};
         DQ_TRY(to_ldr(T(0), q));
         if (out.tri) *out.tri = false;
+        out.touch();
         return gemm(T(1), F.R, out.R);
     }
     int ldr_mul_mat(LdrRef F, CMat M, LdrRef out) {
         DQ_TRY(gemm(F.R, M, T(0), CVec(F.d)));
         LdrRef q{T(1), out.d, out.R, out.jpvt, out.tri};
+        q.xok = out.xok;
         DQ_TRY(to_ldr(T(0), q));
         return gemm(F.L, T(1), out.L);
     }
@@ -173,6 +188,7 @@
         LdrRef q{T(1), out.d, T(2)};
         DQ_TRY(to_ldr(T(0), q));
         if (out.tri) *out.tri = false;
+        out.touch();
         DQ_TRY(gemm(F1.L, T(1), out.L));
         return gemm(T(2), F2.R, out.R);
     }
@@ -187,31 +203,31 @@
     }
     int inv_I_plus_ldr(LdrRef F, Mat G, double* logdet ) {
         DQ_TRY(launch_split_d(F.d, V(0), V(1), logdet, n, C, stream));
-        DQ_TRY(r_inverse_scaled(F, V(0), T(1), T(0)));
-        DQ_TRY(launch_add_scaled_cols(T(1), F.L, V(1), T(2), n, C, stream));
+        Mat X; DQ_TRY(r_inverse_scaled(F, V(0), T(1), T(0), &X));
+        DQ_TRY(launch_add_scaled_cols(X, F.L, V(1), T(2), n, C, stream));
         DQ_TRY(launch_transpose_scale(T(2), T(3), CVec(), n, C, stream));
-        DQ_TRY(launch_transpose_scale(T(1), T(4), CVec(), n, C, stream));
+        DQ_TRY(launch_transpose_scale(X, T(4), CVec(), n, C, stream));
         Mat Y; DQ_TRY(solve(T(3), T(4), T(0), logdet, &Y));
         return launch_transpose_scale(Y, G, CVec(), n, C, stream);
     }
-    int inv_I_plus_ldr_mul_ldr(LdrRef F1, LdrRef F2, Mat G) {
+    int inv_I_plus_ldr_mul_ldr(LdrRef F1, LdrRef F2, Mat G, Mat GT = Mat{nullptr, 0}) {
         DQ_TRY(launch_split_d2(F1.d, V(0), V(1), F2.d, V(2), V(3), n, C, stream));
-        DQ_TRY(r_inverse_scaled(F2, V(2), T(1), T(0)));
-        DQ_TRY(gemm(F1.L, T(1), T(2), V(0), CVec(), CVec(), 1));
+        Mat X; DQ_TRY(r_inverse_scaled(F2, V(2), T(1), T(0), &X));
+        DQ_TRY(gemm(F1.L, X, T(2), V(0), CVec(), CVec(), 1));
         DQ_TRY(gemm(F1.R, F2.L, T(2), V(1), CVec(), V(3), 0, 1));
         DQ_TRY(launch_transpose_scale(F1.L, T(3), V(0), n, C, stream));
         Mat Y; DQ_TRY(solve(T(2), T(3), T(0), nullptr, &Y));
-        return gemm(T(1), Y, G);
+        return gemm(X, Y, G, CVec(), CVec(), CVec(), 0, 0, GT);
     }
     int inv_invldr_plus_ldr(LdrRef F1, LdrRef F2, Mat G, bool negate) {
         DQ_TRY(launch_split_d(F1.d, V(0), V(1), nullptr, n, C, stream));
         DQ_TRY(launch_split_d(F2.d, V(2), V(3), nullptr, n, C, stream));
-        DQ_TRY(r_inverse_scaled(F2, V(2), T(1), T(0)));
-        DQ_TRY(gemm(F1.L, T(1), T(2), V(0), CVec(), CVec(), 1));
+        Mat X; DQ_TRY(r_inverse_scaled(F2, V(2), T(1), T(0), &X));
+        DQ_TRY(gemm(F1.L, X, T(2), V(0), CVec(), CVec(), 1));
         DQ_TRY(gemm(F1.R, F2.L, T(2), V(1), CVec(), V(3), 0, 1));
         DQ_TRY(launch_scale_rows(F1.R, V(1), T(3), n, C, stream));
         Mat Y; DQ_TRY(solve(T(2), T(3), T(0), nullptr, &Y));
-        DQ_TRY(gemm(T(1), Y, G));
+        DQ_TRY(gemm(X, Y, G));
         if (negate) DQ_TRY(launch_axpb_identity(G, G, -1.0, 0.0, n, C, stream));
         return 0;
     }
@@ -258,6 +274,7 @@
     DevPtr<double> expv, invexpv;
     DevPtr<UpdateTables> tabs; DevPtr<double> tab8;
     bool gt_valid = false;
+    bool gt_check = false; long long gt_checks = 0; DevPtr<double> gt_err;
     DevPtr<double> G, Gtmp, GT;
     DevPtr<double> pg_eye, pg_ones;
     DevPtr<double> bb0, bb1;
@@ -324,7 +341,7 @@
         DQ_TRY(dev_alloc(tabs, C)); DQ_TRY(dev_alloc(tab8, (size_t)C * 8));
         if (C == 1) { DQ_TRY(dev_alloc(pg_eye, nn)); DQ_TRY(dev_alloc(pg_ones, (size_t)n)); DQ_TRY(launch_set_identity(Mat{pg_eye.get(), nn}, n, 1, s)); const std::vector<double> one_h((size_t)n, 1.0); DQ_HIP(hipMemcpy(pg_ones.get(), one_h.data(), sizeof(double) * n, hipMemcpyHostToDevice)); }
         DQ_TRY(dev_alloc(G, C * nn)); DQ_TRY(dev_alloc(Gtmp, C * nn)); DQ_TRY(dev_alloc(GT, C * nn)); DQ_TRY(dev_alloc(bb0, C * nn)); DQ_TRY(dev_alloc(bb1, C * nn));
-        DQ_TRY(stack.alloc(n_stack, n, C)); DQ_TRY(spare.alloc(1, n, C));
+        DQ_TRY(stack.alloc(n_stack, n, C, C <= 8)); DQ_TRY(spare.alloc(1, n, C));
         DQ_TRY(dev_alloc(logdet, C));
         DQ_TRY(dev_alloc(rs_perm, (size_t)C * nt * n)); DQ_TRY(dev_alloc(rs_k, (size_t)C * nt * n)); DQ_TRY(dev_alloc(rs_u, (size_t)C * nt * n));
         DQ_TRY(dev_alloc(Upanel, (size_t)C * UPDATE_KD * n)); DQ_TRY(dev_alloc(Wpanel, (size_t)C * UPDATE_KD * n)); DQ_TRY(dev_alloc(Cpanel, (size_t)C * UPDATE_KD * UPDATE_KD));
@@ -454,7 +471,7 @@
         DQ_TRY(launch_copy(own.R, last.R, nn, 1, s));
         DQ_HIP(hipMemcpyAsync(last.d.p, own.d.p, sizeof(double) * n, hipMemcpyDeviceToDevice, s));
         DQ_HIP(hipMemcpyAsync(last.jpvt, own.jpvt, sizeof(int) * n, hipMemcpyDeviceToDevice, s));
-        *last.tri = true;
+        *last.tri = true; last.touch();
         for (int i = S - 2; i >= 0; --i) DQ_TRY(ctx.ldr_mul_ldr(stack.at(i + 1), ib.f.at(i), stack.at(i)));
         stack_valid = true;
         gt_valid = false;
@@ -593,7 +610,15 @@
                 else DQ_TRY(ctx.ldr_mul_mat(stack.at(is + 1), bb, stack.at(is)));
                 gt_valid = false;
                 if (l == 0) DQ_TRY(ctx.inv_I_plus_ldr(stack.at(is), mG(), logdet.get()));
-                else DQ_TRY(ctx.inv_I_plus_ldr_mul_ldr(stack.at(is - 1), stack.at(is), mG()));
+                else {
+                    DQ_TRY(ctx.inv_I_plus_ldr_mul_ldr(stack.at(is - 1), stack.at(is), mG(), use_gt() ? Mat{GT.get(), nn} : Mat{nullptr, 0}));
+                    gt_valid = use_gt();
+                    if (gt_check && gt_valid) {
+                        DQ_TRY(launch_transpose_scale(mG(), ctx.T(0), CVec(), n, C, s));
+                        DQ_TRY(launch_max_abs_diff(CMat(GT.get(), nn), ctx.T(0), gt_err.get(), 1, n, C, s));
+                        ++gt_checks;
+                    }
+                }
                 DQ_TRY(launch_max_abs_diff(CMat(Gtmp.get(), nn), mG(), err.get() + n_err, n_stack, n, C, s));
                 ++n_err;
             }
@@ -1064,6 +1089,15 @@
     if (slice_epoch) *slice_epoch = e.slice_epoch;
     return 0;
 }
+int dqmc_debug_gt_check(dqmc_engine* h, int on, double* max_err, int64_t* n_checks) {
+    ENGINE_CALL(h); DQ_TRY(e.sync_and_check());
+    if (!e.gt_err) { DQ_TRY(dev_alloc(e.gt_err, e.C)); DQ_HIP(hipMemset(e.gt_err.get(), 0, sizeof(double) * e.C)); }
+    if (max_err) DQ_HIP(hipMemcpy(max_err, e.gt_err.get(), sizeof(double) * e.C, hipMemcpyDeviceToHost));
+    if (n_checks) *n_checks = e.gt_checks;
+    DQ_HIP(hipMemset(e.gt_err.get(), 0, sizeof(double) * e.C));
+    e.gt_checks = 0; e.gt_check = on != 0;
+    return 0;
+}
 int dqmc_slice_path(dqmc_engine* h) {
     if (!h) return -1;
     Engine& e = h->e;
diff --git a/dqmc_amd/csrc/qr.hip b/dqmc_amd/csrc/qr.hip
--- a/dqmc_amd/csrc/qr.hip
+++ b/dqmc_amd/csrc/qr.hip
@@ -330,8 +330,7 @@
     return launch_assemble_r(A, d, R, w, n, n_chains, s);
 }
 static int to_ldr_panel(Mat A, Mat L, Vec d, Mat R, const QrWork& w, int n, int n_chains, hipStream_t s) {
-    DQ_TRY(launch_qr_panel(A, w, n, n_chains, s));
-    DQ_TRY(launch_qr_panel_formq(w, L, n, n_chains, s));
+    DQ_TRY(launch_qr_panel(A, L, w, n, n_chains, s));
     return launch_assemble_r(A, d, R, w, n, n_chains, s);
 }
 template <int NR>
diff --git a/dqmc_amd/csrc/qr_panel.hip b/dqmc_amd/csrc/qr_panel.hip
--- a/dqmc_amd/csrc/qr_panel.hip
+++ b/dqmc_amd/csrc/qr_panel.hip
@@ -328,13 +328,91 @@
 }
 
 constexpr int QP_UW = 8;
+constexpr int QP_YT = QP_SR / 16;
+
+template <int TPW>
+__device__ __forceinline__ void qp_q_role(double (&red)[QP_UW][QP_YT * 4][64], double* __restrict__ Qacc, double* __restrict__ L,
+                                          const double* __restrict__ Vp, const double* __restrict__ VTp, const double* __restrict__ Tm,
+                                          int n, int k, int cb) {
+    const int t = threadIdx.x, lane = t & 63, wave = t >> 6;
+    const int r16 = lane & 15, kk = lane >> 4;
+    const int col = 16 * cb + r16;
+    double* __restrict__ Qc = Qacc + (long)n * col;
+    const int m_tiles = (n - k) / 16;
+    d4 Qt[TPW]; double v1[TPW][4], v2[TPW][4], tv[4];
+#pragma unroll
+    for (int ti = 0; ti < TPW; ++ti) {
+        const int rt = wave + QP_UW * ti;
+        Qt[ti] = d4{0.0, 0.0, 0.0, 0.0};
+#pragma unroll
+        for (int s = 0; s < 4; ++s) { v1[ti][s] = 0.0; v2[ti][s] = 0.0; }
+        if (rt < m_tiles) {
+            const int r0 = k + 16 * rt;
+#pragma unroll
+            for (int r = 0; r < 4; ++r) Qt[ti][r] = Qc[r0 + kk + 4 * r];
+#pragma unroll
+            for (int s = 0; s < 4; ++s) { v1[ti][s] = VTp[(long)QP_B * (r0 + kk + 4 * s) + r16]; v2[ti][s] = Vp[(long)n * (kk + 4 * s) + (r0 + r16)]; }
+        }
+    }
+#pragma unroll
+    for (int s = 0; s < 4; ++s) tv[s] = Tm[(kk + 4 * s) + QP_B * r16];
+    const bool first = k == 0;
+#pragma unroll
+    for (int ti = 0; ti < TPW; ++ti)
+#pragma unroll
+        for (int r = 0; r < 4; ++r) Qt[ti][r] = first ? ((16 * (wave + QP_UW * ti) + kk + 4 * r == col) ? 1.0 : 0.0) : Qt[ti][r];
+    d4 acc = {0.0, 0.0, 0.0, 0.0};
+#pragma unroll
+    for (int ti = 0; ti < TPW; ++ti) {
+#pragma unroll
+        for (int s = 0; s < 4; ++s) acc = __builtin_amdgcn_mfma_f64_16x16x4f64(v1[ti][s], Qt[ti][s], acc, 0, 0, 0);
+    }
+#pragma unroll
+    for (int r = 0; r < 4; ++r) red[wave][r][lane] = acc[r];
+    __syncthreads();
+    d4 W;
+#pragma unroll
+    for (int r = 0; r < 4; ++r) {
+        double v = red[0][r][lane];
+#pragma unroll
+        for (int q = 1; q < QP_UW; ++q) v += red[q][r][lane];
+        W[r] = v;
+    }
+    d4 wp = {0.0, 0.0, 0.0, 0.0};
+#pragma unroll
+    for (int s = 0; s < 4; ++s) wp = __builtin_amdgcn_mfma_f64_16x16x4f64(tv[s], W[s], wp, 0, 0, 0);
+    wp = -wp;
+#pragma unroll
+    for (int ti = 0; ti < TPW; ++ti) {
+        const int rt = wave + QP_UW * ti;
+        if (rt < m_tiles) {
+            const int r0 = k + 16 * rt;
+#pragma unroll
+            for (int s = 0; s < 4; ++s) Qt[ti] = __builtin_amdgcn_mfma_f64_16x16x4f64(v2[ti][s], wp[s], Qt[ti], 0, 0, 0);
+            if (rt == 0) {
+#pragma unroll
+                for (int r = 0; r < 4; ++r) L[(long)n * (k + kk + 4 * r) + col] = Qt[ti][r];
+            } else {
+#pragma unroll
+                for (int r = 0; r < 4; ++r) Qc[r0 + kk + 4 * r] = Qt[ti][r];
+            }
+        }
+    }
+}
+
 template <bool UPDATE, int TPW>
-__global__ __launch_bounds__(64 * QP_UW) void qp_update_kernel(Mat Am, QrWork w, int n, int k) {
-    constexpr int YT = QP_SR / 16;
+__global__ __launch_bounds__(64 * QP_UW) void qp_update_kernel(Mat Am, QrWork w, int n, int k, Mat Lm, int q_first) {
+    constexpr int YT = QP_YT;
     __shared__ double red[QP_UW][YT * 4][64];
     const int chain = blockIdx.y;
+    double* __restrict__ pw = w.pw + (long)chain * w.pw_stride;
+    if (UPDATE && (int)blockIdx.x >= q_first) {
+        qp_q_role<TPW>(red, pw + (long)(QP_SR + 2 * n) * n + (long)QP_B * n, Lm.at(chain), pw + (long)QP_SR * n + (long)n * k,
+                       pw + (long)QP_SR * n + (long)n * n + (long)QP_B * n + (long)n * k, pw + (long)QP_SR * n + (long)n * n + (long)QP_B * k, n, k,
+                       (int)blockIdx.x - q_first);
+        return;
+    }
     double* __restrict__ A = Am.at(chain);
-    double* __restrict__ pw = w.pw + (long)chain * w.pw_stride;
     double* __restrict__ Y = pw;
     const double* __restrict__ Vp = pw + (long)QP_SR * n + (long)n * k;
     const double* __restrict__ Tm = pw + (long)QP_SR * n + (long)n * n + (long)QP_B * k;
@@ -435,116 +513,25 @@
     }
 }
 
-template <int TPW>
-__global__ __launch_bounds__(64 * QP_UW) void qp_formq_kernel(QrWork w, Mat Lm, int n) {
-    __shared__ double red[QP_UW][4][64];
-    const int chain = blockIdx.y;
-    const double* __restrict__ pw = w.pw + (long)chain * w.pw_stride;
-    const double* __restrict__ Vall = pw + (long)QP_SR * n;
-    const double* __restrict__ Tall = Vall + (long)n * n;
-    const double* __restrict__ VTall = Tall + (long)QP_B * n;
-    double* __restrict__ L = Lm.at(chain);
-    const int t = threadIdx.x, lane = t & 63, wave = t >> 6;
-    const int r16 = lane & 15, kk = lane >> 4;
-    const int cb = blockIdx.x, col = 16 * cb + r16;
-    const int n_tiles = n / 16;
-    d4 Qt[TPW];
-#pragma unroll
-    for (int ti = 0; ti < TPW; ++ti) {
-        const int rt = wave + QP_UW * ti;
-#pragma unroll
-        for (int r = 0; r < 4; ++r) Qt[ti][r] = (16 * rt + kk + 4 * r == col) ? 1.0 : 0.0;
-    }
-    double v1[TPW][4], v2[TPW][4], tv[4], n1[TPW][4], n2[TPW][4], nt_[4];
-    auto load = [&](int k, double (&a1)[TPW][4], double (&a2)[TPW][4], double (&at)[4]) {
-        const double* Vp = Vall + (long)n * 16 * k;
-        const double* Tm = Tall + (long)QP_B * 16 * k;
-        const double* VTp = VTall + (long)n * 16 * k;
-#pragma unroll
-        for (int s = 0; s < 4; ++s) at[s] = Tm[r16 + QP_B * (kk + 4 * s)];
-#pragma unroll
-        for (int ti = 0; ti < TPW; ++ti) {
-            const int rt = wave + QP_UW * ti;
-            const bool in = rt < n_tiles && rt >= k;
-#pragma unroll
-            for (int s = 0; s < 4; ++s) {
-                a1[ti][s] = in ? VTp[(long)QP_B * (16 * rt + kk + 4 * s) + r16] : 0.0;
-                a2[ti][s] = in ? Vp[(long)n * (kk + 4 * s) + (16 * rt + r16)] : 0.0;
-            }
-        }
-    };
-    load(cb, v1, v2, tv);
-    for (int k = cb; k >= 0; --k) {
-        if (k > 0) load(k - 1, n1, n2, nt_);
-        d4 acc = {0.0, 0.0, 0.0, 0.0};
-#pragma unroll
-        for (int ti = 0; ti < TPW; ++ti)
-#pragma unroll
-            for (int s = 0; s < 4; ++s) acc = __builtin_amdgcn_mfma_f64_16x16x4f64(v1[ti][s], Qt[ti][s], acc, 0, 0, 0);
-#pragma unroll
-        for (int r = 0; r < 4; ++r) red[wave][r][lane] = acc[r];
-        __syncthreads();
-        d4 W;
-#pragma unroll
-        for (int r = 0; r < 4; ++r) {
-            double v = red[0][r][lane];
-#pragma unroll
-            for (int q = 1; q < QP_UW; ++q) v += red[q][r][lane];
-            W[r] = v;
-        }
-        d4 wp = {0.0, 0.0, 0.0, 0.0};
-#pragma unroll
-        for (int s = 0; s < 4; ++s) wp = __builtin_amdgcn_mfma_f64_16x16x4f64(tv[s], W[s], wp, 0, 0, 0);
-        wp = -wp;
-#pragma unroll
-        for (int ti = 0; ti < TPW; ++ti)
-#pragma unroll
-            for (int s = 0; s < 4; ++s) Qt[ti] = __builtin_amdgcn_mfma_f64_16x16x4f64(v2[ti][s], wp[s], Qt[ti], 0, 0, 0);
-        __syncthreads();
-#pragma unroll
-        for (int ti = 0; ti < TPW; ++ti)
-#pragma unroll
-            for (int s = 0; s < 4; ++s) { v1[ti][s] = n1[ti][s]; v2[ti][s] = n2[ti][s]; }
-#pragma unroll
-        for (int s = 0; s < 4; ++s) tv[s] = nt_[s];
-    }
-#pragma unroll
-    for (int ti = 0; ti < TPW; ++ti) {
-        const int rt = wave + QP_UW * ti;
-        if (rt < n_tiles) {
-#pragma unroll
-            for (int r = 0; r < 4; ++r) L[(long)n * col + 16 * rt + kk + 4 * r] = Qt[ti][r];
-        }
-    }
-}
-
-int launch_qr_panel_formq(QrWork w, Mat L, int n, int n_chains, hipStream_t s) {
-    const dim3 grid(n / 16, n_chains);
-    const int tpw = (n / 16 + QP_UW - 1) / QP_UW;
-    if (tpw <= 2) hipLaunchKernelGGL((qp_formq_kernel<2>), grid, dim3(64 * QP_UW), 0, s, w, L, n);
-    else if (tpw <= 5) hipLaunchKernelGGL((qp_formq_kernel<5>), grid, dim3(64 * QP_UW), 0, s, w, L, n);
-    else hipLaunchKernelGGL((qp_formq_kernel<8>), grid, dim3(64 * QP_UW), 0, s, w, L, n);
-    DQ_HIP(hipGetLastError());
-    return 0;
-}
-
 static bool qr_panel_ok(int n, const QrWork& w) { return n >= 16 && n <= 1024 && n % 16 == 0 && w.pw != nullptr && w.pivpos != nullptr && w.pw_stride >= qr_panel_work_doubles(n); }
-long qr_panel_work_doubles(int n) { return (long)(QP_SR + 2 * n) * n + (long)QP_B * n; }
-
-int launch_qr_panel(Mat A, QrWork w, int n, int n_chains, hipStream_t s) {
+long qr_panel_work_doubles(int n) { return (long)(QP_SR + 3 * n) * n + (long)QP_B * n; }
+
+int launch_qr_panel(Mat A, Mat L, QrWork w, int n, int n_chains, hipStream_t s) {
     if (!qr_panel_ok(n, w)) { set_error("panel QR: n must be a multiple of 16 in [16, 1024] and the workspace present"); return -1; }
-    const dim3 ugrid(n / 16, n_chains);
-    const int tpw = (n / 16 + QP_UW - 1) / QP_UW;
-#define QP_UPD(U, K) do { if (tpw <= 2) hipLaunchKernelGGL((qp_update_kernel<U, 2>), ugrid, dim3(64 * QP_UW), 0, s, A, w, n, K); \
-                          else if (tpw <= 5) hipLaunchKernelGGL((qp_update_kernel<U, 5>), ugrid, dim3(64 * QP_UW), 0, s, A, w, n, K); \
-                          else hipLaunchKernelGGL((qp_update_kernel<U, 8>), ugrid, dim3(64 * QP_UW), 0, s, A, w, n, K); } while (0)
-    QP_UPD(false, 0);
+    const int nb = n / 16;
+    const int tpw = (nb + QP_UW - 1) / QP_UW;
+#define QP_UPD(U, K, GRID, QFIRST) do { const dim3 ugrid(GRID, n_chains); \
+                          if (tpw <= 2) hipLaunchKernelGGL((qp_update_kernel<U, 2>), ugrid, dim3(64 * QP_UW), 0, s, A, w, n, K, L, QFIRST); \
+                          else if (tpw <= 5) hipLaunchKernelGGL((qp_update_kernel<U, 5>), ugrid, dim3(64 * QP_UW), 0, s, A, w, n, K, L, QFIRST); \
+                          else hipLaunchKernelGGL((qp_update_kernel<U, 8>), ugrid, dim3(64 * QP_UW), 0, s, A, w, n, K, L, QFIRST); } while (0)
+    QP_UPD(false, 0, nb, nb);
     for (int k = 0; k < n; k += QP_B) {
 #define QP_LAUNCH(NW, CPL) hipLaunchKernelGGL((qp_panel_kernel<NW, CPL>), dim3(1, n_chains), dim3(64 * NW), 0, s, A, w, n, k)
         if (n <= 64) QP_LAUNCH(1, 1); else if (n <= 128) QP_LAUNCH(2, 1); else if (n <= 256) QP_LAUNCH(4, 1); else if (n <= 512) QP_LAUNCH(4, 2);
         else if (n <= 576) QP_LAUNCH(3, 3); else if (n <= 768) QP_LAUNCH(4, 3); else QP_LAUNCH(4, 4);
 #undef QP_LAUNCH
-        if (k + QP_B < n) QP_UPD(true, k);
+        if (k + QP_B < n) QP_UPD(true, k, 2 * nb, nb);
+        else QP_UPD(true, k, nb, 0);
     }
 #undef QP_UPD
     DQ_HIP(hipGetLastError());
diff --git a/include/dqmc_hip.h b/include/dqmc_hip.h
--- a/include/dqmc_hip.h
+++ b/include/dqmc_hip.h
@@ -144,6 +144,7 @@
 int dqmc_update_kernel_time(dqmc_engine* e, double* ms, int64_t* n_launches, int64_t* n_accepted);
 int dqmc_slice_path(dqmc_engine* e);
 int dqmc_debug_snapshot(dqmc_engine* e, double* wrap_err, int* accepted, unsigned int* sync_words, unsigned int* slice_epoch);
+int dqmc_debug_gt_check(dqmc_engine* e, int on, double* max_err, int64_t* n_checks);
 int dqmc_set_profiling(dqmc_engine* e, int on);
 
 #ifdef __cplusplus
```

Result: faster. 12.85 sweeps/s, median of 6 (+2.7%).
